# yigolden/JpegLibrary

Measured on AMD Instinct MI355X. Metric: Mpixels/s decoded, 4K 4:2:0 baseline Q75 RST=4, 1 & 8 GPU vs CPU ref, higher is better.
Workload: dtype f32; 1 GPU; 1024 x 3840x2160 420 baseline Q75 DRI=4 per GPU, output interleaved_u8 resident in HBM; images_per_gpu=1024

## Files before the change

jpeglibrary_amd/csrc/capi.cpp:

```cpp
#include <hip/hip_runtime.h>
#include <string.h>

#include <algorithm>
#include <chrono>
#include <exception>
#include <memory>
#include <new>
#include <thread>
#include <vector>

#include "../../include/jpgpu.h"
#include "device_batch.h"
#include "device_encode.h"
#include "device_optimize.h"
#include "host.h"

using namespace jpgpu;

struct jpgpu_batch {
    jpgpu_ctx *ctx;
    DeviceBatch impl;
    explicit jpgpu_batch(jpgpu_ctx *c) : ctx(c), impl(c) {}
};

// ... 311 lines not shown
    case JPGPU_DETAIL_MARKER_IN_DATA: return "Failed to decode JPEG data. Expect raw data from bit stream. Yet a marker is encountered.";
    case JPGPU_DETAIL_STREAM_ENDED: return "Failed to decode JPEG data. The bit stream ended prematurely.";
    case JPGPU_DETAIL_EXPECT_RESTART: return "Expect restart marker.";
    case JPGPU_DETAIL_MISSING_TABLE: return "Failed to decode JPEG data. A Huffman or quantization table is not defined.";
    case JPGPU_DETAIL_UNSUPPORTED_FRAME: return "This type of JPEG stream is not supported on the GPU path.";
    case JPGPU_DETAIL_BAD_HEADER: return "Failed to decode JPEG data. Malformed marker segment.";
    case JPGPU_DETAIL_EARLY_EOI: return "EndOfImage met at a restart boundary; image partially decoded.";
    case JPGPU_DETAIL_UNEXPECTED_END: return "Failed to decode JPEG data. Unexpected end of JPEG data stream.";
    case JPGPU_DETAIL_NULL_TABLE: return "Object reference not set to an instance of an object.";
    default: return "unknown detail";
    }
}


int jpgpu_batch_create(jpgpu_ctx *ctx, jpgpu_batch **out) {
    if (!ctx || !out) return JPGPU_ERR_ARGUMENT;
    *out = new (std::nothrow) jpgpu_batch(ctx);
    return *out ? JPGPU_OK : JPGPU_ERR_OUT_OF_MEMORY;
}
void jpgpu_batch_destroy(jpgpu_batch *b) { delete b; }

#define JPGPU_GUARD(b, expr)                                                   \
    if (!(b)) return JPGPU_ERR_ARGUMENT;                                       \
    try {                                                                      \
        return (expr);                                                         \
    } catch (const DecodeError &e) {                                           \
        (b)->ctx->last_error = e.what();                                       \
        return e.status;                                                       \
    } catch (const std::bad_alloc &) {                                         \
        (b)->ctx->last_error = "host allocation failed";                       \
        return JPGPU_ERR_OUT_OF_MEMORY;                                        \
    } catch (const std::exception &e) {                                        \
        (b)->ctx->last_error = e.what();                                       \
        return JPGPU_ERR_DEVICE;                                               \
    }

int jpgpu_batch_upload(jpgpu_batch *b, const uint8_t *const *jpeg, const size_t *len, int n, int format) {
    JPGPU_GUARD(b, b->impl.upload_files(jpeg, len, n, format));
}
int jpgpu_batch_upload_segments(jpgpu_batch *b, const jpgpu_segment *segments, const int *segments_per_file, int n, int format, unsigned flags) {
    JPGPU_GUARD(b, b->impl.upload_segments(segments, segments_per_file, n, format, flags));
}
int jpgpu_batch_upload_frames(jpgpu_batch *b, const jpgpu_frame *frames, const uint16_t *qt, int n, int format) {
    JPGPU_GUARD(b, b->impl.upload_frames(frames, qt, n, format));
}
int jpgpu_batch_decode(jpgpu_batch *b) { JPGPU_GUARD(b, b->impl.decode()); }
static int run_entropy_stages(DeviceBatch &impl) {
    impl.note_entropy_only_request();
    const int rc = impl.run_marker_index();
    return rc != JPGPU_OK ? rc : impl.run_huffman();
}
int jpgpu_batch_run_entropy(jpgpu_batch *b) { JPGPU_GUARD(b, run_entropy_stages(b->impl)); }
int jpgpu_batch_run_idct(jpgpu_batch *b) { JPGPU_GUARD(b, b->impl.run_idct()); }
int jpgpu_batch_sync(jpgpu_batch *b) { JPGPU_GUARD(b, b->impl.sync()); }
int jpgpu_batch_size(const jpgpu_batch *b) { return b ? b->impl.size() : 0; }

int jpgpu_batch_image_info(const jpgpu_batch *b, int i, jpgpu_image_info *info) {
    if (!b || !info) return JPGPU_ERR_ARGUMENT;
    const ImagePlan *img = b->impl.image(i);
    if (!img) return JPGPU_ERR_ARGUMENT;
    memset(info, 0, sizeof *info);
    info->status = img->status;
    info->detail = img->detail;
    info->width = img->width;
    info->height = img->height;
    info->precision = img->precision;
    info->num_components = img->num_components;
    info->sof = img->sof;
    info->restart_interval = img->restart_interval;
    info->mcus_per_line = img->mcus_per_line;
    info->mcus_per_column = img->mcus_per_column;
    info->blocks_per_mcu = img->blocks_per_mcu;
    info->total_blocks = img->total_blocks;
    info->out_offset = img->out_offset;
    info->out_bytes = img->out_bytes;
    info->coef_offset = img->coef_offset;
    memcpy(info->plane, img->plane, sizeof info->plane);
    if (img->status != JPGPU_OK) b->ctx->last_error = img->error;
    return JPGPU_OK;
}

int jpgpu_batch_result(jpgpu_batch *b, int i, jpgpu_image_result *res) { JPGPU_GUARD(b, b->impl.result(i, res)); }
void *jpgpu_batch_output_device(const jpgpu_batch *b, uint64_t *total_bytes) { return b ? b->impl.output_device(total_bytes) : nullptr; }
void *jpgpu_batch_coefficients_device(const jpgpu_batch *b, uint64_t *total_blocks) { return b ? b->impl.coefs_device(total_blocks) : nullptr; }
int jpgpu_batch_download_output(jpgpu_batch *b, int i, void *dst, size_t cap) { JPGPU_GUARD(b, b->impl.download_output(i, dst, cap)); }
int jpgpu_batch_download_coefficients(jpgpu_batch *b, int i, int16_t *dst, size_t cap_blocks) {
    JPGPU_GUARD(b, b->impl.download_coefficients(i, dst, cap_blocks));
}
int jpgpu_batch_upload_coefficients(jpgpu_batch *b, int i, const int16_t *src, size_t nblocks) {
    JPGPU_GUARD(b, b->impl.upload_coefficients(i, src, nblocks));
}
int jpgpu_batch_stage_ms(jpgpu_batch *b, float ms[4]) { JPGPU_GUARD(b, b->impl.stage_ms(ms)); }
int jpgpu_batch_subseq_rounds(const jpgpu_batch *b) { return b ? b->impl.last_subseq_rounds() : 0; }
int jpgpu_batch_set_partial_flush(jpgpu_batch *b, int on) {
    if (!b) return JPGPU_ERR_ARGUMENT;
    b->impl.set_partial_flush(on != 0);
    return JPGPU_OK;
}
int jpgpu_batch_marker_fallbacks(const jpgpu_batch *b) { return b ? b->impl.marker_fallbacks() : 0; }
int jpgpu_batch_progressive_replays(const jpgpu_batch *b) { return b ? b->impl.progressive_replays() : 0; }
int jpgpu_batch_subseq_fallbacks(const jpgpu_batch *b) { return b ? b->impl.subseq_fallbacks() : 0; }
int jpgpu_batch_progressive_fallbacks(const jpgpu_batch *b) { return b ? b->impl.progressive_fallbacks() : 0; }
int jpgpu_batch_ingest_stats(const jpgpu_batch *b, jpgpu_ingest_stats *stats) {
    if (!b || !stats) return JPGPU_ERR_ARGUMENT;
    const IngestStats &s = b->impl.ingest_stats();
    stats->threads = s.threads;
    stats->n_header_only = s.n_header_only;
    stats->n_full_walk = s.n_full_walk;
    stats->parse_ms = s.parse_ms;
    stats->copy_ms = s.copy_ms;
    stats->full_walk_ms = s.full_walk_ms;
    stats->layout_ms = s.layout_ms;
    stats->total_ms = s.total_ms;
    stats->n_pinned_dma = s.n_pinned_dma;
    stats->n_linearised = s.n_linearised;
    return JPGPU_OK;
}
size_t jpgpu_sizeof_plan_stats(void) { return sizeof(jpgpu_plan_stats); }
int jpgpu_batch_plan_stats(const jpgpu_batch *b, jpgpu_plan_stats *stats) {
    if (!b || !stats) return JPGPU_ERR_ARGUMENT;
    b->impl.plan_stats(stats);
    return JPGPU_OK;
}
static_assert(JPGPU_PROGRESSIVE_CHAINS == jpgpu_ctx::kProgChains, "jpgpu_progressive_plan: one count per chain stream");
size_t jpgpu_sizeof_progressive_plan(void) { return sizeof(jpgpu_progressive_plan); }
int jpgpu_batch_progressive_plan(const jpgpu_batch *b, jpgpu_progressive_plan *plan) {
    if (!b || !plan) return JPGPU_ERR_ARGUMENT;
    b->impl.progressive_plan(plan);
    return JPGPU_OK;
}
static_assert(JPGPU_IDCT_LAYOUT_CLASSES == kNumIdctLayoutClasses, "jpgpu_batch_idct_work: one count per K3 layout class");
int jpgpu_batch_idct_work(const jpgpu_batch *b, int32_t *counts, int n) {
    if (!b || !counts || n != JPGPU_IDCT_LAYOUT_CLASSES) return JPGPU_ERR_ARGUMENT;
    b->impl.idct_work(counts);
    return JPGPU_OK;
}
int jpgpu_batch_totals(const jpgpu_batch *b, uint64_t *compressed_bytes, uint64_t *blocks, uint64_t *pixels, uint64_t *output_bytes) {
    if (!b) return JPGPU_ERR_ARGUMENT;
    b->impl.totals(compressed_bytes, blocks, pixels, output_bytes);
    return JPGPU_OK;
}

}


namespace {

[[noreturn]] void throw_for_result(const jpgpu_image_result &res) {
    throw DecodeError(res.status, jpgpu_detail_string(res.detail), res.detail);
}

void write_block_expanded(jpgpu_write_block_fn fn, void *user, const int16_t *block, int component_index, int x, int y, int hs, int vs) {
    if (hs == 1 && vs == 1) {
        fn(user, block, component_index, x, y);
        return;
    }
    int16_t temp[64];
    int hshift = 0, vshift = 0;
    while ((1 << (hshift + 1)) <= hs) hshift++;
    while ((1 << (vshift + 1)) <= vs) vshift++;
    for (int v = 0; v < vs; v++)
        for (int h = 0; h < hs; h++) {
            for (int i = 0; i < 8; i++) {
                const int16_t *row = block + ((8 * v + i) >> vshift) * 8;
                for (int j = 0; j < 8; j++) temp[8 * i + j] = row[(8 * h + j) >> hshift];
            }
            fn(user, temp, component_index, x + 8 * h, y + 8 * v);
// ... 887 lines not shown
```

jpeglibrary_amd/csrc/common.h:

```cpp
#pragma once
#include <stdint.h>

namespace jpgpu {

constexpr int kMaxScanComponents = 4;
constexpr int kMaxBlocksPerMcu = 16;
constexpr int kHuffLutBits = 9;
constexpr int kHuffLutSize = 1 << kHuffLutBits;
constexpr int kMaxHuffSlots = 8;

struct alignas(16) DevHuffTable {
    uint16_t lut[kHuffLutSize];
    uint16_t maxcode[18];
    uint8_t valoffset[20];
    uint8_t values[256];
    uint8_t pad[8];
};
static_assert(sizeof(DevHuffTable) % 16 == 0, "DevHuffTable must be a multiple of 16 bytes");

struct alignas(16) DevQuantTable {
    uint16_t q[64];
};

struct DevScanComponent {
    uint8_t component_index;
    uint8_t h, v;
    uint8_t hs, vs;
    uint8_t quant_slot;
    uint8_t dc_slot, ac_slot;
};

enum OutputFormat : int32_t { kFmtInterleavedU8 = 0, kFmtPlanarU8 = 1, kFmtPlanarI16 = 2, kFmtRgbU8 = 3, kFmtRgbaU8 = 4, kFmtExtendedU16 = 5, kFmtInterleavedU8Scaled = 6 };
constexpr int kNumOutputFormats = 7;
constexpr bool fmt_is_sample_bytes(int f) { return f == kFmtInterleavedU8 || f == kFmtInterleavedU8Scaled; }
constexpr bool fmt_is_interleaved(int f) { return fmt_is_sample_bytes(f) || f == kFmtRgbU8 || f == kFmtRgbaU8; }
constexpr int fmt_bytes_per_pixel_rgb(int f) { return f == kFmtRgbaU8 ? 4 : 3; }

struct YccRgbFactors {
    int32_t cr_r, cr_g, cb_b, cb_g;
};

struct alignas(16) DevScan {
    uint64_t data_off;
    uint64_t coef_off;
    uint64_t out_off;
    uint64_t plane_off[kMaxScanComponents];
    uint32_t plane_pitch[kMaxScanComponents];
    uint32_t data_len;
    uint32_t dri;
    uint32_t total_mcus, mcus_per_line, mcus_per_column;
    uint32_t n_intervals;
    uint32_t ends_off;
    uint32_t image_index;
    uint32_t level_shift;
    uint16_t width, height;
    uint8_t precision, frame_components, scan_components, max_h, max_v, blocks_per_mcu;
    uint8_t restart_check_at_end;
    uint8_t shadow_mask;
    DevScanComponent comp[kMaxScanComponents];
    uint8_t blk_comp[kMaxBlocksPerMcu];
    uint8_t blk_x[kMaxBlocksPerMcu];
    uint8_t blk_y[kMaxBlocksPerMcu];
    uint16_t huff_pool[kMaxHuffSlots];
    uint16_t quant_pool[kMaxScanComponents];
    uint64_t reserved0;
    uint32_t chunk_off;
    uint32_t n_chunks;
    uint32_t sub_off;
    uint32_t n_subs;
    uint8_t kind;
    uint8_t ss, se, ah, al;
    uint8_t frame_bpm;
    uint8_t fblk_base[kMaxScanComponents];
    uint8_t publishes;
    uint8_t sub_shift;
    uint8_t wave_next;
    uint8_t debug_delay_ms;
    uint8_t pad1[2];
    uint16_t hblocks[kMaxScanComponents];
    uint16_t vblocks[kMaxScanComponents];
    uint32_t units_per_line;
    uint32_t dep[3];
    uint32_t last_interval;
    uint32_t first_scan;
    uint32_t sr_set;
    uint32_t pad2;
};
constexpr uint32_t kNoDep = 0xFFFFFFFFu;
constexpr uint32_t kFailBlockBase = 0xFFFFFFFFu;
constexpr uint32_t kIdctPartialMcu = 0xFFFFFFFFu;
constexpr uint64_t kScanStoreHoldsSamples = 1;
struct alignas(16) DisposeJob {
    uint64_t coef_off;
    uint32_t n_blocks;
    uint32_t bpm, level_shift;
    uint8_t blk_comp[kMaxBlocksPerMcu];
    uint8_t n[kMaxScanComponents];
    uint16_t quant[kMaxScanComponents][kMaxScanComponents];
    uint32_t pad[3];
};
constexpr uint8_t kKeepUnreachedMcus = 0x80;
enum ScanKind : uint8_t { kScanSequential = 0, kScanFrameOnly = 1, kScanProgressive = 2 };
static_assert(sizeof(DevScan) % 16 == 0, "DevScan must be a multiple of 16 bytes");

struct alignas(16) DevScanStatus {
    uint32_t n_ends;
    uint32_t terminator;
    uint32_t first_error;
    uint32_t decoded_mcus;
    uint32_t end_pos;
    uint32_t pad[3];
};

struct HuffWork {
    uint32_t scan;
    uint32_t first_interval;
};
struct ChunkWork {
    uint32_t scan;
    uint32_t chunk;
};
struct GatherPiece {
    uint64_t src;
    uint64_t dst_off;
    uint32_t len;
    uint32_t pad;
};
struct ChunkSum {
    uint32_t rst_cnt;
    uint32_t keep_cnt;
    uint32_t first_term;
    uint32_t pad;
};
struct IdctWork {
    uint32_t scan;
    uint32_t first_mcu;
    uint32_t n_mcus;
    uint32_t mcus_per_tile;
};

struct ExtendPlanes {
    uint64_t plane_off[4];
    uint64_t out_off;
    uint32_t pitch[4];
    uint32_t hshift[4], vshift[4];
    uint32_t width, height, ncomp, precision;
    uint32_t hcnt[4], vcnt[4];
    uint32_t max_h, max_v;
};

constexpr uint32_t kNoError = 0xFFFFFFFFu;

enum Detail : uint32_t {
    kDetailNone = 0,
    kDetailInvalidHuffmanCode = 1,
    kDetailMarkerInData = 2,
    kDetailStreamEnded = 3,
    kDetailExpectRestart = 4,
    kDetailMissingTable = 5,
    kDetailUnsupportedFrame = 6,
    kDetailBadHeader = 7,
    kDetailEarlyEoi = 8,
    kDetailUnexpectedEnd = 9,
    kDetailNullTable = 10,
    kDetailSpinTimeout = 11
};

}
```

jpeglibrary_amd/csrc/device_batch.cpp:

```cpp
#include "device_batch.h"

#include <hip/hip_runtime.h>
#include <sched.h>
#include <stdio.h>
#include <stdlib.h>
#include <string.h>

#include <algorithm>
#include <atomic>
#include <chrono>
#include <thread>

#include "host_pool.h"
#include "kernels.h"

namespace jpgpu {

static inline uint64_t align_up(uint64_t v, uint64_t a) { return (v + a - 1) / a * a; }

hipError_t DevBuffer::reserve(size_t bytes) {
    if (bytes <= cap && ptr) return hipSuccess;
    if (ptr) {
        hipError_t e = hipFree(ptr);
        ptr = nullptr;
        cap = 0;
        if (e != hipSuccess) return e;
    }
    if (bytes == 0) bytes = 256;
    hipError_t e = hipMalloc(&ptr, bytes);
    if (e == hipSuccess) cap = bytes;
    return e;
}
void DevBuffer::release() {
    if (ptr) (void)hipFree(ptr);
    ptr = nullptr;
    cap = 0;
}

DeviceBatch::~DeviceBatch() {
    if (ctx_) (void)hipSetDevice(ctx_->device);
    for (DevBuffer *b : {&d_sub_work_, &d_sub_final_work_, &d_sub_scan_ids_, &d_sub_exit_a_, &d_sub_exit_b_, &d_sub_nblk_, &d_sub_first_, &d_sub_entry_, &d_sub_dcsum_, &d_sub_dcentry_, &d_sub_changed_, &d_sub_same_, &d_sub_perm_, &d_k1_desc_, &d_k1_tickets_, &d_k2_tickets_, &d_sr_luts_, &d_sr_set_scan_, &d_k1_order_, &d_prog_snapshot_, &d_dispose_, &d_verify_, &d_lut_pool_, &d_prog_work_, &d_prog_sync_, &d_planes_, &d_extend_desc_, &d_gather_, &d_rgb_scratch_, &d_chunk_work_, &d_chunk_sums_, &d_unstuffed_, &d_ends_u_, &d_input_, &d_scans_, &d_status_, &d_ends_, &d_huff_pool_, &d_quant_pool_, &d_huff_work_, &d_idct_work_, &d_idct_work_split_, &d_coefs_, &d_out_})
        b->release();
    for (hipEvent_t &e : ev_pool_)
        if (e) (void)hipEventDestroy(e);
    if (done_ev_) (void)hipEventDestroy(done_ev_);
    if (h_k1_giveup_) (void)hipHostFree(h_k1_giveup_);
}

int DeviceBatch::fail(int status, const std::string &msg) {
    ctx_->last_error = msg;
    return status;
}
int DeviceBatch::hip_fail(hipError_t e, const char *what) {
    return fail(e == hipErrorOutOfMemory ? JPGPU_ERR_OUT_OF_MEMORY : JPGPU_ERR_DEVICE, std::string(what) + ": " + hipGetErrorString(e));
}

namespace {

class PlanHandler final : public ScanHandler {
  public:
    explicit PlanHandler(std::vector<ScanJob> *jobs, bool first_scan_only = false, const std::vector<int> *forced = nullptr)
        : jobs_(jobs), first_scan_only_(first_scan_only), forced_(forced) {}
    PlanHandler(const std::vector<size_t> *ends, int swallow) : jobs_(nullptr), replay_ends_(ends), swallow_(swallow) {}
    const std::vector<size_t> &sequential_ends() const { return ends_; }
    void on_frame(HostDecoder &dec, int sof) override {
        sof_ = sof;
        baseline_ = false;
        flush_progressive();
        if (sof == kSOF0 || sof == kSOF1) {
            geo_ = BaselineGeometry::latch(dec, dec.frame_header());
            baseline_ = true;
        } else if (sof == kSOF2) {
            prog_.begin(dec, dec.frame_header());
        }
    }
    void on_scan(HostDecoder &dec, MarkerReader &reader, const ScanHeader &scan) override {
        const uint8_t *entropy = reader.remaining_bytes();
        const size_t len = (size_t)reader.remaining_byte_count();
        if (prog_.active()) {
            prog_.add_scan(dec, scan, entropy, len);
            return;
        }
        if (!baseline_)
            throw DecodeError(JPGPU_ERR_NOT_SUPPORTED, "Only Huffman DCT frames (SOF0, SOF1, SOF2) run on this path.", kDetailUnsupportedFrame);
        if (scan.num_components == 0) {
            const uint64_t mcus = (uint64_t)geo_.mcus_per_line * (uint64_t)geo_.mcus_per_column;
            if (geo_.restart_interval != 0 && mcus >= geo_.restart_interval && len != 0 &&
                !(len >= 2 && entropy[0] == 0xFF && entropy[1] != 0x00 && entropy[1] != 0xFF))
                throw DecodeError(JPGPU_ERR_INVALID_OPERATION, "Expect restart marker.", kDetailExpectRestart);
            if (first_scan_only_)
                throw DecodeError(JPGPU_ERR_NOT_SUPPORTED, "A scan without components is not supported by the optimizer path.", kDetailUnsupportedFrame);
            if (geo_.restart_interval != 0 && mcus >= geo_.restart_interval)
                throw DecodeError(JPGPU_ERR_NOT_SUPPORTED, "A scan without components in front of restart markers is not supported.", kDetailUnsupportedFrame);
            reader.try_advance((int)find_scan_end(entropy, len));
            return;
        }
        if (replay_ends_) {
            const int k = replayed_++;
            if (k > swallow_ || k >= (int)replay_ends_->size())
                throw DecodeError(JPGPU_ERR_NOT_SUPPORTED, "A scan behind a scan that left one byte unread is not supported.", kDetailUnsupportedFrame);
            reader.try_advance((int)(*replay_ends_)[k] + (k == swallow_ ? 1 : 0));
            return;
        }
        jobs_->push_back(make_scan_job(dec, geo_, scan, entropy, len, first_scan_only_));
        if (!first_scan_only_) {
            const bool forced = forced_ != nullptr && std::find(forced_->begin(), forced_->end(), (int)ends_.size()) != forced_->end();
            ends_.push_back(find_scan_end(entropy, len));
            jobs_->back().forced_swallow = forced && ends_.back() < len;
            reader.try_advance((int)ends_.back() + (jobs_->back().forced_swallow ? 1 : 0));
            return;
        }
        reader.try_advance(first_scan_only_ ? (int)len : (int)find_scan_end(entropy, len));
    }
    void on_dispose(HostDecoder &) override { flush_progressive(); }
    const BaselineGeometry &geo() const { return prog_geo_valid_ ? prog_geo_ : geo_; }
    int sof() const { return sof_; }

  private:
    void flush_progressive() {
        if (!prog_.active()) return;
        if (jobs_) {
            jobs_->push_back(prog_.make_frame_job());
            for (ScanJob &j : prog_.scans()) jobs_->push_back(std::move(j));
            prog_geo_ = prog_.geo();
// ... 941 lines not shown
```

jpeglibrary_amd/csrc/device_batch.h:

```cpp
#pragma once
#include <hip/hip_runtime_api.h>

#include <map>
#include <string>
#include <vector>

#include "../../include/jpgpu.h"
#include "common.h"
#include "host.h"
#include "kernels.h"

namespace jpgpu {
int default_host_threads();
int granted_host_cpus();
}

struct StagingRing {
    static constexpr int kMaxSlots = 16;
    int n_slots = 8;
    size_t slot_bytes = 32u << 20;
    uint8_t *slot[kMaxSlots] = {};
    hipEvent_t drained[kMaxSlots] = {};
    uint32_t *verdict = nullptr;
    size_t verdict_cap = 0;
// ... 12 lines not shown
    std::string last_error;
    int num_cus = 0;
    uint64_t device_bytes = 0;
};

namespace jpgpu {

struct DevBuffer {
    void *ptr = nullptr;
    size_t cap = 0;
    hipError_t reserve(size_t bytes);
    void release();
};

struct IngestStats {
    int threads = 0;
    int n_header_only = 0;
    int n_full_walk = 0;
    float parse_ms = 0, copy_ms = 0, full_walk_ms = 0, layout_ms = 0, total_ms = 0;
    int n_pinned_dma = 0;
    int n_linearised = 0;
};

struct ImagePlan {
    int status = JPGPU_OK;
    int detail = 0;
    std::string error;
    int late_status = JPGPU_OK, late_detail = 0;
    bool replay_skip = false;
    std::string late_error;
    int swallow_job = -1, swallow_status = JPGPU_OK, swallow_detail = 0;
    std::string swallow_error;
    uint16_t width = 0, height = 0;
    uint8_t precision = 0, num_components = 0, sof = 0;
    uint32_t restart_interval = 0;
    uint32_t mcus_per_line = 0, mcus_per_column = 0, blocks_per_mcu = 0;
    uint64_t total_blocks = 0;
    uint64_t out_offset = 0, out_bytes = 0;
    uint64_t planes_offset = 0, planes_bytes = 0;
    uint64_t coef_offset = 0;
    jpgpu_plane_info plane[4] = {};
    std::vector<int> jobs;
    uint64_t file_offset = 0;
    size_t file_len = 0;
};

class WorkCrew;

class DeviceBatch {
  public:
    const IngestStats &ingest_stats() const { return ingest_; }
    void plan_stats(jpgpu_plan_stats *st) const;
    void progressive_plan(jpgpu_progressive_plan *p) const;
    void idct_work(int32_t counts[kNumIdctLayoutClasses]) const;
    explicit DeviceBatch(jpgpu_ctx *ctx) : ctx_(ctx) {}
    ~DeviceBatch();

    int upload_files(const uint8_t *const *jpeg, const size_t *len, int n, int format);
    void set_forced_swallow(const std::vector<int> &ordinals) { forced_swallow_ = ordinals; }
    int upload_segments(const jpgpu_segment *segments, const int *segments_per_file, int n, int format, unsigned flags);
    int upload_progressive_frame(const ProgressiveFrame &frame, const uint8_t *file, size_t file_len, int sof, int format);
    int upload_progressive_scan(const ProgressiveFrame &frame, int scan_index, bool first_scan);
    int snapshot_progressive_store();
    int rerun_failed_progressive_scan(bool first_scan);
    int upload_progressive_dispose(const ProgressiveFrame &frame, int format);
    int upload_single_job(const ScanJob &job, int format, const void *initial_output, size_t initial_output_bytes);
    int upload_frames(const jpgpu_frame *frames, const uint16_t *qt , int n, int format);

    int run_marker_index();
    int run_huffman();
    int run_subseq_sync(const uint32_t **final_state, const uint32_t **first_block);
    int run_idct();
    int run_progressive();
    int decode();
    int sync();

    int size() const { return (int)images_.size(); }
    const ImagePlan *image(int i) const { return (i >= 0 && i < (int)images_.size()) ? &images_[i] : nullptr; }
    int result(int i, jpgpu_image_result *res);
    void *output_device(uint64_t *total) const {
        if (total) *total = out_bytes_;
        return d_out_.ptr;
    }
    void *coefs_device(uint64_t *total_blocks) const {
        if (total_blocks) *total_blocks = total_blocks_;
        return d_coefs_.ptr;
    }
    int download_output(int i, void *dst, size_t cap);
    int download_coefficients(int i, int16_t *dst, size_t cap_blocks);
    int upload_coefficients(int i, const int16_t *src, size_t nblocks);
    int stage_ms(float ms[4]);
    void totals(uint64_t *compressed, uint64_t *blocks, uint64_t *pixels, uint64_t *out_bytes) const;
    int format() const { return format_; }
    void note_entropy_only_request() { in_decode_request_ = false; }
    int last_subseq_rounds() const { return last_subseq_rounds_; }
    int progressive_fallbacks() const { return prog_fallbacks_; }
    int subseq_fallbacks() const { return k2s_fallbacks_; }
    int marker_fallbacks() const { return k1_fallbacks_; }
    int progressive_replays() const { return prog_replays_; }
    void set_partial_flush(bool on) { partial_flush_ = on; }
    void set_entropy_only(bool on) { entropy_only_ = on; }
    void set_preset_restart_intervals(std::vector<int> v) { preset_dri_ = std::move(v); }
    void set_preset_no_subseq(std::vector<uint8_t> v) { preset_no_subseq_ = std::move(v); }

  private:
    friend class OptimizeBatch;
    bool entropy_only_ = false;
    std::vector<int> preset_dri_;
    std::vector<uint8_t> preset_no_subseq_;
    int fail(int status, const std::string &msg);
    int hip_fail(hipError_t e, const char *what);
    int layout_and_upload(const std::vector<const uint8_t *> &file_ptr, const std::vector<size_t> &file_len);
    void plan_image_geometry(ImagePlan &img, const BaselineGeometry &geo) const;
    struct FilePlan;
    void plan_file_headers(const uint8_t *file, size_t len, FilePlan &fp) const;
    void plan_file_full(const uint8_t *file, size_t len, int index, FilePlan &fp) const;
    void plan_swallowed_terminator(FilePlan &fp, const uint8_t *file, size_t len, bool identify_is_clean) const;
    struct FileSegs;
    int stage_files(WorkCrew &crew, const std::vector<FileSegs> &files, const std::vector<FilePlan> &plans, bool pinned);
    int mark_work();
    int order_upload_behind_work();
    std::pair<const uint8_t *, size_t> arena_span_ = {nullptr, 0};
    hipEvent_t done_ev_ = nullptr;
    bool work_in_flight_ = false;
    int verify_plans(const std::vector<FilePlan> &plans, const std::vector<int> &spec, std::vector<uint32_t> &first);
    bool whole_files_ = false;
    bool files_resident_ = false;
    IngestStats ingest_;
    DevBuffer d_verify_;
    int fetch_status();
    int clear_partial_outputs();
    bool keep_progressive_store_ = false;
    bool defer_refusal_ = false;
    bool keep_canvas_ = false;
    struct OutClear {
        uint64_t first, second;
        uint64_t planes_first, planes_bytes;
    };
    std::vector<OutClear> out_clear_;

    jpgpu_ctx *ctx_;
    int format_ = JPGPU_FMT_INTERLEAVED_U8;
    std::vector<ImagePlan> images_;
    std::vector<ScanJob> jobs_;
    std::vector<int> job_image_;
    std::vector<uint64_t> job_entropy_off_;
    std::vector<DevScan> h_scans_;
    std::vector<DevScanStatus> h_status_;
    bool status_valid_ = false;
    std::vector<DevHuffTable> huff_pool_;
    std::vector<DevQuantTable> quant_pool_;
    int n_huff_slots_ = 1;
    int redo_swallowed(int i, int job, jpgpu_image_result *res);
    std::vector<int> forced_swallow_;
    struct Redo {
        jpgpu_image_result res;
        std::string error;
    };
    std::map<int, Redo> redo_;
    std::vector<SubseqPool> k2_pools_;
    uint32_t k2_ticket_base_[kK2MaxPools] = {};
    uint32_t k2_tab_bytes_ = 0;
    int n_huff_work_ = 0, n_idct_work_ = 0;
    int idct_class_begin_[kNumIdctLayoutClasses + 1] = {};
    std::vector<int> idct_later_begin_;
    uint64_t total_blocks_ = 0, out_bytes_ = 0, planes_bytes_ = 0, input_bytes_ = 0, compressed_bytes_ = 0, total_pixels_ = 0;
    DevBuffer d_planes_;
    DevBuffer d_extend_desc_;
    DevBuffer d_gather_;
    bool in_decode_request_ = false;
    uint32_t total_ends_ = 0;

    DevBuffer d_lut_pool_;
    DevBuffer d_sub_work_, d_sub_scan_ids_, d_sub_exit_a_, d_sub_exit_b_, d_sub_nblk_, d_sub_first_, d_sub_entry_, d_sub_dcsum_, d_sub_dcentry_, d_sub_changed_, d_sub_same_, d_sub_perm_;
    DevBuffer d_prog_snapshot_;
    uint64_t prog_snapshot_blocks_ = 0;
    DevBuffer d_dispose_;
    std::vector<DisposeJob> dispose_jobs_;
    uint32_t dispose_max_blocks_ = 0;
    int run_dispose_passes(hipStream_t stream);
    bool dispose_done_ = false;
    int replay_failed_progressive();
    bool replay_done_ = false, replay_possible_ = false, prog_by_scan_ = false;
    bool replay_layout_active_ = false, in_replay_ = false;
    bool partial_flush_ = true;
    std::vector<std::pair<size_t, ScanJob>> replay_saved_jobs_;
    int restore_after_replay();
    int prog_replays_ = 0;
  public:
    int clear_progressive_stores();
  private:
    DevBuffer d_k1_desc_, d_k1_tickets_, d_k1_order_;
    int n_k1_groups_ = 0;
    uint32_t *h_k1_giveup_ = nullptr;
    uint32_t k1_epoch_ = 0, k1_tag_ = 0;
    bool k1_onepass_ = true;
    int k1_fallbacks_ = 0;
    bool sub_same_valid_ = false;
    int n_sub_work_ = 0, n_sub_gather_ = 0, n_sub_scans_ = 0, n_sub_final_work_ = 0, sub_final_spl_ = 2;
    int n_sr_sets_ = 0;
    DevBuffer d_sub_final_work_;
    std::vector<SubseqPool> sub_pools_;
    uint32_t total_subs_ = 0, max_subs_per_scan_ = 0;
    std::vector<uint32_t> sub_scan_ids_;
    int last_subseq_rounds_ = 0;
    int k2s_budget_ = 0, k2s_issued_ = 0, k2s_fallbacks_ = 0;
    bool k2s_unchecked_ = false, k2s_idct_behind_ = false, k2s_host_checked_ = false;
    int check_subseq_rounds();
    DevBuffer d_prog_work_, d_prog_sync_;
    std::vector<int> prog_begin_;
    std::vector<int> prog_stream_begin_;
    int prog_pipe_begin_ = 0, prog_pipe_count_ = 0;
    std::vector<int> prog_chain_begin_[jpgpu_ctx::kProgChains];
    bool prog_chains_ok_ = false;
    bool prog_pipelined_ = false;
    uint32_t prog_spin_budget_ = 1u << 22;
    int prog_scans_ = 0, prog_max_deps_ = 0, prog_wave_tails_ = 0, prog_launch_form_ = 0;
    int prog_chain_scans_[jpgpu_ctx::kProgChains] = {};
    int prog_fallbacks_ = 0;
    std::vector<std::pair<uint64_t, uint64_t>> prog_clear_;
    struct RgbConvert {
        uint32_t image;
        uint64_t out_offset, pixels;
        int components;
    };
    std::vector<RgbConvert> rgb_convert_;
    DevBuffer d_rgb_scratch_;
    DevBuffer d_chunk_work_, d_chunk_sums_;
    int n_chunk_work_ = 0;
    DevBuffer d_unstuffed_, d_ends_u_;
    DevBuffer d_input_, d_scans_, d_status_, d_ends_, d_huff_pool_, d_quant_pool_, d_huff_work_, d_idct_work_, d_coefs_, d_out_, d_k2_tickets_;
    DevBuffer d_sr_luts_, d_sr_set_scan_;
    std::vector<hipEvent_t> ev_pool_;
    size_t ev_used_ = 0;
    std::vector<bool> ev_serial_;
    static constexpr int kSerialEvery = 8;
    bool overlap_ok_ = false;
    int decodes_since_query_ = 0;
    int huff_split_ = 0;
    int idct_split_begin_[2][kNumIdctLayoutClasses + 1] = {};
    DevBuffer d_idct_work_split_;
};

}
```

jpeglibrary_amd/csrc/device_batch_launch.cpp:

```cpp
#include "device_batch.h"

#include <hip/hip_runtime.h>
#include <stdio.h>
#include <stdlib.h>
#include <string.h>

#include <algorithm>
#include <atomic>
#include <chrono>
#include <thread>
#include <vector>

#include "kernels.h"

namespace jpgpu {

int DeviceBatch::run_marker_index() {
    status_valid_ = false;
    redo_.clear();
    if (k1_onepass_) {
        const char *bev = getenv("JPGPU_K1_SPIN_BUDGET");
        const uint32_t budget = bev ? (uint32_t)strtoul(bev, nullptr, 10) : (1u << 20);
        uint32_t *tickets = (uint32_t *)d_k1_tickets_.ptr;
        hipError_t e1 = launch_marker_onepass(ctx_->stream, (const uint8_t *)d_input_.ptr, (const DevScan *)d_scans_.ptr, (const ChunkWork *)d_k1_order_.ptr,
                                              n_k1_groups_, d_k1_desc_.ptr, tickets, k1_epoch_, ++k1_tag_ ? k1_tag_ : ++k1_tag_, budget,
                                              h_k1_giveup_, (uint32_t *)d_ends_.ptr, (DevScanStatus *)d_status_.ptr,
                                              (uint8_t *)d_unstuffed_.ptr, (uint32_t *)d_ends_u_.ptr);
        if (e1 != hipSuccess) return hip_fail(e1, "marker_onepass_kernel");
        k1_epoch_++;
        return mark_work();
    }
    hipError_t e = launch_marker_index(ctx_->stream, (const uint8_t *)d_input_.ptr, (const DevScan *)d_scans_.ptr, (int)h_scans_.size(),
                                       (const ChunkWork *)d_chunk_work_.ptr, n_chunk_work_, (ChunkSum *)d_chunk_sums_.ptr,
                                       (uint32_t *)d_ends_.ptr, (DevScanStatus *)d_status_.ptr, (uint8_t *)d_unstuffed_.ptr,
                                       (uint32_t *)d_ends_u_.ptr);
    return e == hipSuccess ? mark_work() : hip_fail(e, "marker_index_kernel");
}
int DeviceBatch::run_huffman() {
    status_valid_ = false;
    redo_.clear();
    dispose_done_ = false;
    hipError_t e = launch_huffman(ctx_->stream, (const uint8_t *)d_unstuffed_.ptr, (const DevScan *)d_scans_.ptr, (const HuffWork *)d_huff_work_.ptr,
                                  n_huff_work_, (const uint32_t *)d_ends_u_.ptr, (DevScanStatus *)d_status_.ptr,
                                  (const DevHuffTable *)d_huff_pool_.ptr, (int16_t *)d_coefs_.ptr, n_huff_slots_, (const uint8_t *)d_lut_pool_.ptr, k2_tab_bytes_);
    if (e != hipSuccess) return hip_fail(e, "huffman_decode_kernel");
    for (size_t p = 0; p < k2_pools_.size(); p++) {
        const int waves = huffman_waves(k2_tab_bytes_);
        const int groups = std::min(ctx_->num_cus > 0 ? ctx_->num_cus : 256, (k2_pools_[p].count + waves - 1) / waves);
        e = launch_huffman_pool(ctx_->stream, (const uint8_t *)d_unstuffed_.ptr, (const DevScan *)d_scans_.ptr,
                                (const HuffWork *)d_huff_work_.ptr + n_huff_work_ + k2_pools_[p].first, k2_pools_[p].count, (uint32_t *)d_k2_tickets_.ptr + p,
                                k2_ticket_base_[p], groups, (const uint32_t *)d_ends_u_.ptr, (DevScanStatus *)d_status_.ptr, (int16_t *)d_coefs_.ptr,
                                n_huff_slots_, (const uint8_t *)d_lut_pool_.ptr, k2_tab_bytes_);
        if (e != hipSuccess) return hip_fail(e, "huffman_pool_kernel");
        k2_ticket_base_[p] += (uint32_t)k2_pools_[p].count + (uint32_t)(groups * waves);
    }
    if (n_sub_work_ > 0) {
        const int max_rounds = (int)max_subs_per_scan_ + 2;
        const int first_budget = getenv("JPGPU_SUBSEQ_BUDGET") ? std::max(2, atoi(getenv("JPGPU_SUBSEQ_BUDGET"))) : kSubseqFirstBudget;
        const int device_rounds = k2s_host_checked_ ? 0 : std::min(max_rounds, k2s_budget_ > 0 ? k2s_budget_ : first_budget);
        k2s_issued_ = std::min(device_rounds, kSubseqMaxDeviceRounds);
        k2s_unchecked_ = device_rounds > 0;
        k2s_idct_behind_ = false;
        e = launch_subseq_decode(ctx_->stream, (const uint8_t *)d_unstuffed_.ptr, (const DevScan *)d_scans_.ptr, (const HuffWork *)d_sub_work_.ptr,
                                 n_sub_work_, (const uint32_t *)d_sub_scan_ids_.ptr, n_sub_scans_, (const uint32_t *)d_ends_u_.ptr,
                                 (DevScanStatus *)d_status_.ptr, (const DevHuffTable *)d_huff_pool_.ptr, (uint32_t *)d_sub_exit_a_.ptr,
                                 (uint32_t *)d_sub_exit_b_.ptr, (uint32_t *)d_sub_nblk_.ptr, (uint32_t *)d_sub_first_.ptr,
                                 (uint32_t *)d_sub_entry_.ptr, d_sub_dcsum_.ptr, d_sub_dcentry_.ptr, (uint32_t *)d_sub_changed_.ptr, (int16_t *)d_coefs_.ptr, n_huff_slots_, max_rounds,
                                 &last_subseq_rounds_, (const uint8_t *)d_lut_pool_.ptr, (const HuffWork *)d_sub_final_work_.ptr, n_sub_final_work_,
                                 (uint32_t *)d_sub_same_.ptr, &sub_same_valid_, device_rounds, (const HuffWork *)d_sub_work_.ptr + n_sub_work_, n_sub_gather_,
                                 (const HuffWork *)d_sub_final_work_.ptr + n_sub_final_work_, sub_pools_.data(), (int)sub_pools_.size(), ctx_->num_cus,
                                 (uint32_t *)d_sub_perm_.ptr, sub_final_spl_, k2_tab_bytes_, (const uint8_t *)d_sr_luts_.ptr);
        if (e != hipSuccess) return hip_fail(e, "subsequence decode");
    }
    const int rc = run_progressive();
    return rc != JPGPU_OK ? rc : mark_work();
}
int DeviceBatch::run_subseq_sync(const uint32_t **final_state, const uint32_t **first_block) {
    *final_state = (const uint32_t *)d_sub_exit_a_.ptr;
    *first_block = (const uint32_t *)d_sub_first_.ptr;
    if (n_sub_work_ <= 0) return JPGPU_OK;
    status_valid_ = false;
    hipError_t e = launch_subseq_sync(ctx_->stream, (const uint8_t *)d_unstuffed_.ptr, (const DevScan *)d_scans_.ptr, (const HuffWork *)d_sub_work_.ptr,
                                      n_sub_work_, (const uint32_t *)d_sub_scan_ids_.ptr, n_sub_scans_, (const uint32_t *)d_ends_u_.ptr,
                                      (DevScanStatus *)d_status_.ptr, (const DevHuffTable *)d_huff_pool_.ptr, (uint32_t *)d_sub_exit_a_.ptr,
                                      (uint32_t *)d_sub_exit_b_.ptr, (uint32_t *)d_sub_nblk_.ptr, (uint32_t *)d_sub_first_.ptr,
                                      (uint32_t *)d_sub_entry_.ptr, d_sub_dcsum_.ptr, d_sub_dcentry_.ptr, (uint32_t *)d_sub_changed_.ptr,
                                      n_huff_slots_, (int)max_subs_per_scan_ + 2, &last_subseq_rounds_, (const uint8_t *)d_lut_pool_.ptr,
                                      final_state, (uint32_t *)d_sub_same_.ptr, &sub_same_valid_, 0 ,
                                      (const HuffWork *)d_sub_work_.ptr + n_sub_work_, n_sub_gather_, (const uint8_t *)d_sr_luts_.ptr);
    if (e != hipSuccess) return hip_fail(e, "subsequence synchronisation");
    return mark_work();
}
int DeviceBatch::run_progressive() {
    if (prog_begin_.size() <= 1 && prog_clear_.empty()) return JPGPU_OK;
    status_valid_ = false;
    for (size_t k = 0; k < prog_clear_.size() && !keep_progressive_store_;) {
        uint64_t first = prog_clear_[k].first, blocks = prog_clear_[k].second;
        for (k++; k < prog_clear_.size() && prog_clear_[k].first == first + blocks; k++) blocks += prog_clear_[k].second;
        hipError_t e = hipMemsetAsync((int16_t *)d_coefs_.ptr + first * 64, 0, (size_t)blocks * 128, ctx_->stream);
        if (e != hipSuccess) return hip_fail(e, "hipMemsetAsync(progressive store)");
    }
    if (prog_begin_.size() <= 1) return JPGPU_OK;
    const char *dbg_max = getenv("JPGPU_DEBUG_MAX_PROGRESSIVE_SCANS");
    const int n_streams = prog_stream_begin_.back() - prog_stream_begin_.front();
    const int n_waves = prog_pipe_count_;
    const size_t lds_per_wg = (progressive_stream_lds_bytes(n_huff_slots_) + 1023) / 1024 * 1024;
    const int cus = ctx_->num_cus > 0 ? ctx_->num_cus : 256;
    int per_cu = (int)std::min<size_t>(32, (160u << 10) / lds_per_wg);
    {
        static std::atomic<int> cached[kMaxHuffSlots + 1];
        const int slot_key = std::min(std::max(n_huff_slots_, 0), kMaxHuffSlots);
        int occ = cached[slot_key].load(std::memory_order_relaxed);
        if (occ == 0) {
            occ = progressive_stream_blocks_per_cu(n_huff_slots_);
            cached[slot_key].store(occ > 0 ? occ : -1, std::memory_order_relaxed);
        }
        if (occ > 0) per_cu = std::min(per_cu, occ);
    }
    const bool force = getenv("JPGPU_PROG_FORCE_PIPELINE") != nullptr;
    const bool resident = n_waves <= per_cu * 3 / 4 * cus;
    const bool fits = resident || force;
    const int launch_mode = resident && !force ? 1 : 2;
    const bool no_chains = getenv("JPGPU_PROG_NO_CHAINS") != nullptr;
    if (!(prog_pipelined_ && fits) && prog_chains_ok_ && !no_chains && !dbg_max && getenv("JPGPU_PROG_BY_SCAN") == nullptr && !prog_by_scan_ && n_streams > 0) {
// ... 19 lines not shown
            if ((e = hipStreamWaitEvent(st, cx->prog_ev[jpgpu_ctx::kProgChains], 0)) != hipSuccess) return hip_fail(e, "hipStreamWaitEvent");
            for (size_t jx = 0; jx + 1 < prog_chain_begin_[x].size(); jx++) {
                e = launch_progressive_streams(st, (const uint8_t *)d_unstuffed_.ptr, (const DevScan *)d_scans_.ptr,
                                               (const HuffWork *)d_prog_work_.ptr + prog_chain_begin_[x][jx],
                                               prog_chain_begin_[x][jx + 1] - prog_chain_begin_[x][jx], (const uint32_t *)d_ends_u_.ptr,
                                               (DevScanStatus *)d_status_.ptr, (const DevHuffTable *)d_huff_pool_.ptr, (int16_t *)d_coefs_.ptr,
                                               n_huff_slots_, 0, 0, nullptr);
                if (e != hipSuccess) return hip_fail(e, "progressive_stream_kernel");
            }
            if ((e = hipEventRecord(cx->prog_ev[x], st)) != hipSuccess) return hip_fail(e, "hipEventRecord");
            if ((e = hipStreamWaitEvent(cx->stream, cx->prog_ev[x], 0)) != hipSuccess) return hip_fail(e, "hipStreamWaitEvent");
        }
        return JPGPU_OK;
    }
    if (prog_pipelined_ && fits && !dbg_max) {
        hipError_t e0 = hipMemsetAsync(d_prog_sync_.ptr, 0, 256, ctx_->stream);
        if (e0 != hipSuccess) return hip_fail(e0, "hipMemsetAsync(progressive sync)");
        const int n = n_waves;
        prog_launch_form_ = launch_mode == 1 ? JPGPU_PROG_LAUNCH_PIPELINED_GATED : JPGPU_PROG_LAUNCH_PIPELINED_FORCED;
        hipError_t e = launch_progressive_streams(ctx_->stream, (const uint8_t *)d_unstuffed_.ptr, (const DevScan *)d_scans_.ptr,
                                                  (const HuffWork *)d_prog_work_.ptr + prog_pipe_begin_, n,
                                                  (const uint32_t *)d_ends_u_.ptr, (DevScanStatus *)d_status_.ptr,
                                                  (const DevHuffTable *)d_huff_pool_.ptr, (int16_t *)d_coefs_.ptr, n_huff_slots_, launch_mode, prog_spin_budget_, (uint32_t *)d_prog_sync_.ptr);
        if (e != hipSuccess) return hip_fail(e, "progressive_stream_kernel");
        return JPGPU_OK;
    }
    prog_launch_form_ = JPGPU_PROG_LAUNCH_BY_LEVEL;
    for (size_t k = 0; k + 1 < prog_begin_.size(); k++) {
        if (dbg_max && (int)k >= atoi(dbg_max)) break;
        hipError_t e = launch_progressive(ctx_->stream, (const uint8_t *)d_unstuffed_.ptr, (const DevScan *)d_scans_.ptr,
                                          (const HuffWork *)d_prog_work_.ptr + prog_begin_[k], prog_begin_[k + 1] - prog_begin_[k],
                                          (const uint32_t *)d_ends_u_.ptr, (DevScanStatus *)d_status_.ptr,
                                          (const DevHuffTable *)d_huff_pool_.ptr, (int16_t *)d_coefs_.ptr, n_huff_slots_);
        if (e != hipSuccess) return hip_fail(e, "progressive_scan_kernel");
        e = launch_progressive_streams(ctx_->stream, (const uint8_t *)d_unstuffed_.ptr, (const DevScan *)d_scans_.ptr,
                                       (const HuffWork *)d_prog_work_.ptr + prog_stream_begin_[k],
                                       prog_stream_begin_[k + 1] - prog_stream_begin_[k], (const uint32_t *)d_ends_u_.ptr,
                                       (DevScanStatus *)d_status_.ptr, (const DevHuffTable *)d_huff_pool_.ptr, (int16_t *)d_coefs_.ptr,
                                       n_huff_slots_, 0, 0, nullptr);
        if (e != hipSuccess) return hip_fail(e, "progressive_stream_kernel");
    }
    return JPGPU_OK;
}
int DeviceBatch::clear_partial_outputs() {
    for (const auto &c : out_clear_) {
        hipError_t e = hipMemsetAsync((uint8_t *)d_out_.ptr + c.first, 0, c.second, ctx_->stream);
        if (e == hipSuccess && format_ == JPGPU_FMT_EXTENDED_U16 && c.planes_bytes)
            e = hipMemsetAsync((uint8_t *)d_planes_.ptr + c.planes_first, 0, c.planes_bytes, ctx_->stream);
        if (e == hipSuccess && d_rgb_scratch_.ptr && c.first + c.second <= d_rgb_scratch_.cap)
            e = hipMemsetAsync((uint8_t *)d_rgb_scratch_.ptr + c.first, 0, c.second, ctx_->stream);
        if (e != hipSuccess) return hip_fail(e, "hipMemsetAsync(output)");
    }
    return JPGPU_OK;
}

int DeviceBatch::clear_progressive_stores() {
    dispose_done_ = false;
    for (const auto &c : prog_clear_) {
        hipError_t e = hipMemsetAsync((int16_t *)d_coefs_.ptr + c.first * 64, 0, (size_t)c.second * 128, ctx_->stream);
        if (e != hipSuccess) return hip_fail(e, "hipMemsetAsync(progressive store)");
    }
    return JPGPU_OK;
}

int DeviceBatch::run_dispose_passes(hipStream_t stream) {
    if (dispose_jobs_.empty() || dispose_done_) return JPGPU_OK;
    dispose_done_ = true;
    const hipError_t e = launch_dispose_pass(stream, (int16_t *)d_coefs_.ptr, (const DisposeJob *)d_dispose_.ptr, (int)dispose_jobs_.size(), dispose_max_blocks_,
                                             (const DevQuantTable *)d_quant_pool_.ptr);
    return e == hipSuccess ? JPGPU_OK : hip_fail(e, "dispose_pass_kernel");
}

int DeviceBatch::run_idct() {
    redo_.clear();
    if (k2s_unchecked_) k2s_idct_behind_ = true;
    const YccRgbFactors kf = ycc_rgb_factors();
    int rc0 = clear_partial_outputs();
    if (rc0 != JPGPU_OK) return rc0;
    if ((rc0 = run_dispose_passes(ctx_->stream)) != JPGPU_OK) return rc0;
    const bool extended = format_ == JPGPU_FMT_EXTENDED_U16;
    hipError_t e = launch_idct(ctx_->stream, (const int16_t *)d_coefs_.ptr, (const DevScan *)d_scans_.ptr, (const IdctWork *)d_idct_work_.ptr,
                               idct_class_begin_, (const DevScanStatus *)d_status_.ptr, (const DevQuantTable *)d_quant_pool_.ptr,
                               extended ? (uint8_t *)d_planes_.ptr : (uint8_t *)d_out_.ptr, extended ? (int)JPGPU_FMT_PLANAR_I16 : format_, kf,
                               (uint8_t *)d_rgb_scratch_.ptr);
    if (e != hipSuccess) return hip_fail(e, "idct_output_kernel");
    for (size_t lv = 0; lv + 1 < idct_later_begin_.size(); lv++) {
        int cb[kNumIdctLayoutClasses + 1];
        cb[0] = idct_later_begin_[lv];
        for (int c = 1; c <= kNumIdctLayoutClasses; c++) cb[c] = idct_later_begin_[lv + 1];
        e = launch_idct(ctx_->stream, (const int16_t *)d_coefs_.ptr, (const DevScan *)d_scans_.ptr, (const IdctWork *)d_idct_work_.ptr, cb,
                        (const DevScanStatus *)d_status_.ptr, (const DevQuantTable *)d_quant_pool_.ptr,
                        extended ? (uint8_t *)d_planes_.ptr : (uint8_t *)d_out_.ptr, extended ? (int)JPGPU_FMT_PLANAR_I16 : format_, kf,
                        (uint8_t *)d_rgb_scratch_.ptr);
        if (e != hipSuccess) return hip_fail(e, "idct_output_kernel (ordered scans)");
    }
    if (extended) {
        std::vector<ExtendPlanes> desc;
        uint32_t max_pixels = 0;
        for (const ImagePlan &img : images_) {
            if (img.status != JPGPU_OK || img.jobs.empty() || img.out_bytes == 0) continue;
            ExtendPlanes g;
            memset(&g, 0, sizeof g);
            const BaselineGeometry &geo = jobs_[img.jobs[0]].geo;
            for (int c = 0; c < 4; c++) g.pitch[c] = 1;
            for (int c = 0; c < img.num_components && c < 4; c++) {
                g.plane_off[c] = img.planes_offset + img.plane[c].offset;
                g.pitch[c] = img.plane[c].pitch;
                const int hs = geo.max_h / std::max<int>(1, geo.frame.components[c].h), vs = geo.max_v / std::max<int>(1, geo.frame.components[c].v);
                while ((1 << (g.hshift[c] + 1)) <= hs) g.hshift[c]++;
                while ((1 << (g.vshift[c] + 1)) <= vs) g.vshift[c]++;
                g.hcnt[c] = std::max<int>(1, geo.frame.components[c].h);
                g.vcnt[c] = std::max<int>(1, geo.frame.components[c].v);
            }
            bool flush = false;
            for (int j : img.jobs) flush |= jobs_[j].kind != kScanSequential;
            g.max_h = flush ? 0u : (uint32_t)geo.max_h;
            g.max_v = flush ? 0u : (uint32_t)geo.max_v;
            g.out_off = img.out_offset;
            g.width = img.width;
            g.height = img.height;
            g.ncomp = img.num_components;
            g.precision = img.precision;
            max_pixels = std::max<uint64_t>(max_pixels, std::min<uint64_t>((uint64_t)img.width * img.height, 0xFFFFFFFFu));
            desc.push_back(g);
        }
        if (!desc.empty()) {
            e = d_extend_desc_.reserve(desc.size() * sizeof(ExtendPlanes));
            if (e != hipSuccess) return hip_fail(e, "hipMalloc(extend descriptors)");
            e = hipMemcpyAsync(d_extend_desc_.ptr, desc.data(), desc.size() * sizeof(ExtendPlanes), hipMemcpyHostToDevice, ctx_->stream);
            if (e == hipSuccess) e = hipStreamSynchronize(ctx_->stream);
            if (e != hipSuccess) return hip_fail(e, "hipMemcpyAsync(extend descriptors)");
            e = launch_extend_u16(ctx_->stream, (const uint8_t *)d_planes_.ptr, (uint8_t *)d_out_.ptr, (const ExtendPlanes *)d_extend_desc_.ptr,
                                  (int)desc.size(), max_pixels);
            if (e != hipSuccess) return hip_fail(e, "extend_u16_kernel");
        }
    }
    for (const RgbConvert &rc : rgb_convert_) {
        e = launch_ycc_to_rgb(ctx_->stream, (const uint8_t *)d_rgb_scratch_.ptr + rc.out_offset, (uint8_t *)d_out_.ptr + rc.out_offset, rc.pixels,
                              rc.components, format_ == JPGPU_FMT_RGBA_U8 ? 4 : 3, kf);
        if (e != hipSuccess) return hip_fail(e, "ycc_to_rgb_kernel");
    }
    return mark_work();
}

int DeviceBatch::decode() {
    hipError_t e = hipSetDevice(ctx_->device);
    if (e != hipSuccess) return hip_fail(e, "hipSetDevice");
    if (replay_layout_active_ && !in_replay_) {
        const int rr = restore_after_replay();
        if (rr != JPGPU_OK) return rr;
    }
    if (ev_used_ + 4 > 4 * 256) {
        ev_used_ = 0;
        ev_serial_.clear();
    }
    if (ev_pool_.size() < ev_used_ + 4) {
        for (int k = 0; k < 64; k++) {
            hipEvent_t ev = nullptr;
            e = hipEventCreate(&ev);
            if (e != hipSuccess) return hip_fail(e, "hipEventCreate");
            ev_pool_.push_back(ev);
        }
    }
    hipEvent_t *ev = &ev_pool_[ev_used_];
    redo_.clear();
    in_decode_request_ = true;
    const bool serial = !overlap_ok_ || (decodes_since_query_ % kSerialEvery) == 0;
// ... 118 lines not shown
```

jpeglibrary_amd/csrc/device_batch_layout.cpp:

```cpp
#include "device_batch.h"

#include <hip/hip_runtime.h>
#include <stdio.h>
#include <stdlib.h>
#include <string.h>

#include <algorithm>
#include <atomic>
#include <chrono>
#include <thread>
#include <vector>

#include "kernels.h"

namespace jpgpu {

static inline uint64_t align_up(uint64_t v, uint64_t a) { return (v + a - 1) / a * a; }

namespace {
template <typename T>
void xcd_interleave(std::vector<T> &w, int xcds) {
    if (xcds <= 1 || w.size() < (size_t)xcds * 8) return;
    const size_t n = w.size(), per = (n + xcds - 1) / xcds;
    std::vector<T> m;
// ... 8 lines not shown

int DeviceBatch::layout_and_upload(const std::vector<const uint8_t *> &file_ptr, const std::vector<size_t> &file_len) {
    dispose_done_ = false;
    if (!in_replay_) {
        replay_done_ = false;
        replay_possible_ = false;
        prog_by_scan_ = false;
        replay_layout_active_ = false;
        replay_saved_jobs_.clear();
        for (ImagePlan &img : images_) img.replay_skip = false;
    }
    hipError_t e = hipSetDevice(ctx_->device);
    if (e != hipSuccess) return hip_fail(e, "hipSetDevice");
    {
        const int rc0 = order_upload_behind_work();
        if (rc0 != JPGPU_OK) return rc0;
    }
    status_valid_ = false;
    ev_used_ = 0;
    keep_progressive_store_ = false;
    defer_refusal_ = false;

    if (!files_resident_) {
        uint64_t in_off = 256;
        for (size_t i = 0; i < images_.size(); i++) {
            images_[i].file_offset = in_off;
            if (images_[i].status == JPGPU_OK && !images_[i].jobs.empty()) in_off = align_up(in_off + file_len[i], 256);
        }
        input_bytes_ = in_off + 256;
    }
    hipStream_t up = ctx_->upload_stream;

    int dbg_delay_scan = -1, dbg_delay_ms = 0;
    if (const char *dd = getenv("JPGPU_DEBUG_DELAY_SCAN")) {
        if (sscanf(dd, "%d:%d", &dbg_delay_scan, &dbg_delay_ms) != 2) dbg_delay_scan = -1;
    }
    const bool dbg_status = getenv("JPGPU_DEBUG_STATUS") != nullptr;
    huff_pool_.clear();
    quant_pool_.clear();
    h_scans_.assign(jobs_.size(), DevScan());
    std::vector<HuffWork> huff_work;
    std::vector<ChunkWork> chunk_work;
    std::vector<ChunkWork> k1_order;
    std::vector<HuffWork> sub_work;
    uint32_t subseq_shift = 10;
    {
        uint64_t dri0_bits = 0;
        for (size_t j = 0; j < jobs_.size(); j++)
            if (jobs_[j].kind == kScanSequential && jobs_[j].geo.restart_interval == 0) dri0_bits += (uint64_t)jobs_[j].entropy_len * 8;
        while (subseq_shift < 12 && (dri0_bits >> subseq_shift) >= 500000u) subseq_shift++;
        while (subseq_shift > 9 && (dri0_bits >> subseq_shift) < 4096u) subseq_shift--;
        if (const char *ev = getenv("JPGPU_SUBSEQ_SHIFT")) subseq_shift = (uint32_t)std::min(14, std::max(8, atoi(ev)));
    }
    uint32_t idct_tiles_per_wg = (uint32_t)kIdctTilesPerWg;
    {
        uint64_t blocks = 0;
        for (const ScanJob &job : jobs_)
            if (job.kind != kScanProgressive) blocks += (uint64_t)job.geo.mcus_per_line * job.geo.mcus_per_column * (uint64_t)std::max(1, job.blocks_per_mcu);
        const uint64_t tiles = blocks / (uint64_t)kIdctBlocksPerWg + 1, want_wgs = 3ull * (uint64_t)(ctx_->num_cus > 0 ? ctx_->num_cus : 256);
        while (idct_tiles_per_wg > 1 && tiles / idct_tiles_per_wg < want_wgs) idct_tiles_per_wg /= 2;
    }
    std::vector<std::vector<HuffWork>> prog_work_by_ordinal, prog_streams_by_ordinal;
    std::vector<std::vector<HuffWork>> prog_chain_work[jpgpu_ctx::kProgChains];
    prog_chains_ok_ = true;
    prog_scans_ = prog_max_deps_ = prog_wave_tails_ = prog_launch_form_ = 0;
    for (int &n : prog_chain_scans_) n = 0;
    const uint32_t stream_max_intervals = getenv("JPGPU_PROG_STREAM_MAX_INTERVALS") ? (uint32_t)atoi(getenv("JPGPU_PROG_STREAM_MAX_INTERVALS")) : 16u;
    prog_clear_.clear();
    prog_pipelined_ = getenv("JPGPU_PROG_NO_PIPELINE") == nullptr;
    prog_spin_budget_ = getenv("JPGPU_PROG_SPIN_BUDGET") ? (uint32_t)strtoul(getenv("JPGPU_PROG_SPIN_BUDGET"), nullptr, 10) : (1u << 17);
    prog_fallbacks_ = 0;
    rgb_convert_.clear();
    sub_scan_ids_.clear();
    total_subs_ = 0;
    max_subs_per_scan_ = 0;
    sub_same_valid_ = false;
    k2s_budget_ = 0;
    k2s_unchecked_ = k2s_idct_behind_ = false;
    k2s_host_checked_ = getenv("JPGPU_SUBSEQ_HOST_CHECK") != nullptr || keep_canvas_;
    dispose_jobs_.clear();
    dispose_max_blocks_ = 0;
    std::vector<IdctWork> idct_work;
    std::vector<IdctWork> idct_work_by_class[kNumIdctLayoutClasses];
    std::vector<std::vector<IdctWork>> idct_later_levels;
    std::vector<IdctWork> idct_partial;
    std::vector<int> scan_level(jobs_.size(), 0);
    const bool tile_align = !(getenv("JPGPU_TILE_ALIGN") && atoi(getenv("JPGPU_TILE_ALIGN")) == 0);
    uint64_t out_off = 0, coef_off = 0, planes_off = 0;
    uint32_t ends_off = 0, total_chunks = 0;
    compressed_bytes_ = 0;
    total_pixels_ = 0;
    n_huff_slots_ = 1;
    for (const ScanJob &job : jobs_) n_huff_slots_ = std::max(n_huff_slots_, job.n_huff);
    k2_tab_bytes_ = kK2AcTabBytes + kK2DcTabBytes;
    for (const ScanJob &job : jobs_) {
        if (job.kind != kScanSequential) continue;
        uint32_t bytes = 0;
        for (int k = 0; k < job.n_huff; k++) {
            bool is_dc = false;
            for (int c = 0; c < job.scan_components; c++) is_dc |= job.dc_slot[c] == k;
            bytes += is_dc ? kK2DcTabBytes : kK2AcTabBytes;
        }
        k2_tab_bytes_ = std::max(k2_tab_bytes_, bytes);
    }
    const uint32_t huff_intervals_per_wg = 64u * (uint32_t)huffman_waves(k2_tab_bytes_);
    struct HuffKey {
        uint8_t bits[16];
        uint16_t num_values;
        uint8_t values[256];
    };
    std::vector<HuffKey> huff_keys;
    auto huff_index = [&](const HuffTable &t) -> uint16_t {
        for (size_t i = 0; i < huff_keys.size(); i++)
            if (huff_keys[i].num_values == t.num_values && memcmp(huff_keys[i].bits, t.bits, 16) == 0 &&
                memcmp(huff_keys[i].values, t.values, t.num_values) == 0)
                return (uint16_t)i;
        DevHuffTable d;
        t.to_device(&d);
        HuffKey k;
        memcpy(k.bits, t.bits, 16);
        k.num_values = t.num_values;
        memcpy(k.values, t.values, sizeof k.values);
        huff_keys.push_back(k);
        huff_pool_.push_back(d);
        return (uint16_t)(huff_pool_.size() - 1);
    };
    auto quant_index = [&](const QuantTable &t) -> uint16_t {
        DevQuantTable d;
        memcpy(d.q, t.elements, sizeof d.q);
        for (size_t i = 0; i < quant_pool_.size(); i++)
            if (memcmp(&quant_pool_[i], &d, sizeof d) == 0) return (uint16_t)i;
        quant_pool_.push_back(d);
        return (uint16_t)(quant_pool_.size() - 1);
    };

    for (size_t ii = 0; ii < images_.size(); ii++) {
        ImagePlan &img = images_[ii];
        img.out_offset = out_off;
        img.planes_offset = planes_off;
        img.coef_offset = coef_off;
        img.total_blocks = 0;
        if (img.status != JPGPU_OK) continue;
        out_off = align_up(out_off + img.out_bytes, 256);
        planes_off = align_up(planes_off + img.planes_bytes, 256);
        if (!img.jobs.empty()) total_pixels_ += (uint64_t)img.width * img.height;
        bool overlapping_scans = false;
        {
            uint32_t seen = 0;
            for (int j : img.jobs) {
                const ScanJob &job = jobs_[j];
                if (job.kind != kScanSequential || job.disabled) continue;
                uint32_t mine = 0;
                for (int c = 0; c < job.scan_components; c++) mine |= 1u << (job.comp[c].component_index & 31);
                overlapping_scans |= (mine & seen) != 0;
                seen |= mine;
            }
        }
        for (int j : img.jobs) {
            const ScanJob &job = jobs_[j];
            DevScan &s = h_scans_[j];
            memset(&s, 0, sizeof s);
            const BaselineGeometry &g = job.geo;
            s.kind = (uint8_t)job.kind;
            s.last_interval = job.last_interval;
            s.data_off = img.file_offset + job_entropy_off_[j];
            s.data_len = (uint32_t)(file_len[ii] - job_entropy_off_[j]);
// ... 43 lines not shown
            s.blocks_per_mcu = (uint8_t)job.blocks_per_mcu;
            s.restart_check_at_end = (s.dri != 0 && s.total_mcus % s.dri == 0) ? 1 : 0;
            for (int k = 0; k < kMaxHuffSlots; k++) s.huff_pool[k] = 0xFFFF;
            for (int k = 0; k < job.n_huff; k++) s.huff_pool[k] = huff_index(job.huff_copy[k]);
            n_huff_slots_ = std::max(n_huff_slots_, job.n_huff);
            for (int c = 0; c < job.scan_components; c++) {
                DevScanComponent &dc = s.comp[c];
                dc.component_index = (uint8_t)job.comp[c].component_index;
                dc.h = job.comp[c].h;
                dc.v = job.comp[c].v;
                dc.hs = (uint8_t)job.comp[c].hs;
                dc.vs = (uint8_t)job.comp[c].vs;
                dc.quant_slot = (uint8_t)c;
                dc.dc_slot = job.dc_slot[c];
                dc.ac_slot = job.ac_slot[c];
                s.quant_pool[c] = quant_index(job.quant_copy[c]);
                const int fc = job.comp[c].component_index;
                if (fc < 4) {
                    s.plane_off[c] = img.plane[fc].offset;
                    s.plane_pitch[c] = img.plane[fc].pitch;
                }
            }
            s.shadow_mask = keep_canvas_ ? kKeepUnreachedMcus : 0;
            for (int c = 0; c < job.scan_components; c++)
                for (int d = c + 1; d < job.scan_components; d++)
                    if (job.comp[c].component_index == job.comp[d].component_index) s.shadow_mask |= (uint8_t)(1u << c);
            memcpy(s.blk_comp, job.blk_comp, sizeof s.blk_comp);
            memcpy(s.blk_x, job.blk_x, sizeof s.blk_x);
            memcpy(s.blk_y, job.blk_y, sizeof s.blk_y);
            if (job.kind == kScanFrameOnly && job.dispose_generic) {
                s.reserved0 |= kScanStoreHoldsSamples;
                DisposeJob dj;
                memset(&dj, 0, sizeof dj);
                dj.bpm = (uint32_t)job.blocks_per_mcu;
                dj.level_shift = 1u << (g.frame.precision - 1);
                memcpy(dj.blk_comp, job.blk_comp, sizeof dj.blk_comp);
                for (int c = 0; c < kMaxScanComponents; c++) {
                    dj.n[c] = job.dispose_n[c];
                    for (int t = 0; t < job.dispose_n[c]; t++) dj.quant[c][t] = quant_index(job.dispose_q[c][t]);
                }
                dj.n_blocks = 0xFFFFFFFFu;
                dj.coef_off = (uint64_t)j;
                if (!img.replay_skip) dispose_jobs_.push_back(dj);
            }

            if (job.kind == kScanProgressive) {
                static const bool by_scan_env = getenv("JPGPU_PROG_BY_SCAN") != nullptr;
                const bool by_scan = by_scan_env || prog_by_scan_;
                if (job.disabled || img.replay_skip) continue;
                const int ordinal = by_scan ? j - img.jobs[0] - 1 : job.ordinal;
                prog_scans_++;
                prog_max_deps_ = std::max(prog_max_deps_, (int)job.n_deps);
                if (by_scan) prog_pipelined_ = false;
                if ((size_t)ordinal >= prog_work_by_ordinal.size()) {
                    prog_work_by_ordinal.resize((size_t)ordinal + 1);
                    prog_streams_by_ordinal.resize((size_t)ordinal + 1);
                }
                for (int d = 0; d < 3; d++) s.dep[d] = d < job.n_deps && job.deps[d] >= 0 ? (uint32_t)(img.jobs[0] + 1 + job.deps[d]) : kNoDep;
                s.publishes = job.has_consumers ? 1 : 0;
                if (dbg_delay_scan >= 0 && dbg_delay_scan == j - img.jobs[0] - 1) s.debug_delay_ms = (uint8_t)std::min(255, std::max(0, dbg_delay_ms));
                const bool empty_band = job.ss != 0 && job.ss > job.se;
                if (job.n_deps > 3 || s.n_intervals != 1 || s.n_intervals > stream_max_intervals || empty_band || job.force_lane) prog_pipelined_ = false;
                if (s.n_intervals <= stream_max_intervals && !job.force_lane && !empty_band) {
                    for (uint32_t i = 0; i < s.n_intervals; i++) prog_streams_by_ordinal[ordinal].push_back({(uint32_t)j, i});
                    const int chain = (job.scan_components != 1 || job.ss == 0) ? 0 : 1 + std::min(3, job.comp[0].component_index);
                    int in_chain = 0;
                    for (int jj = img.jobs[0] + 1; jj < j; jj++) {
                        const ScanJob &o = jobs_[jj];
                        in_chain += ((o.scan_components != 1 || o.ss == 0) ? 0 : 1 + std::min(3, o.comp[0].component_index)) == chain;
                    }
                    if (prog_chain_work[chain].size() <= (size_t)in_chain) prog_chain_work[chain].resize((size_t)in_chain + 1);
                    prog_chain_scans_[chain]++;
                    for (uint32_t i = 0; i < s.n_intervals; i++) prog_chain_work[chain][(size_t)in_chain].push_back({(uint32_t)j, i});
                } else {
                    prog_chains_ok_ = false;
                    for (uint32_t first = 0; first < s.n_intervals; first += 256) prog_work_by_ordinal[ordinal].push_back({(uint32_t)j, first});
                }
                compressed_bytes_ += s.data_len;
                continue;
            }
            const uint64_t nblocks = (uint64_t)s.mcus_per_line * s.mcus_per_column * s.blocks_per_mcu;
            if (job.kind == kScanFrameOnly && !img.replay_skip) prog_clear_.push_back({coef_off, nblocks});
            coef_off += nblocks;
            img.total_blocks += nblocks;
            compressed_bytes_ += s.data_len;
            bool null_table = false;
            for (int c = 0; c < job.scan_components; c++) null_table |= job.dc_slot[c] == kNullHuffSlot || job.ac_slot[c] == kNullHuffSlot;
            const bool use_subseq = s.dri == 0 && s.total_mcus > 0 && s.data_len >= 512 && !null_table && getenv("JPGPU_NO_SUBSEQ") == nullptr &&
                                    !(entropy_only_ && (size_t)ii < preset_no_subseq_.size() && preset_no_subseq_[ii]);
            if (job.kind == kScanFrameOnly) {
            } else if (use_subseq) {
                s.sub_shift = (uint8_t)subseq_shift;
                s.n_subs = (uint32_t)((((uint64_t)s.data_len * 8) + ((1u << subseq_shift) - 1)) >> subseq_shift);
                s.sub_off = total_subs_;
                total_subs_ += s.n_subs;
                max_subs_per_scan_ = std::max(max_subs_per_scan_, s.n_subs);
                if (!img.replay_skip) {
                    sub_scan_ids_.push_back((uint32_t)j);
                    for (uint32_t first = 0; first < s.n_subs; first += 256) sub_work.push_back({(uint32_t)j, first});
                }
            } else {
                for (uint32_t first = 0; first < s.n_intervals && !img.replay_skip; first += huff_intervals_per_wg) huff_work.push_back({(uint32_t)j, first});
            }
            if (img.replay_skip) continue;
            if (s.blocks_per_mcu == 0) continue;
            uint32_t mcus_per_wg = (uint32_t)kIdctBlocksPerWg / s.blocks_per_mcu;
            if (tile_align) {
                uint32_t row_bytes = 8u * s.max_h;
                if (fmt_is_sample_bytes(format_)) row_bytes *= s.frame_components;
                else if (format_ == JPGPU_FMT_RGB_U8) row_bytes *= 3;
                else if (format_ == JPGPU_FMT_RGBA_U8) row_bytes *= 4;
                else if (format_ == JPGPU_FMT_PLANAR_I16 || format_ == JPGPU_FMT_EXTENDED_U16) row_bytes *= 2;
                for (uint32_t t = mcus_per_wg; t * 4 >= mcus_per_wg * 3 && t > 0; t--)
                    if ((t * row_bytes) % 128 == 0) {
                        mcus_per_wg = t;
                        break;
                    }
            }
            const bool holds_samples = (s.reserved0 & kScanStoreHoldsSamples) != 0;
            int cls = holds_samples ? kIdctClassStoreHoldsSamples : (fmt_is_interleaved(format_) ? idct_layout_class(s) : 0);
            if (!holds_samples && overlapping_scans && (format_ == JPGPU_FMT_RGB_U8 || format_ == JPGPU_FMT_RGBA_U8)) cls = 0;
            if ((cls == 0 || holds_samples) && (format_ == JPGPU_FMT_RGB_U8 || format_ == JPGPU_FMT_RGBA_U8)) {
                bool listed = false;
                for (const RgbConvert &rc : rgb_convert_) listed |= rc.image == (uint32_t)ii;
                if (!listed) rgb_convert_.push_back({(uint32_t)ii, img.out_offset, (uint64_t)img.width * img.height, img.num_components});
            }
            int level = 0;
            if (job.kind == kScanSequential && img.jobs.size() > 1) {
                uint32_t mine = 0;
                for (int c = 0; c < job.scan_components; c++) mine |= 1u << (job.comp[c].component_index & 31);
                for (int j2 : img.jobs) {
                    if (j2 == j) break;
                    const ScanJob &o = jobs_[(size_t)j2];
                    if (o.kind != kScanSequential || o.disabled) continue;
                    uint32_t theirs = 0;
                    for (int c = 0; c < o.scan_components; c++) theirs |= 1u << (o.comp[c].component_index & 31);
                    if (mine & theirs) level = std::max(level, scan_level[(size_t)j2] + 1);
                }
            }
            scan_level[(size_t)j] = level;
            const uint32_t run = mcus_per_wg * idct_tiles_per_wg;
            if (level > 0) {
                h_scans_[j].shadow_mask |= kKeepUnreachedMcus;
                if ((size_t)level > idct_later_levels.size()) idct_later_levels.resize((size_t)level);
                const uint32_t generic_per_wg = ((uint32_t)kIdctBlocksPerWg / s.blocks_per_mcu);
                const uint32_t grun = generic_per_wg * idct_tiles_per_wg;
                for (uint32_t first = 0; first < s.total_mcus; first += grun)
                    idct_later_levels[(size_t)level - 1].push_back({(uint32_t)j, first, std::min(grun, s.total_mcus - first), generic_per_wg});
                if (format_ == JPGPU_FMT_RGB_U8 || format_ == JPGPU_FMT_RGBA_U8) {
                    bool listed = false;
                    for (const RgbConvert &rc : rgb_convert_) listed |= rc.image == (uint32_t)ii;
                    if (!listed) rgb_convert_.push_back({(uint32_t)ii, img.out_offset, (uint64_t)img.width * img.height, img.num_components});
                }
            } else {
                for (uint32_t first = 0; first < s.total_mcus; first += run)
                    idct_work_by_class[cls].push_back({(uint32_t)j, first, std::min(run, s.total_mcus - first), mcus_per_wg});
                if (keep_canvas_ && job.kind == kScanSequential && fmt_is_sample_bytes(format_) &&
                    cls >= 1 && cls <= 3)
                    idct_partial.push_back({(uint32_t)j, kIdctPartialMcu, 1, ((uint32_t)kIdctBlocksPerWg / s.blocks_per_mcu)});
            }
        }
    }
    for (DisposeJob &dj : dispose_jobs_) {
        const DevScan &fs = h_scans_[(size_t)dj.coef_off];
        dj.coef_off = fs.coef_off;
        dj.n_blocks = fs.total_mcus * (uint32_t)fs.blocks_per_mcu;
        dispose_max_blocks_ = std::max(dispose_max_blocks_, dj.n_blocks);
    }
    total_blocks_ = coef_off;
    out_bytes_ = out_off;
    planes_bytes_ = planes_off;
    total_ends_ = ends_off;
    auto same_tables = [&](const DevScan &a, const DevScan &b) {
        return memcmp(a.huff_pool, b.huff_pool, sizeof a.huff_pool) == 0 && a.scan_components == b.scan_components &&
               a.blocks_per_mcu == b.blocks_per_mcu && memcmp(a.blk_comp, b.blk_comp, sizeof a.blk_comp) == 0 &&
               memcmp(a.comp, b.comp, sizeof a.comp) == 0;
    };
    k2_pools_.clear();
    {
        std::vector<HuffWork> plain, pooled;
#ifdef JPGPU_K2_NO_POOL
        const bool no_pool = true;
#else
        const bool no_pool = getenv("JPGPU_OVERLAP") != nullptr && atoi(getenv("JPGPU_OVERLAP")) != 0;
#endif
        size_t i = 0;
        while (i < huff_work.size() && !no_pool) {
            size_t k = i;
            uint64_t chunks = 0;
            const DevScan &a = h_scans_[huff_work[i].scan];
            while (k < huff_work.size() && same_tables(a, h_scans_[huff_work[k].scan])) {
                if (huff_work[k].first_interval == 0) chunks += (h_scans_[huff_work[k].scan].n_intervals + 63u) / 64u;
                k++;
            }
            const bool pool = (int)k2_pools_.size() < kK2MaxPools && chunks >= 2 && chunks < 0x7FFFFFFFu;
            if (pool) k2_pools_.push_back({(int)pooled.size(), (int)chunks});
            for (size_t q = i; q < k; q++) {
                if (!pool) plain.push_back(huff_work[q]);
                else if (huff_work[q].first_interval == 0)
                    for (uint32_t first = 0; first < h_scans_[huff_work[q].scan].n_intervals; first += 64u) pooled.push_back({huff_work[q].scan, first});
            }
            i = k;
        }
        if (!no_pool) huff_work.swap(plain);
        n_huff_work_ = (int)huff_work.size();
        huff_work.insert(huff_work.end(), pooled.begin(), pooled.end());
    }
    for (uint32_t &b : k2_ticket_base_) b = 0;
    std::vector<uint32_t> sr_set_scan;
    for (uint32_t j : sub_scan_ids_) {
        uint32_t k = 0;
        while (k < sr_set_scan.size() && !same_tables(h_scans_[sr_set_scan[k]], h_scans_[j])) k++;
        if (k == sr_set_scan.size()) sr_set_scan.push_back(j);
        h_scans_[j].sr_set = k;
    }
    n_sr_sets_ = (int)sr_set_scan.size();
    n_chunk_work_ = (int)chunk_work.size();
    std::stable_sort(k1_order.begin(), k1_order.end(), [](const ChunkWork &a, const ChunkWork &b) { return a.chunk < b.chunk; });
    n_k1_groups_ = (int)k1_order.size();
    n_sub_work_ = (int)sub_work.size();
    for (uint32_t j : sub_scan_ids_)
        for (uint32_t first = 0; first < h_scans_[j].n_subs; first += kSubseqGatherSpan) sub_work.push_back({j, first});
    n_sub_gather_ = (int)sub_work.size() - n_sub_work_;
    std::vector<HuffWork> sub_final_work;
    sub_pools_.clear();
    {
#ifdef JPGPU_SF_NO_POOL
        const bool no_pool = true;
#else
        const bool no_pool = !subseq_pool_fits(k2_tab_bytes_);
#endif
#ifdef JPGPU_SF_ONE_SUB
        sub_final_spl_ = 1;
#else
        sub_final_spl_ = (kSubFinalSubsPerLane >= 2 && total_subs_ >= kSubFinalFewSubs) ? 2 : 1;
#endif
        const uint32_t lanes_subs = 64u * (uint32_t)sub_final_spl_;
        std::vector<HuffWork> pooled;
        size_t i = 0;
        while (i < sub_scan_ids_.size()) {
            size_t k = i + 1;
            uint64_t waves = (h_scans_[sub_scan_ids_[i]].n_subs + lanes_subs - 1) / lanes_subs;
            while (k < sub_scan_ids_.size() && same_tables(h_scans_[sub_scan_ids_[i]], h_scans_[sub_scan_ids_[k]])) {
                waves += (h_scans_[sub_scan_ids_[k]].n_subs + lanes_subs - 1) / lanes_subs;
                k++;
            }
            const bool pool = !no_pool && waves >= (uint64_t)kSubFinalPoolMinChunks && (int)sub_pools_.size() < kSubFinalMaxPools && waves < 0x7FFFFFFFu;
            if (pool) sub_pools_.push_back({(int)pooled.size(), (int)waves});
            for (size_t q = i; q < k; q++) {
                const uint32_t j = sub_scan_ids_[q];
                const uint32_t step = pool ? lanes_subs : lanes_subs * (uint32_t)subseq_final_waves();
                for (uint32_t first = 0; first < h_scans_[j].n_subs; first += step) (pool ? pooled : sub_final_work).push_back({j, first});
// ... 6 lines not shown
    n_sub_scans_ = (int)sub_scan_ids_.size();
    std::vector<HuffWork> prog_work;
    prog_begin_.assign(1, 0);
    for (const std::vector<HuffWork> &w : prog_work_by_ordinal) {
        prog_work.insert(prog_work.end(), w.begin(), w.end());
        prog_begin_.push_back((int)prog_work.size());
    }
    prog_stream_begin_.assign(1, (int)prog_work.size());
    for (const std::vector<HuffWork> &w : prog_streams_by_ordinal) {
        prog_work.insert(prog_work.end(), w.begin(), w.end());
        prog_stream_begin_.push_back((int)prog_work.size());
    }
    prog_pipe_begin_ = (int)prog_work.size();
    {
        static const bool no_wave_chains = getenv("JPGPU_PROG_NO_WAVE_CHAINS") != nullptr;
        std::vector<uint8_t> is_tail(h_scans_.size(), 0);
        for (const ImagePlan &img : images_) {
            if (img.jobs.size() < 2 || no_wave_chains) continue;
            const int j0 = img.jobs[0] + 1, n = (int)img.jobs.size() - 1;
            uint64_t largest = 0;
            for (int k = 0; k < n; k++)
                if (jobs_[(size_t)(j0 + k)].kind == kScanProgressive) largest = std::max<uint64_t>(largest, h_scans_[(size_t)(j0 + k)].data_len);
            std::vector<uint64_t> wave_bytes((size_t)n, 0);
            std::vector<uint8_t> has_next((size_t)n, 0);
            for (int k = 0; k < n; k++) {
                const ScanJob &job = jobs_[(size_t)(j0 + k)];
                if (job.kind != kScanProgressive) continue;
                const uint64_t own = h_scans_[(size_t)(j0 + k)].data_len;
                wave_bytes[(size_t)k] = own;
                if (job.n_deps != 1 || job.deps[0] < 0 || job.deps[0] >= k || job.has_consumers) continue;
                if (job.scan_components != 1 || job.ss == 0) continue;
                const int a = job.deps[0];
                if (jobs_[(size_t)(j0 + a)].kind != kScanProgressive || has_next[(size_t)a] || k - a > 255) continue;
                const uint64_t together = wave_bytes[(size_t)a] + own;
                if (together > largest / 2 || together > (1u << 20)) continue;
                if (dbg_status && &img == &images_[0])
                    fprintf(stderr, "jpgpu: wave chain: scan %d behind scan %d (%llu + %llu bytes, largest scan %llu)\n", k, a,
                            (unsigned long long)wave_bytes[(size_t)a], (unsigned long long)own, (unsigned long long)largest);
                h_scans_[(size_t)(j0 + a)].wave_next = (uint8_t)(k - a);
                has_next[(size_t)a] = 1;
                is_tail[(size_t)(j0 + k)] = 1;
                prog_wave_tails_++;
                wave_bytes[(size_t)k] = together;
            }
        }
        for (const std::vector<HuffWork> &w : prog_streams_by_ordinal)
            for (const HuffWork &hw : w)
                if (!is_tail[hw.scan]) prog_work.push_back(hw);
    }
    prog_pipe_count_ = (int)prog_work.size() - prog_pipe_begin_;
    for (int x = 0; x < jpgpu_ctx::kProgChains; x++) {
        prog_chain_begin_[x].assign(1, (int)prog_work.size());
        for (const std::vector<HuffWork> &w : prog_chain_work[x]) {
            prog_work.insert(prog_work.end(), w.begin(), w.end());
            prog_chain_begin_[x].push_back((int)prog_work.size());
        }
    }
    out_clear_.clear();
    for (const ImagePlan &img : images_) {
        if (img.status != JPGPU_OK || img.out_bytes == 0) continue;
        uint64_t covered[4] = {0, 0, 0, 0};
        for (int j : img.jobs) {
            const DevScan &s = h_scans_[j];
            if (jobs_[j].kind == kScanProgressive) continue;
            for (int c = 0; c < s.scan_components; c++) covered[s.comp[c].component_index >> 6] |= 1ull << (s.comp[c].component_index & 63);
        }
        bool all = true;
        for (int j : img.jobs) {
            const DevScan &s = h_scans_[j];
            if (jobs_[j].kind != kScanSequential) continue;
            for (int c = 0; c < s.scan_components; c++) all &= !((s.comp[c].h > 1 && s.comp[c].hs > 1) || (s.comp[c].v > 1 && s.comp[c].vs > 1));
        }
        for (int c = 0; c < img.num_components; c++) all &= ((covered[c >> 6] >> (c & 63)) & 1ull) != 0;
        if (!all && !img.replay_skip) out_clear_.push_back({img.out_offset, img.out_bytes, img.planes_offset, img.planes_bytes});
        if (img.jobs.empty() && !img.replay_skip && (format_ == JPGPU_FMT_RGB_U8 || format_ == JPGPU_FMT_RGBA_U8))
            rgb_convert_.push_back({(uint32_t)(&img - images_.data()), img.out_offset, (uint64_t)img.width * img.height, img.num_components});
    }
    idct_class_begin_[0] = 0;
    const int xcds = getenv("JPGPU_XCD_MAP") ? atoi(getenv("JPGPU_XCD_MAP")) : 8;
    for (int c = 0; c < kNumIdctLayoutClasses; c++) {
        std::vector<IdctWork> &w = idct_work_by_class[c];
        xcd_interleave(w, xcds);
        idct_work.insert(idct_work.end(), w.begin(), w.end());
        idct_class_begin_[c + 1] = (int)idct_work.size();
    }
    n_idct_work_ = (int)idct_work.size();
    idct_later_begin_.assign(1, n_idct_work_);
    for (const std::vector<IdctWork> &w : idct_later_levels) {
        idct_work.insert(idct_work.end(), w.begin(), w.end());
        idct_later_begin_.push_back((int)idct_work.size());
    }
    if (!idct_partial.empty()) {
        idct_work.insert(idct_work.end(), idct_partial.begin(), idct_partial.end());
        idct_later_begin_.push_back((int)idct_work.size());
    }

    overlap_ok_ = false;
    std::vector<IdctWork> idct_work_split;
    {
        const char *ev = getenv("JPGPU_OVERLAP");
        const bool wanted = ev && atoi(ev) != 0 && dispose_jobs_.empty();
        uint32_t split_image = 0;
        uint64_t acc = 0;
        for (size_t ii = 0; ii < images_.size() && acc * 2 < total_blocks_; ii++) {
            acc += images_[ii].total_blocks;
            split_image = (uint32_t)ii + 1;
        }
        huff_split_ = 0;
        while (huff_split_ < n_huff_work_ && h_scans_[huff_work[huff_split_].scan].image_index < split_image) huff_split_++;
        if (wanted && !entropy_only_ && sub_work.empty() && prog_work.empty() && total_blocks_ >= (4u << 20) && huff_split_ > 0 &&
            huff_split_ < n_huff_work_ && rgb_convert_.empty() && format_ != JPGPU_FMT_EXTENDED_U16 && idct_later_begin_.size() == 1) {
            for (int half = 0; half < 2; half++) {
                idct_split_begin_[half][0] = (int)idct_work_split.size();
                for (int c = 0; c < kNumIdctLayoutClasses; c++) {
                    std::vector<IdctWork> w;
                    for (const IdctWork &x : idct_work_by_class[c])
                        if ((h_scans_[x.scan].image_index < split_image) == (half == 0)) w.push_back(x);
                    std::sort(w.begin(), w.end(), [](const IdctWork &a, const IdctWork &b) { return a.scan != b.scan ? a.scan < b.scan : a.first_mcu < b.first_mcu; });
                    xcd_interleave(w, xcds);
                    idct_work_split.insert(idct_work_split.end(), w.begin(), w.end());
                    idct_split_begin_[half][c + 1] = (int)idct_work_split.size();
                }
            }
            overlap_ok_ = true;
        }
    }
    decodes_since_query_ = 0;

    h_status_.assign(jobs_.size(), DevScanStatus());
    for (size_t j = 0; j < jobs_.size(); j++) {
        DevScanStatus &st = h_status_[j];
        memset(&st, 0, sizeof st);
        st.first_error = kNoError;
        st.decoded_mcus = h_scans_[j].total_mcus;
    }

    struct Up {
        DevBuffer *buf;
        const void *src;
        size_t bytes;
        size_t reserve;
    };
    const Up ups[] = {
        {&d_scans_, h_scans_.data(), h_scans_.size() * sizeof(DevScan), 0},
        {&d_status_, h_status_.data(), h_status_.size() * sizeof(DevScanStatus), 0},
        {&d_huff_pool_, huff_pool_.data(), huff_pool_.size() * sizeof(DevHuffTable), 0},
        {&d_quant_pool_, quant_pool_.data(), quant_pool_.size() * sizeof(DevQuantTable), 0},
        {&d_huff_work_, huff_work.data(), huff_work.size() * sizeof(HuffWork), 0},
        {&d_chunk_work_, chunk_work.data(), chunk_work.size() * sizeof(ChunkWork), 0},
        {&d_k1_order_, k1_order.data(), k1_order.size() * sizeof(ChunkWork), 16},
        {&d_sub_work_, sub_work.data(), sub_work.size() * sizeof(HuffWork), 0},
        {&d_sub_final_work_, sub_final_work.data(), sub_final_work.size() * sizeof(HuffWork), 0},
        {&d_prog_work_, prog_work.data(), prog_work.size() * sizeof(HuffWork), 0},
        {&d_prog_sync_, nullptr, 0, (size_t)(prog_work.empty() ? 0 : 256)},
        {&d_sub_scan_ids_, sub_scan_ids_.data(), sub_scan_ids_.size() * sizeof(uint32_t), 0},
        {&d_sub_exit_a_, nullptr, 0, (size_t)total_subs_ * sizeof(uint32_t) + 256},
        {&d_sub_exit_b_, nullptr, 0, (size_t)total_subs_ * sizeof(uint32_t) + 256},
        {&d_sub_nblk_, nullptr, 0, (size_t)total_subs_ * sizeof(uint32_t) + 256},
        {&d_sub_first_, nullptr, 0, (size_t)total_subs_ * sizeof(uint32_t) + 256},
        {&d_sub_entry_, nullptr, 0, (size_t)total_subs_ * sizeof(uint32_t) + 256},
        {&d_sub_dcsum_, nullptr, 0, (size_t)total_subs_ * 16 + 256},
        {&d_sub_dcentry_, nullptr, 0, (size_t)total_subs_ * 16 + 256},
        {&d_sub_changed_, nullptr, 0, kSubseqCtlWords * sizeof(uint32_t)},
        {&d_dispose_, dispose_jobs_.data(), dispose_jobs_.size() * sizeof(DisposeJob), 0},
        {&d_sub_same_, nullptr, 0, (size_t)total_subs_ * sizeof(uint32_t) + 256},
        {&d_sub_perm_, nullptr, 0, (size_t)total_subs_ * sizeof(uint32_t) + 256},
        {&d_lut_pool_, nullptr, 0, huff_pool_.size() * kLutPoolBytesPerTable},
        {&d_chunk_sums_, nullptr, 0, (size_t)total_chunks * sizeof(ChunkSum) + 256},
        {&d_k1_tickets_, nullptr, 0, 256},
        {&d_k2_tickets_, nullptr, 0, 256},
        {&d_sr_set_scan_, sr_set_scan.data(), sr_set_scan.size() * sizeof(uint32_t), 16},
        {&d_sr_luts_, nullptr, 0, sr_set_scan.size() * kSrLutSetBytes + 16},
        {&d_idct_work_, idct_work.data(), idct_work.size() * sizeof(IdctWork), 0},
        {&d_idct_work_split_, idct_work_split.data(), idct_work_split.size() * sizeof(IdctWork), 0},
        {&d_ends_, nullptr, 0, (size_t)total_ends_ * sizeof(uint32_t) + 256},
        {&d_ends_u_, nullptr, 0, (size_t)total_ends_ * sizeof(uint32_t) + 256},
        {&d_unstuffed_, nullptr, 0, (size_t)input_bytes_},
        {&d_coefs_, nullptr, 0, entropy_only_ ? 256 : (size_t)total_blocks_ * 128 + (size_t)kIdctBlocksPerWg * 128 + 256},
        {&d_out_, nullptr, 0, entropy_only_ ? 256 : (size_t)out_bytes_ + 256},
        {&d_rgb_scratch_, nullptr, 0, rgb_convert_.empty() ? 0 : (size_t)out_bytes_ + 256},
        {&d_planes_, nullptr, 0, format_ == JPGPU_FMT_EXTENDED_U16 && !entropy_only_ ? (size_t)planes_bytes_ + 256 : 0},
        {&d_input_, nullptr, 0, (size_t)input_bytes_},
    };
    for (const Up &u : ups) {
        e = u.buf->reserve(std::max(u.bytes, u.reserve));
        if (e != hipSuccess) return hip_fail(e, "hipMalloc");
        if (u.bytes) {
            e = hipMemcpyAsync(u.buf->ptr, u.src, u.bytes, hipMemcpyHostToDevice, up);
            if (e != hipSuccess) return hip_fail(e, "hipMemcpyAsync(descriptors)");
        }
    }
    e = hipMemsetAsync(d_k2_tickets_.ptr, 0, kK2MaxPools * sizeof(uint32_t), up);
    if (e != hipSuccess) return hip_fail(e, "hipMemsetAsync(K2 tickets)");
    {
        const size_t want = (size_t)total_chunks * kMarkerDescBytes + 256;
        if (want > d_k1_desc_.cap) {
            e = d_k1_desc_.reserve(want);
            if (e != hipSuccess) return hip_fail(e, "hipMalloc(K1 descriptors)");
            e = hipMemsetAsync(d_k1_desc_.ptr, 0, d_k1_desc_.cap, up);
            if (e != hipSuccess) return hip_fail(e, "hipMemsetAsync(K1 descriptors)");
        }
        e = hipMemsetAsync(d_k1_tickets_.ptr, 0, 2 * sizeof(uint32_t), up);
        if (e != hipSuccess) return hip_fail(e, "hipMemsetAsync(K1 tickets)");
        if (!h_k1_giveup_) {
            e = hipHostMalloc((void **)&h_k1_giveup_, 64, hipHostMallocMapped);
            if (e != hipSuccess) return hip_fail(e, "hipHostMalloc(K1 give-up word)");
        }
        *h_k1_giveup_ = 0;
        k1_epoch_ = 0;
        static const bool three_pass = getenv("JPGPU_K1_THREE_PASS") != nullptr;
        k1_onepass_ = !three_pass;
    }
    e = hipMemsetAsync(d_sub_changed_.ptr, 0, kSubseqCtlWords * sizeof(uint32_t), up);
    if (e != hipSuccess) return hip_fail(e, "hipMemsetAsync(K2S control)");
    e = launch_lut_pool(up, (const DevHuffTable *)d_huff_pool_.ptr, (int)huff_pool_.size(), (uint8_t *)d_lut_pool_.ptr);
    if (e != hipSuccess) return hip_fail(e, "lut_pool_kernel");
    e = launch_sr_luts(up, (const DevScan *)d_scans_.ptr, (const uint32_t *)d_sr_set_scan_.ptr, (int)sr_set_scan.size(), (const uint8_t *)d_lut_pool_.ptr,
                       (uint8_t *)d_sr_luts_.ptr);
    if (e != hipSuccess) return hip_fail(e, "sr_lut_build_kernel");
    if (!files_resident_) {
        e = hipMemsetAsync(d_input_.ptr, 0, 256, up);
        if (e != hipSuccess) return hip_fail(e, "hipMemsetAsync");
        for (size_t i = 0; i < images_.size(); i++) {
            const ImagePlan &img = images_[i];
            if (img.status != JPGPU_OK || img.jobs.empty() || !file_ptr[i] || file_len[i] == 0) continue;
            e = hipMemcpyAsync((uint8_t *)d_input_.ptr + img.file_offset, file_ptr[i], file_len[i], hipMemcpyHostToDevice, up);
            if (e != hipSuccess) return hip_fail(e, "hipMemcpyAsync(input)");
            const uint64_t tail = img.file_offset + file_len[i];
            if (align_up(tail, 256) > tail) {
                e = hipMemsetAsync((uint8_t *)d_input_.ptr + tail, 0, (size_t)(align_up(tail, 256) - tail), up);
                if (e != hipSuccess) return hip_fail(e, "hipMemsetAsync(tail)");
            }
        }
        e = hipMemsetAsync((uint8_t *)d_input_.ptr + input_bytes_ - 256, 0, 256, up);
        if (e != hipSuccess) return hip_fail(e, "hipMemsetAsync(slack)");
    }
    e = hipStreamSynchronize(up);
    if (e != hipSuccess) return hip_fail(e, "hipStreamSynchronize(upload)");
    work_in_flight_ = false;
    return JPGPU_OK;
}

}
```

jpeglibrary_amd/csrc/device_batch_result.cpp:

```cpp
#include "device_batch.h"

#include <hip/hip_runtime.h>
#include <stdio.h>
#include <stdlib.h>
#include <string.h>

#include <algorithm>
#include <atomic>
#include <chrono>
#include <thread>
#include <vector>

#include "kernels.h"

namespace jpgpu {

int DeviceBatch::fetch_status() {
    if (status_valid_) return JPGPU_OK;
    int rc = sync();
    if (rc != JPGPU_OK) return rc;
    if (!h_status_.empty()) {
        hipError_t e = hipMemcpy(h_status_.data(), d_status_.ptr, h_status_.size() * sizeof(DevScanStatus), hipMemcpyDeviceToHost);
        if (e != hipSuccess) return hip_fail(e, "hipMemcpy(status)");
    }
// ... 173 lines not shown

int DeviceBatch::redo_swallowed(int i, int job, jpgpu_image_result *res) {
    auto hit = redo_.find(i);
    if (hit == redo_.end()) {
        const ImagePlan &img = images_[(size_t)i];
        if (forced_swallow_.size() >= 64) {
            res->status = JPGPU_ERR_NOT_SUPPORTED;
            res->detail = kDetailUnsupportedFrame;
            ctx_->last_error = "More than 64 scans of one file leave a byte unread in front of their terminating markers.";
            return JPGPU_OK;
        }
        int ordinal = 0;
        for (int j : img.jobs) {
            if (j == job) break;
            ordinal += jobs_[j].kind == kScanSequential ? 1 : 0;
        }
        std::vector<uint8_t> file(img.file_len);
        hipError_t e = hipMemcpy(file.data(), (const uint8_t *)d_input_.ptr + img.file_offset, img.file_len, hipMemcpyDeviceToHost);
        if (e != hipSuccess) return hip_fail(e, "hipMemcpy(file of a re-planned image)");
        Redo r;
        memset(&r.res, 0, sizeof r.res);
        {
            DeviceBatch sub(ctx_);
            std::vector<int> forced = forced_swallow_;
            forced.push_back(ordinal);
            sub.set_forced_swallow(forced);
            const uint8_t *fptr = file.data();
            const size_t flen = file.size();
            int rc = sub.upload_files(&fptr, &flen, 1, format_);
            if (rc == JPGPU_OK) rc = sub.decode();
            if (rc == JPGPU_OK) rc = sub.result(0, &r.res);
            if (rc != JPGPU_OK) return rc;
            r.error = ctx_->last_error;
            const ImagePlan *si = sub.image(0);
            if (si && si->status == JPGPU_OK && si->out_bytes == img.out_bytes && img.out_bytes != 0) {
                e = hipMemcpy((uint8_t *)d_out_.ptr + img.out_offset, (const uint8_t *)sub.d_out_.ptr + si->out_offset, img.out_bytes, hipMemcpyDeviceToDevice);
                if (e != hipSuccess) return hip_fail(e, "hipMemcpy(output of a re-planned image)");
            } else if (si && si->status != JPGPU_OK) {
                r.res.status = si->status;
                r.res.detail = si->detail;
                r.error = si->error;
            }
        }
        hit = redo_.emplace(i, std::move(r)).first;
    }
    *res = hit->second.res;
    ctx_->last_error = hit->second.error;
    return JPGPU_OK;
}

int DeviceBatch::download_output(int i, void *dst, size_t cap) {
    const ImagePlan *img = image(i);
    if (!img || !dst) return fail(JPGPU_ERR_ARGUMENT, "jpgpu_batch_download_output: bad argument");
    if (img->status != JPGPU_OK) return fail(img->status, img->error);
    if (cap < img->out_bytes) return fail(JPGPU_ERR_ARGUMENT, "Destination buffer is too small.");
    if (img->jobs.size() > 1 && !entropy_only_ && redo_.find(i) == redo_.end()) {
        jpgpu_image_result tmp;
        const int rr = result(i, &tmp);
        if (rr != JPGPU_OK) return rr;
    }
    int rc = (replay_possible_ && !replay_done_) ? fetch_status() : sync();
    if (rc != JPGPU_OK) return rc;
    hipError_t e = hipMemcpy(dst, (const uint8_t *)d_out_.ptr + img->out_offset, img->out_bytes, hipMemcpyDeviceToHost);
    return e == hipSuccess ? JPGPU_OK : hip_fail(e, "hipMemcpy(output)");
}

int DeviceBatch::download_coefficients(int i, int16_t *dst, size_t cap_blocks) {
    const ImagePlan *img = image(i);
    if (!img || !dst) return fail(JPGPU_ERR_ARGUMENT, "jpgpu_batch_download_coefficients: bad argument");
    if (img->status != JPGPU_OK) return fail(img->status, img->error);
    if (cap_blocks < img->total_blocks) return fail(JPGPU_ERR_ARGUMENT, "Destination buffer is too small.");
    if (img->jobs.size() > 1 && !entropy_only_) {
        if (redo_.find(i) == redo_.end()) {
            jpgpu_image_result tmp;
            const int rr = result(i, &tmp);
            if (rr != JPGPU_OK) return rr;
        }
        if (redo_.find(i) != redo_.end())
            return fail(JPGPU_ERR_NOT_SUPPORTED, "The image's scans were planned again (a middle scan leaves one byte unread in front of its "
                                                 "terminating marker): its coefficients are not in the batch's store.");
    }
    int rc = (replay_possible_ && !replay_done_) ? fetch_status() : sync();
    if (rc != JPGPU_OK) return rc;
    hipError_t e = hipMemcpy(dst, (const int16_t *)d_coefs_.ptr + img->coef_offset * 64, img->total_blocks * 128, hipMemcpyDeviceToHost);
    return e == hipSuccess ? JPGPU_OK : hip_fail(e, "hipMemcpy(coefficients)");
}

int DeviceBatch::upload_coefficients(int i, const int16_t *src, size_t nblocks) {
    const ImagePlan *img = image(i);
    if (!img || !src) return fail(JPGPU_ERR_ARGUMENT, "jpgpu_batch_upload_coefficients: bad argument");
    if (img->status != JPGPU_OK) return fail(img->status, img->error);
    if (nblocks != img->total_blocks) return fail(JPGPU_ERR_ARGUMENT, "Block count does not match the image.");
    dispose_done_ = false;
    int rc = sync();
    if (rc != JPGPU_OK) return rc;
    hipError_t e = hipMemcpy((int16_t *)d_coefs_.ptr + img->coef_offset * 64, src, nblocks * 128, hipMemcpyHostToDevice);
    return e == hipSuccess ? JPGPU_OK : hip_fail(e, "hipMemcpy(coefficients)");
}

void DeviceBatch::plan_stats(jpgpu_plan_stats *st) const {
    memset(st, 0, sizeof *st);
    st->k2_plain_work = n_huff_work_;
    st->k2_pools = (int32_t)k2_pools_.size();
    for (const SubseqPool &p : k2_pools_) st->k2_pooled_chunks += p.count;
    st->huffman_waves = huffman_waves(k2_tab_bytes_);
    st->k2s_scans = n_sub_scans_;
    st->k2s_plain_work = n_sub_final_work_;
    st->k2s_pools = (int32_t)sub_pools_.size();
    st->k2s_table_sets = n_sr_sets_;
    st->k2s_subs_per_lane = sub_final_spl_;
}

void DeviceBatch::progressive_plan(jpgpu_progressive_plan *p) const {
    memset(p, 0, sizeof *p);
    p->scans = prog_scans_;
    p->levels = prog_begin_.empty() ? 0 : (int32_t)prog_begin_.size() - 1;
    p->max_deps = prog_max_deps_;
    p->pipelined = prog_scans_ > 0 && prog_pipelined_;
    p->chains_ok = prog_scans_ > 0 && prog_chains_ok_;
    p->pipe_waves = prog_pipe_count_;
    p->wave_tails = prog_wave_tails_;
    p->lane_work = prog_begin_.empty() ? 0 : prog_begin_.back();
    for (int x = 0; x < jpgpu_ctx::kProgChains; x++) p->chain_scans[x] = prog_chain_scans_[x];
    p->launch_form = prog_launch_form_;
}

void DeviceBatch::idct_work(int32_t counts[kNumIdctLayoutClasses]) const {
    for (int c = 0; c < kNumIdctLayoutClasses; c++) counts[c] = idct_class_begin_[c + 1] - idct_class_begin_[c];
}

void DeviceBatch::totals(uint64_t *compressed, uint64_t *blocks, uint64_t *pixels, uint64_t *out_bytes) const {
    if (compressed) *compressed = compressed_bytes_;
    if (blocks) *blocks = total_blocks_;
    if (pixels) *pixels = total_pixels_;
    if (out_bytes) {
        uint64_t s = 0;
        for (const ImagePlan &img : images_)
            if (img.status == JPGPU_OK && !img.jobs.empty()) s += img.out_bytes;
        *out_bytes = s;
    }
}

}
```

jpeglibrary_amd/csrc/k2_huffman.hip:

```cpp
#include <hip/hip_runtime.h>
#include <stdint.h>

#include <algorithm>
#include <atomic>
#include <cstdio>
#include <cstdlib>

#include "common.h"
#include "kernels.h"
#include "encode_kernels.h"
#include "kernels_device.h"

namespace jpgpu {


__global__ __launch_bounds__(256) void lut_pool_kernel(const DevHuffTable *__restrict__ pool, uint8_t *__restrict__ lut_pool) {
    const DevHuffTable &h = pool[blockIdx.x >> 1];
    const bool is_dc = (blockIdx.x & 1) != 0;
    uint8_t *tab = lut_pool + (size_t)(blockIdx.x >> 1) * kLutPoolBytesPerTable;
    uint8_t *img = tab + (is_dc ? kK2TabBytes : 0u);
    uint16_t *l1 = reinterpret_cast<uint16_t *>(img);
    uint16_t *l2 = reinterpret_cast<uint16_t *>(img + kK2L1Bytes);
    const uint32_t lb = is_dc ? kK2DcBits : kK2AcBits;
    uint8_t *img32 = tab + (is_dc ? kPoolNewDc : kPoolNewAc);
// ... 27 lines not shown
        const uint32_t t16 = lo > 65536u - kK2L2Entries ? lo : 65536u - kK2L2Entries;
        for (uint32_t j = threadIdx.x; j < kK2L2Entries; j += 256) f2[j] = t16 + j < 65536u ? (uint16_t)k2_entry_of(h, t16 + j, is_dc, 16) : (uint16_t)0;
        if (threadIdx.x < 4) reinterpret_cast<uint32_t *>(img32 + (4u << lb) + 2u * kK2L2Entries)[threadIdx.x] = threadIdx.x == 0 ? t16 : 0u;
        if (threadIdx.x < kK2SmallBytes / 16)
            reinterpret_cast<uint4 *>(img32 + (4u << lb) + 2u * kK2L2Entries + 16u)[threadIdx.x] =
                reinterpret_cast<const uint4 *>(reinterpret_cast<const uint8_t *>(&h) + offsetof(DevHuffTable, maxcode))[threadIdx.x];
    }
}

#ifdef JPGPU_K2_PROFILE
__device__ unsigned long long k2_prof[8];
#define K2_TICK() __builtin_readcyclecounter()
#define K2_PROF_ADD(i, v) do { if (lane == 0) atomicAdd(&k2_prof[i], (unsigned long long)(v)); } while (0)
extern "C" int jpgpu_debug_k2_profile(unsigned long long *out, int reset) {
    if (hipMemcpyFromSymbol(out, HIP_SYMBOL(k2_prof), sizeof(k2_prof)) != hipSuccess) return 1;
    if (reset) { unsigned long long z[8] = {}; if (hipMemcpyToSymbol(HIP_SYMBOL(k2_prof), z, sizeof z) != hipSuccess) return 1; }
    return 0;
}
#else
#define K2_TICK() 0ull
#define K2_PROF_ADD(i, v) do { (void)(v); } while (0)
#endif

__device__ __forceinline__ void k2_wave(const uint8_t *__restrict__ udata, const DevScan &s, uint32_t scan_index, uint32_t wave_first,
                                        const uint32_t *__restrict__ ends_u, DevScanStatus *__restrict__ status, int16_t *__restrict__ coefs,
                                        const uint8_t *tabs, const uint32_t *blk_info, uint8_t *stage, uint8_t *ring, uint32_t lane,
                                        unsigned long long k2_t0) {
    struct { uint32_t scan; } wk = {scan_index};
    const unsigned long long k2_t1 = K2_TICK();
    const DevScanStatus st = status[wk.scan];
    const uint32_t n_ends = st.n_ends;
    const uint32_t n_intervals = s.n_intervals;
    const uint32_t total_mcus = s.total_mcus;
    const uint32_t dri_eff = s.dri ? s.dri : total_mcus;
    const uint32_t bpm = s.blocks_per_mcu;
    const uint32_t interval = wave_first + lane;
    const bool active = interval < n_ends;
    const uint32_t *eu = ends_u + s.ends_off;
    const uint8_t *ubase = udata + s.data_off;

    uint32_t my_mcus = 0;
    bool closed_by_marker = false;
    uint32_t u0 = 0, u1 = 0;
    if (active) {
        u0 = interval == 0 ? 0u : eu[interval - 1] + 2u;
        u1 = eu[interval];
        my_mcus = (interval == n_intervals - 1) ? total_mcus - interval * dri_eff : dri_eff;
        closed_by_marker = !(interval == n_ends - 1 && st.terminator == 0);
    }
    const int32_t pm1_0 = (int32_t)((u0 & 3u) * 8u) - 1;
    const int32_t endpos = pm1_0 + 1 + (int32_t)((u1 - u0) * 8u);
    K2Feed feed;
    K2Pos pos;
    {
        const uint8_t *g = ubase + (u0 & ~3u);
        uint4 c0, c1, c2, c3;
        __builtin_memcpy(&c0, g, 16);
        __builtin_memcpy(&c1, g + 16, 16);
        __builtin_memcpy(&c2, g + 32, 16);
        __builtin_memcpy(&c3, g + 48, 16);
        __builtin_memcpy(&feed.nx, g + 64, 16);
        k2_ring_write(ring, 0, c0);
        k2_ring_write(ring, 1, c1);
        k2_ring_write(ring, 2, c2);
        k2_ring_write(ring, 3, c3);
        feed.wr = 4;
        feed.gp = g + 80;
        k2_pos_init(pos, ring, pm1_0);
    }
    uint32_t wave_mcus = 0;
    if (wave_first < n_ends) {
        wave_mcus = dri_eff;
        if (wave_first == n_intervals - 1) wave_mcus = total_mcus - wave_first * dri_eff;
    }

    int32_t pred0 = 0, pred1 = 0, pred2 = 0, pred3 = 0;
    uint32_t err = 0;
    const unsigned long long k2_t2 = K2_TICK();
    unsigned long long k2_dec = 0, k2_top = 0, k2_fl = 0;
    uint8_t *my_stage = stage + lane * 128;
    const uint32_t swz16 = ((lane >> 1) & 7u) << 4;

    const uint64_t coef_off = s.coef_off;

    for (uint32_t mcu = 0; mcu < wave_mcus; mcu++) {
        for (uint32_t b = 0; b < bpm; b++) {
            const uint32_t bi = __builtin_amdgcn_readfirstlane(blk_info[b]);
            const uint32_t ci = bi & 0xFFu;
            const K2Tab hdc = k2_tab_dc(tabs, bi);
            const K2Tab hac = k2_tab_ac(tabs, bi);
            const unsigned long long k2_a = K2_TICK();
            int32_t lim = k2_limit(endpos, feed.wr);
            if (active && err == 0 && mcu < my_mcus) {
                int32_t v, vb;
                uint32_t ia = 0, adv_b = 0;
                k2_symbol<true>(ring, feed, pos, endpos, lim, hdc, closed_by_marker, 0u, v, vb, ia, adv_b, err);
                const int32_t pred = ci == 0 ? pred0 : (ci == 1 ? pred1 : (ci == 2 ? pred2 : pred3));
                v += pred;
                if (ci == 0) pred0 = v;
                else if (ci == 1) pred1 = v;
                else if (ci == 2) pred2 = v;
                else pred3 = v;
                *reinterpret_cast<int16_t *>(my_stage + swz16) = (int16_t)v;
                uint32_t i2 = err == 0 ? 2u : 128u;
                while (i2 < 128u) {
                    k2_symbol<false>(ring, feed, pos, endpos, lim, hac, closed_by_marker, i2, v, vb, ia, adv_b, err);
                    const uint32_t at = ia - 2u < 126u ? ia - 2u : 126u;
                    *reinterpret_cast<int16_t *>(my_stage + (at ^ swz16)) = (int16_t)v;
                    i2 = ia + 2u * adv_b;
                    const uint32_t at_b = i2 - 2u < 126u ? i2 - 2u : 126u;
                    *reinterpret_cast<int16_t *>(my_stage + (at_b ^ swz16)) = (int16_t)vb;
                }
                if (err != 0)
                    atomicMax(&status[wk.scan].pad[1], fail_block_word(((uint64_t)interval * dri_eff + mcu) * bpm + b));
            }
            const unsigned long long k2_b = K2_TICK();
            k2_topup(ring, feed, pos.pm1);
            const unsigned long long k2_c = K2_TICK();
            __builtin_amdgcn_fence(__ATOMIC_RELEASE, "wavefront");
            __builtin_amdgcn_wave_barrier();
            __builtin_amdgcn_fence(__ATOMIC_ACQUIRE, "wavefront");
#pragma unroll
            for (int it = 0; it < 8; it++) {
                const uint32_t blk = it * 8 + (lane >> 3);
                const uint32_t chunk = lane & 7;
                uint4 *src = reinterpret_cast<uint4 *>(stage + blk * 128 + ((chunk ^ ((blk >> 1) & 7)) * 16));
                const uint4 v = *src;
                const uint4 z = {0, 0, 0, 0};
                *src = z;
                const uint32_t owner = wave_first + blk;
                if (owner < n_ends) {
                    const uint32_t owner_mcus = (owner == n_intervals - 1) ? total_mcus - owner * dri_eff : dri_eff;
                    if (mcu < owner_mcus) {
                        const uint64_t block_index = coef_off + ((uint64_t)owner * dri_eff + mcu) * bpm + b;
                        *reinterpret_cast<uint4 *>(coefs + block_index * 64 + chunk * 8) = v;
                    }
                }
            }
            __builtin_amdgcn_fence(__ATOMIC_RELEASE, "wavefront");
            __builtin_amdgcn_wave_barrier();
            __builtin_amdgcn_fence(__ATOMIC_ACQUIRE, "wavefront");
            const unsigned long long k2_d = K2_TICK();
            k2_dec += k2_b - k2_a;
            k2_top += k2_c - k2_b;
            k2_fl += k2_d - k2_c;
        }
    }
    K2_PROF_ADD(0, 1);
    K2_PROF_ADD(1, k2_t1 - k2_t0);
    K2_PROF_ADD(2, k2_t2 - k2_t1);
    K2_PROF_ADD(3, k2_dec);
    K2_PROF_ADD(4, k2_top);
    K2_PROF_ADD(5, k2_fl);
    K2_PROF_ADD(6, K2_TICK() - k2_t0);

    if (active) {
        int32_t rem = endpos - (pos.pm1 + 1);
        if (rem < 0) rem = 0;
        const uint32_t code = restart_check(s, st, &status[wk.scan], interval, n_ends, n_intervals, dri_eff, rem, err);
        if (code != kNoError) atomicMin(&status[wk.scan].first_error, code);
    }
}

template <int WAVES>
__global__ __launch_bounds__(64 * WAVES) void huffman_decode_kernel(const uint8_t *__restrict__ udata,
                                                                    const DevScan *__restrict__ scans,
                                                                    const HuffWork *__restrict__ work,
                                                                    const uint32_t *__restrict__ ends_u,
                                                                    DevScanStatus *__restrict__ status,
                                                                    const DevHuffTable *__restrict__ huff_pool,
                                                                    int16_t *__restrict__ coefs, int n_slots,
                                                                    const uint8_t *__restrict__ lut_pool, uint32_t tab_bytes) {
    extern __shared__ __attribute__((aligned(16))) uint8_t smem[];
    uint8_t *tabs = smem;
    uint8_t *wave_all = smem + tab_bytes;
    uint32_t *blk_info = reinterpret_cast<uint32_t *>(wave_all + WAVES * kK2WaveBytes);
    const HuffWork wk = work[blockIdx.x];
    const DevScan &s = scans[wk.scan];
    const uint32_t lane = threadIdx.x & 63, wave = threadIdx.x >> 6;
    const unsigned long long k2_t0 = K2_TICK();
    k2_stage_scan_tables(s, lut_pool, tabs, blk_info, n_slots, 64 * WAVES);
    uint8_t *stage = wave_all + wave * kK2WaveBytes;
    uint8_t *ring = stage + 8192 + lane * kK2RingStride;
    {
        const uint4 z = {0, 0, 0, 0};
#pragma unroll
        for (int i = 0; i < 8; i++) reinterpret_cast<uint4 *>(stage)[i * 64 + lane] = z;
    }
    __syncthreads();
    k2_wave(udata, s, wk.scan, wk.first_interval + wave * 64, ends_u, status, coefs, tabs, blk_info, stage, ring, lane, k2_t0);
}

template <int WAVES>
__global__ __launch_bounds__(64 * WAVES) void huffman_pool_kernel(const uint8_t *__restrict__ udata, const DevScan *__restrict__ scans,
                                                                  const HuffWork *__restrict__ work, uint32_t n_chunks,
                                                                  uint32_t *__restrict__ counter, uint32_t ticket_base,
                                                                  const uint32_t *__restrict__ ends_u, DevScanStatus *__restrict__ status,
                                                                  int16_t *__restrict__ coefs, int n_slots, const uint8_t *__restrict__ lut_pool,
                                                                  uint32_t tab_bytes) {
    extern __shared__ __attribute__((aligned(16))) uint8_t smem[];
    uint8_t *tabs = smem;
    uint8_t *wave_all = smem + tab_bytes;
    uint32_t *blk_info = reinterpret_cast<uint32_t *>(wave_all + WAVES * kK2WaveBytes);
    const uint32_t lane = threadIdx.x & 63, wave = threadIdx.x >> 6;
    const unsigned long long k2_t0 = K2_TICK();
    k2_stage_scan_tables(scans[work[0].scan], lut_pool, tabs, blk_info, n_slots, 64 * WAVES);
    uint8_t *stage = wave_all + wave * kK2WaveBytes;
    uint8_t *ring = stage + 8192 + lane * kK2RingStride;
    {
        const uint4 z = {0, 0, 0, 0};
#pragma unroll
        for (int i = 0; i < 8; i++) reinterpret_cast<uint4 *>(stage)[i * 64 + lane] = z;
    }
    __syncthreads();
#if !defined(JPGPU_K2_TICKET_AHEAD)
    for (;;) {
        uint32_t c = 0;
        if (lane == 0) c = atomicAdd(counter, 1u) - ticket_base;
        c = (uint32_t)__builtin_amdgcn_readfirstlane((int)c);
        if (c >= n_chunks) break;
// ... 84 lines not shown
```

jpeglibrary_amd/csrc/k3_idct.hip:

```cpp
#include <hip/hip_runtime.h>
#include <stdint.h>

#include <algorithm>
#include <atomic>
#include <cstdio>
#include <cstdlib>

#include "common.h"
#include "kernels.h"
#include "encode_kernels.h"
#include "kernels_device.h"

namespace jpgpu {


__device__ constexpr uint8_t kNat[64] = {0,  1,  8,  16, 9,  2,  3,  10, 17, 24, 32, 25, 18, 11, 4,  5,  12, 19, 26, 33, 40, 48,
                                         41, 34, 27, 20, 13, 6,  7,  14, 21, 28, 35, 42, 49, 56, 57, 50, 43, 36, 29, 22, 15, 23,
                                         30, 37, 44, 51, 58, 59, 52, 45, 38, 31, 39, 46, 53, 60, 61, 54, 47, 55, 62, 63};

#define JPGPU_IDCT8(y0, y1, y2, y3, y4, y5, y6, y7)                     \
    {                                                                   \
        float mz0 = y1 + y7;                                            \
        float mz2 = y3 + y7;                                            \
        float mz1 = y3 + y5;                                            \
        float mz3 = y1 + y5;                                            \
        float mz4 = (mz0 + mz1) * 1.175875602f;                         \
        mz2 = (mz2 * -1.961570560f) + mz4;                              \
        mz3 = (mz3 * -0.390180644f) + mz4;                              \
        mz0 = mz0 * -0.899976223f;                                      \
        mz1 = mz1 * -2.562915447f;                                      \
        const float mb3 = ((y7 * 0.298631336f) + mz0) + mz2;            \
        const float mb2 = ((y5 * 2.053119869f) + mz1) + mz3;            \
        const float mb1 = ((y3 * 3.072711026f) + mz1) + mz2;            \
        const float mb0 = ((y1 * 1.501321110f) + mz0) + mz3;            \
        mz4 = (y2 + y6) * 0.541196100f;                                 \
        mz0 = y0 + y4;                                                  \
        mz1 = y0 - y4;                                                  \
        mz2 = mz4 + (y6 * -1.847759065f);                               \
        mz3 = mz4 + (y2 * 0.765366865f);                                \
        const float a0 = mz0 + mz3;                                     \
        const float a3 = mz0 - mz3;                                     \
        const float a1 = mz1 + mz2;                                     \
        const float a2 = mz1 - mz2;                                     \
        y0 = a0 + mb0;                                                  \
        y7 = a0 - mb0;                                                  \
        y1 = a1 + mb1;                                                  \
        y6 = a1 - mb1;                                                  \
        y2 = a2 + mb2;                                                  \
        y5 = a2 - mb2;                                                  \
        y3 = a3 + mb3;                                                  \
        y4 = a3 - mb3;                                                  \
    }

__device__ __forceinline__ void block_dequant(const uint8_t *c_lds, uint32_t swz, const uint16_t *q_lds, float (&f)[64]) {
#pragma unroll
    for (int piece = 0; piece < 8; piece++) {
        const uint4 cv = *reinterpret_cast<const uint4 *>(c_lds + ((piece ^ swz) * 16));
        const uint4 qv = reinterpret_cast<const uint4 *>(q_lds)[piece];
        const uint32_t cw[4] = {cv.x, cv.y, cv.z, cv.w};
        const uint32_t qw[4] = {qv.x, qv.y, qv.z, qv.w};
#pragma unroll
        for (int j = 0; j < 8; j++) {
            const int k = piece * 8 + j;
            const uint32_t w = cw[j >> 1], q = qw[j >> 1];
            const int32_t c = (j & 1) ? ((int32_t)w >> 16) : (int32_t)(int16_t)(w & 0xFFFF);
            const int32_t qq = (j & 1) ? (int32_t)(q >> 16) : (int32_t)(q & 0xFFFF);
            f[kNat[k]] = (float)(qq * c);
        }
    }
}

typedef float float2v __attribute__((ext_vector_type(2)));
typedef short short2v __attribute__((ext_vector_type(2)));
typedef unsigned short ushort2v __attribute__((ext_vector_type(2)));

template <typename T>
__device__ __forceinline__ void idct8(T &y0, T &y1, T &y2, T &y3, T &y4, T &y5, T &y6, T &y7) {
    T mz0 = y1 + y7;
    T mz2 = y3 + y7;
    T mz1 = y3 + y5;
    T mz3 = y1 + y5;
    T mz4 = (mz0 + mz1) * 1.175875602f;
    mz2 = (mz2 * -1.961570560f) + mz4;
    mz3 = (mz3 * -0.390180644f) + mz4;
    mz0 = mz0 * -0.899976223f;
    mz1 = mz1 * -2.562915447f;
    const T mb3 = ((y7 * 0.298631336f) + mz0) + mz2;
    const T mb2 = ((y5 * 2.053119869f) + mz1) + mz3;
    const T mb1 = ((y3 * 3.072711026f) + mz1) + mz2;
    const T mb0 = ((y1 * 1.501321110f) + mz0) + mz3;
    mz4 = (y2 + y6) * 0.541196100f;
    mz0 = y0 + y4;
    mz1 = y0 - y4;
    mz2 = mz4 + (y6 * -1.847759065f);
    mz3 = mz4 + (y2 * 0.765366865f);
    const T a0 = mz0 + mz3;
    const T a3 = mz0 - mz3;
    const T a1 = mz1 + mz2;
    const T a2 = mz1 - mz2;
    y0 = a0 + mb0;
    y7 = a0 - mb0;
// ... 243 lines not shown
    constexpr uint32_t vshift = max_v >> 1;
    constexpr uint32_t kbpm = max_h * max_v + 2;
    const uint32_t n_tasks = rows_per_mcu * n_mcu;
    for (uint32_t t = tid; t < n_tasks; t += kIdctThreads) {
        const uint32_t row = t / n_mcu, m = t - row * n_mcu;
        const uint32_t gm = tile_first + m;
        const uint32_t gx = gm % s.mcus_per_line, gy = gm / s.mcus_per_line;
        const uint32_t y = gy * rows_per_mcu + row;
        if (y >= H) continue;
        const uint8_t *yrow = sh_px + (row & 7) * kPxRowStride + (m * kbpm + (row >> 3) * max_h) * 8;
        const uint8_t *crow = sh_px + (row >> vshift) * kPxRowStride + (m * kbpm + max_h * max_v) * 8;
        if (max_h == 2 && CONV != 0) {
            const uint4 yv = *reinterpret_cast<const uint4 *>(yrow);
            const uint4 cv = *reinterpret_cast<const uint4 *>(crow);
            uint32_t px[16];
#pragma unroll
            for (int j = 0; j < 8; j++) {
                const ChromaTerms t = chroma_terms(byte_of(cv.x, cv.y, j), byte_of(cv.z, cv.w, j), kf);
                px[2 * j] = rgb_pixel(byte_of(j < 4 ? yv.x : yv.z, j < 4 ? yv.y : yv.w, (2 * j) & 7), t);
                px[2 * j + 1] = rgb_pixel(byte_of(j < 4 ? yv.x : yv.z, j < 4 ? yv.y : yv.w, (2 * j + 1) & 7), t);
            }
            store_rgb_pixels<16, (CONV == 4 ? 4 : 3)>(img + ((size_t)y * W + gx * 16) * (CONV == 4 ? 4 : 3), px);
        } else if (CONV != 0) {
            const uint2 yv = *reinterpret_cast<const uint2 *>(yrow);
            const uint2 bv = *reinterpret_cast<const uint2 *>(crow);
            const uint2 rv = *reinterpret_cast<const uint2 *>(crow + 8);
            uint32_t px[8];
#pragma unroll
            for (int j = 0; j < 8; j++) px[j] = rgb_pixel(byte_of(yv.x, yv.y, j), chroma_terms(byte_of(bv.x, bv.y, j), byte_of(rv.x, rv.y, j), kf));
            store_rgb_pixels<8, (CONV == 4 ? 4 : 3)>(img + ((size_t)y * W + gx * 8) * (CONV == 4 ? 4 : 3), px);
        } else if (max_h == 2) {
            const uint4 yv = *reinterpret_cast<const uint4 *>(yrow);
            const uint4 cv = *reinterpret_cast<const uint4 *>(crow);
            const uint32_t cc0 = pick4(cv.x, cv.z, JPGPU_SEL(0, 4, 1, 5)), cc1 = pick4(cv.x, cv.z, JPGPU_SEL(2, 6, 3, 7));
            const uint32_t cc2 = pick4(cv.y, cv.w, JPGPU_SEL(0, 4, 1, 5)), cc3 = pick4(cv.y, cv.w, JPGPU_SEL(2, 6, 3, 7));
            uint4 o0, o1, o2;
            o0.x = pick4(yv.x, cc0, JPGPU_SEL(0, 4, 5, 1));
            o0.y = pick4(yv.x, cc0, JPGPU_SEL(4, 5, 2, 6));
            o0.z = pick4(yv.x, cc0, JPGPU_SEL(7, 3, 6, 7));
            o0.w = pick4(yv.y, cc1, JPGPU_SEL(0, 4, 5, 1));
            o1.x = pick4(yv.y, cc1, JPGPU_SEL(4, 5, 2, 6));
            o1.y = pick4(yv.y, cc1, JPGPU_SEL(7, 3, 6, 7));
            o1.z = pick4(yv.z, cc2, JPGPU_SEL(0, 4, 5, 1));
            o1.w = pick4(yv.z, cc2, JPGPU_SEL(4, 5, 2, 6));
            o2.x = pick4(yv.z, cc2, JPGPU_SEL(7, 3, 6, 7));
            o2.y = pick4(yv.w, cc3, JPGPU_SEL(0, 4, 5, 1));
            o2.z = pick4(yv.w, cc3, JPGPU_SEL(4, 5, 2, 6));
            o2.w = pick4(yv.w, cc3, JPGPU_SEL(7, 3, 6, 7));
            uint4 *dst = reinterpret_cast<uint4 *>(img + ((size_t)y * W + gx * 16) * 3);
            dst[0] = o0;
            dst[1] = o1;
            dst[2] = o2;
        } else {
            const uint2 yv = *reinterpret_cast<const uint2 *>(yrow);
            const uint2 bv = *reinterpret_cast<const uint2 *>(crow);
            const uint2 rv = *reinterpret_cast<const uint2 *>(crow + 8);
            uint2 o0, o1, o2;
            {
                const uint32_t lo = pick4(bv.x, rv.x, JPGPU_SEL(0, 4, 1, 5)), hi = pick4(bv.x, rv.x, JPGPU_SEL(2, 6, 3, 7));
                const uint32_t mid = pick4(lo, hi, JPGPU_SEL(2, 3, 4, 5));
                o0.x = pick4(yv.x, lo, JPGPU_SEL(0, 4, 5, 1));
                o0.y = pick4(yv.x, mid, JPGPU_SEL(4, 5, 2, 6));
                o1.x = pick4(yv.x, hi, JPGPU_SEL(5, 3, 6, 7));
            }
            {
                const uint32_t lo = pick4(bv.y, rv.y, JPGPU_SEL(0, 4, 1, 5)), hi = pick4(bv.y, rv.y, JPGPU_SEL(2, 6, 3, 7));
                const uint32_t mid = pick4(lo, hi, JPGPU_SEL(2, 3, 4, 5));
                o1.y = pick4(yv.y, lo, JPGPU_SEL(0, 4, 5, 1));
                o2.x = pick4(yv.y, mid, JPGPU_SEL(4, 5, 2, 6));
                o2.y = pick4(yv.y, hi, JPGPU_SEL(5, 3, 6, 7));
            }
            uint2 *dst = reinterpret_cast<uint2 *>(img + ((size_t)y * W + gx * 8) * 3);
            dst[0] = o0;
            dst[1] = o1;
            dst[2] = o2;
        }
    }
    }
}

typedef __attribute__((address_space(3))) void jpgpu_lds_void;
typedef const __attribute__((address_space(1))) void jpgpu_gbl_void;

template <int FMT, int LAY, bool PRE>
__device__ __forceinline__ void idct_output_body(
    const int16_t *__restrict__ coefs, const DevScan *__restrict__ scans, const IdctWork *__restrict__ work,
    const DevScanStatus *__restrict__ status, const DevQuantTable *__restrict__ quant_pool, uint8_t *__restrict__ out, YccRgbFactors kf) {
    constexpr int CONV = FMT == kFmtRgbU8 ? 3 : (FMT == kFmtRgbaU8 ? 4 : 0);
    constexpr bool kSampleBytes = fmt_is_sample_bytes(FMT);
    __shared__ __attribute__((aligned(16))) uint8_t sh_all[kIdctThreads * 128 + kIdctThreads * 64 + kMaxScanComponents * 128];
    uint8_t *sh = sh_all;
    uint8_t *sh_px = sh_all + kIdctThreads * 128;
    uint16_t(*sh_q)[64] = reinterpret_cast<uint16_t(*)[64]>(sh_all + kIdctThreads * 128 + kIdctThreads * 64);

    const IdctWork wk = work[blockIdx.x];
    const DevScan &s = scans[wk.scan];
    const uint32_t tid = threadIdx.x;
    const uint32_t wave = tid >> 6;
    const uint32_t bpm = s.blocks_per_mcu;
    const uint32_t mcus_per_tile = wk.mcus_per_tile;
    uint32_t decoded = status ? status[wk.scan].decoded_mcus : s.total_mcus;
    if (decoded > s.total_mcus) decoded = s.total_mcus;
    uint32_t fail_block = 0xFFFFFFFFu;
    if (status != nullptr && s.kind == kScanSequential) {
        const uint32_t fb = status[wk.scan].pad[1];
        if (fb != 0) fail_block = kFailBlockBase - fb;
        for (uint32_t j = s.first_scan; j < wk.scan; j++)
            if (scans[j].image_index == s.image_index && status[j].first_error != kNoError) fail_block = 0;
    }
    const bool keep = (s.shadow_mask & kKeepUnreachedMcus) != 0;
    constexpr bool kPerMcuLayout = fmt_is_interleaved(FMT) && (LAY == kLayYccH1V1 || LAY == kLayYccH2V1 || LAY == kLayYccH2V2);
    uint32_t first_mcu = wk.first_mcu;
    uint32_t range_end = wk.first_mcu + wk.n_mcus;
    if (first_mcu == kIdctPartialMcu) {
        if (fail_block == 0xFFFFFFFFu || fail_block % bpm == 0 || fail_block / bpm >= decoded) return;
        first_mcu = fail_block / bpm;
        range_end = first_mcu + 1;
    } else if (keep) {
        const uint32_t reach = kPerMcuLayout ? fail_block / bpm : (fail_block == 0xFFFFFFFFu ? fail_block : (fail_block + bpm - 1) / bpm);
        if (range_end > decoded) range_end = decoded;
        if (range_end > reach) range_end = reach;
        if (first_mcu >= range_end) return;
    }

    if (tid < (uint32_t)s.scan_components * 32) {
        const uint32_t c = tid >> 5, i = tid & 31;
        reinterpret_cast<uint32_t *>(sh_q[c])[i] =
            reinterpret_cast<const uint32_t *>(quant_pool[s.quant_pool[s.comp[c].quant_slot]].q)[i];
    }

    const uint32_t mcu_local = tid / bpm;
    const uint32_t b = tid - mcu_local * bpm;
    const uint32_t ci_early = s.blk_comp[b < kMaxBlocksPerMcu ? b : 0];
    const uint8_t *coef_bytes = reinterpret_cast<const uint8_t *>(coefs + s.coef_off * 64);

    auto tile_mcus = [&](uint32_t first) { return (range_end - first) < mcus_per_tile ? (range_end - first) : mcus_per_tile; };
    const uint32_t tile_blocks = mcus_per_tile * bpm;
    auto dma_tile = [&](uint32_t tile_first) {
        uint32_t t_ = tid;
        asm volatile("" : "+v"(t_));
        const uint32_t dma_lane_off = (t_ >> 3) * 128 + (((t_ & 7) ^ ((t_ >> 4) & 7)) * 16);
        const uint8_t *src = coef_bytes + (uint64_t)tile_first * bpm * 128;
#pragma unroll
        for (int k = 0; k < 8; k++)
            if (k < 6 || (uint32_t)k * 32 + (tid >> 3) < tile_blocks)
                __builtin_amdgcn_global_load_lds((jpgpu_gbl_void *)(src + (uint32_t)(k * 4096) + dma_lane_off),
                                                 (jpgpu_lds_void *)(sh + ((uint32_t)k * kIdctThreads + wave * 64) * 16), 16, 0, 0);
    };

    dma_tile(first_mcu);
    asm volatile("s_waitcnt vmcnt(0)" ::: "memory");
    __syncthreads();

  for (uint32_t tile_first = first_mcu; tile_first < range_end; tile_first += mcus_per_tile) {
    const uint32_t n_mcu = tile_mcus(tile_first);
    const uint32_t n_blk = n_mcu * bpm;
    const uint32_t next_first = tile_first + mcus_per_tile;
    const bool have_next = next_first < range_end;

    const uint32_t mcu = tile_first + mcu_local;
    const bool have_block = tid < n_blk;
    bool writes = have_block && ((s.shadow_mask >> ci_early) & 1u) == 0;

    float f[64];
    uint32_t px[32];
    if (PRE) {
        if (have_block) {
#pragma unroll
            for (int piece = 0; piece < 8; piece++) {
                const uint4 cv = *reinterpret_cast<const uint4 *>(sh + tid * 128 + ((piece ^ ((tid >> 1) & 7)) * 16));
                px[piece * 4] = cv.x;
                px[piece * 4 + 1] = cv.y;
                px[piece * 4 + 2] = cv.z;
                px[piece * 4 + 3] = cv.w;
            }
        }
    } else {
        constexpr bool kPerTile = (FMT == kFmtRgbU8 && (LAY == kLayYccH2V1 || LAY == kLayYccH2V2)) || (kSampleBytes && LAY == kLayGeneric);
        uint32_t t_ = tid;
        if (kPerTile) asm volatile("" : "+v"(t_));
        if (have_block) block_dequant(sh + t_ * 128, (t_ >> 1) & 7, sh_q[ci_early], f);
    }
    asm volatile("s_waitcnt lgkmcnt(0)" ::: "memory");
    __builtin_amdgcn_s_barrier();
    if (have_next) dma_tile(next_first);

    if (!PRE && have_block) block_idct(f, (int32_t)s.level_shift, px);
    const bool reached = mcu < decoded && mcu * bpm + b < fail_block;
    if ((s.shadow_mask & 0xFu) == 0) {
        writes = writes && (reached || !keep);
    } else {
        const uint32_t bb = b < kMaxBlocksPerMcu ? b : 0u, me = s.blk_comp[bb], fc = s.comp[me & 3u].component_index;
        uint32_t later = 0xFFu, earlier = 0xFFu;
        for (uint32_t cc = 0; cc < s.scan_components && cc < (uint32_t)kMaxScanComponents; cc++) {
            if (cc == me || s.comp[cc].component_index != fc) continue;
            if (cc > me && later == 0xFFu) later = cc;
            if (cc < me) earlier = cc;
        }
        uint32_t first_me = 0xFFu, first_later = 0xFFu, first_earlier = 0xFFu;
        for (uint32_t k = 0; k < bpm && k < (uint32_t)kMaxBlocksPerMcu; k++) {
            const uint32_t ck = s.blk_comp[k];
            if (ck == me && first_me == 0xFFu) first_me = k;
            if (ck == later && first_later == 0xFFu) first_later = k;
            if (ck == earlier && first_earlier == 0xFFu) first_earlier = k;
        }
        const bool later_reached = later != 0xFFu && mcu < decoded && mcu * bpm + (b - first_me + first_later) < fail_block;
        const bool earlier_reached = earlier != 0xFFu && mcu < decoded && mcu * bpm + (b - first_me + first_earlier) < fail_block;
        writes = have_block && (reached ? !later_reached : (!keep && later == 0xFFu && !earlier_reached));
    }
    if (!reached) {
#pragma unroll
        for (int i = 0; i < 32; i++) px[i] = 0;
    }
    bool synced = false;
    uint32_t mcu_late = mcu, b_late = b;
    asm volatile("" : "+v"(mcu_late), "+v"(b_late));
    const uint32_t mcu_y = mcu_late / s.mcus_per_line, mcu_x = mcu_late - mcu_y * s.mcus_per_line;
    const uint32_t ci = s.blk_comp[b_late < kMaxBlocksPerMcu ? b_late : 0];
    const DevScanComponent comp = s.comp[ci];

    if (FMT == kFmtPlanarI16) {
        if (writes) {
            int16_t *plane = reinterpret_cast<int16_t *>(out + s.out_off + s.plane_off[ci]);
            const uint32_t pitch = s.plane_pitch[ci];
            const uint32_t x0 = (mcu_x * comp.h + s.blk_x[b]) * 8, y0 = (mcu_y * comp.v + s.blk_y[b]) * 8;
#pragma unroll
            for (int r = 0; r < 8; r++) {
                const uint4 v = {px[r * 4 + 0], px[r * 4 + 1], px[r * 4 + 2], px[r * 4 + 3]};
                *reinterpret_cast<uint4 *>(plane + (size_t)(y0 + r) * pitch + x0) = v;
            }
        }
    } else {
    uint2 rows[8];
    if constexpr (FMT == kFmtInterleavedU8Scaled) {
        const ScaleTo8 k8 = scale_to_8(s.precision);
        if (k8.expand) {
#pragma unroll
            for (int r = 0; r < 8; r++) {
                rows[r].x = __builtin_amdgcn_perm(expand2_u8(px[r * 4 + 1], k8), expand2_u8(px[r * 4 + 0], k8), 0x06040200u);
                rows[r].y = __builtin_amdgcn_perm(expand2_u8(px[r * 4 + 3], k8), expand2_u8(px[r * 4 + 2], k8), 0x06040200u);
            }
        } else {
#pragma unroll
            for (int r = 0; r < 8; r++) {
                rows[r].x = __builtin_amdgcn_perm(shift_sat2_u8(px[r * 4 + 1], k8), shift_sat2_u8(px[r * 4 + 0], k8), 0x05040100u);
                rows[r].y = __builtin_amdgcn_perm(shift_sat2_u8(px[r * 4 + 3], k8), shift_sat2_u8(px[r * 4 + 2], k8), 0x05040100u);
            }
        }
    } else {
#pragma unroll
    for (int r = 0; r < 8; r++) {
        rows[r].x = pack4_u8(px[r * 4 + 0], px[r * 4 + 1]);
        rows[r].y = pack4_u8(px[r * 4 + 2], px[r * 4 + 3]);
    }
    }

    if (CONV != 0 && LAY == kLayGray) {
        if (writes) {
            const uint32_t x0 = (mcu_x * comp.h + s.blk_x[b]) * 8, y0 = (mcu_y * comp.v + s.blk_y[b]) * 8;
#pragma unroll
            for (int r = 0; r < 8; r++) {
                if (y0 + r >= s.height) continue;
                uint32_t px[8];
#pragma unroll
                for (int j = 0; j < 8; j++) px[j] = byte_of(rows[r].x, rows[r].y, j) * 0x010101u;
                store_rgb_pixels<8, (CONV == 4 ? 4 : 3)>(out + s.out_off + ((size_t)(y0 + r) * s.width + x0) * (CONV == 4 ? 4 : 3), px);
            }
        }
    } else if (FMT == kFmtPlanarU8 || (kSampleBytes && LAY == kLayGray)) {
        if (writes) {
            const bool gray = kSampleBytes;
            uint8_t *plane = out + s.out_off + (gray ? 0 : s.plane_off[ci]);
            const uint32_t pitch = gray ? s.width : s.plane_pitch[ci];
            const uint32_t x0 = (mcu_x * comp.h + s.blk_x[b]) * 8, y0 = (mcu_y * comp.v + s.blk_y[b]) * 8;
#pragma unroll
            for (int r = 0; r < 8; r++)
                if (!gray || y0 + r < s.height) *reinterpret_cast<uint2 *>(plane + (size_t)(y0 + r) * pitch + x0) = rows[r];
        }
    } else {
    if (have_block) {
#pragma unroll
        for (int r = 0; r < 8; r++) *reinterpret_cast<uint2 *>(sh_px + r * kPxRowStride + tid * 8) = rows[r];
    }
    asm volatile("s_waitcnt vmcnt(0)\n\ts_waitcnt lgkmcnt(0)" ::: "memory");
    __builtin_amdgcn_s_barrier();
    synced = true;

    interleaved_output_from_tile<LAY, CONV>(sh_px, s, tile_first, n_mcu, tid, writes, comp, mcu_x, mcu_y, b, out, kf, reached, mcu, fail_block);
    }
    }

    if (!synced) {
        asm volatile("s_waitcnt vmcnt(0)\n\ts_waitcnt lgkmcnt(0)" ::: "memory");
        __builtin_amdgcn_s_barrier();
    }
  }
}


hipError_t launch_extend_u16(hipStream_t stream, const uint8_t *planes, uint8_t *out_base, const ExtendPlanes *images, int n_images,
                             uint32_t max_pixels) {
    if (n_images <= 0 || max_pixels == 0) return hipSuccess;
    const uint32_t bx = (uint32_t)std::min<uint64_t>(((uint64_t)max_pixels + 255) / 256, 4096);
    for (int base = 0; base < n_images; base += 65535) {
        const int n = n_images - base < 65535 ? n_images - base : 65535;
        hipLaunchKernelGGL(extend_u16_kernel, dim3(bx, (uint32_t)n), dim3(256), 0, stream, planes, out_base, images + base);
    }
    return hipGetLastError();
}


template <int FMT, int LAY>
__global__ __launch_bounds__(kIdctThreads, (FMT == kFmtPlanarI16 ? 2 : 3)) void idct_output_kernel(
    const int16_t *__restrict__ coefs, const DevScan *__restrict__ scans, const IdctWork *__restrict__ work,
    const DevScanStatus *__restrict__ status, const DevQuantTable *__restrict__ quant_pool, uint8_t *__restrict__ out, YccRgbFactors kf) {
    idct_output_body<FMT, LAY, false>(coefs, scans, work, status, quant_pool, out, kf);
}
template <int FMT>
__global__ __launch_bounds__(kIdctThreads, 2) void flush_output_kernel(
    const int16_t *__restrict__ coefs, const DevScan *__restrict__ scans, const IdctWork *__restrict__ work,
    const DevScanStatus *__restrict__ status, const DevQuantTable *__restrict__ quant_pool, uint8_t *__restrict__ out, YccRgbFactors kf) {
    idct_output_body<FMT, kLayGeneric, true>(coefs, scans, work, status, quant_pool, out, kf);
}

__global__ __launch_bounds__(64) void dispose_pass_kernel(int16_t *__restrict__ coefs, const DisposeJob *__restrict__ jobs,
                                                          const DevQuantTable *__restrict__ quant_pool) {
    const DisposeJob &j = jobs[blockIdx.y];
    const uint32_t g = blockIdx.x * 64u + threadIdx.x;
    if (g >= j.n_blocks) return;
    const uint32_t c = j.blk_comp[g % j.bpm];
    const uint32_t n = j.n[c];
    if (n == 0) return;
    int16_t *blk = coefs + (j.coef_off + g) * 64;
    uint32_t w[32];
#pragma unroll
    for (int i = 0; i < 8; i++) {
        const uint4 v = reinterpret_cast<const uint4 *>(blk)[i];
        w[i * 4] = v.x;
        w[i * 4 + 1] = v.y;
        w[i * 4 + 2] = v.z;
        w[i * 4 + 3] = v.w;
    }
    for (uint32_t t = 0; t < n; t++) {
        const uint16_t *q = quant_pool[j.quant[c][t]].q;
        float f[64];
#pragma unroll
        for (int k = 0; k < 64; k++) {
            const int32_t cv = (k & 1) ? ((int32_t)w[k >> 1] >> 16) : (int32_t)(int16_t)(w[k >> 1] & 0xFFFFu);
            f[kNat[k]] = (float)((int32_t)q[k] * cv);
        }
        block_idct(f, (int32_t)j.level_shift, w);
    }
#pragma unroll
    for (int i = 0; i < 8; i++) reinterpret_cast<uint4 *>(blk)[i] = make_uint4(w[i * 4], w[i * 4 + 1], w[i * 4 + 2], w[i * 4 + 3]);
}

template <int FMT, int LAY>
static void launch_idct_one(hipStream_t stream, const int16_t *coefs, const DevScan *scans, const IdctWork *work, int n_work,
                            const DevScanStatus *status, const DevQuantTable *quant_pool, uint8_t *out,
                            YccRgbFactors kf = YccRgbFactors{0, 0, 0, 0}) {
    hipLaunchKernelGGL((idct_output_kernel<FMT, LAY>), dim3(n_work), dim3(kIdctThreads), 0, stream, coefs, scans, work, status,
                       quant_pool, out, kf);
}

hipError_t launch_idct(hipStream_t stream, const int16_t *coefs, const DevScan *scans, const IdctWork *work,
                       const int class_begin[kNumIdctLayoutClasses + 1], const DevScanStatus *status,
                       const DevQuantTable *quant_pool, uint8_t *out, int format, const YccRgbFactors &kf, uint8_t *generic_out) {
    for (int c = 0; c < kNumIdctLayoutClasses; c++) {
        const int n = class_begin[c + 1] - class_begin[c];
        if (n <= 0) continue;
        const IdctWork *w = work + class_begin[c];
        if (c == kIdctClassStoreHoldsSamples) {
            if (format == kFmtPlanarI16) hipLaunchKernelGGL((flush_output_kernel<kFmtPlanarI16>), dim3(n), dim3(kIdctThreads), 0, stream, coefs, scans, w, status, quant_pool, out, kf);
            else if (format == kFmtPlanarU8) hipLaunchKernelGGL((flush_output_kernel<kFmtPlanarU8>), dim3(n), dim3(kIdctThreads), 0, stream, coefs, scans, w, status, quant_pool, out, kf);
            else if (format == kFmtInterleavedU8Scaled) hipLaunchKernelGGL((flush_output_kernel<kFmtInterleavedU8Scaled>), dim3(n), dim3(kIdctThreads), 0, stream, coefs, scans, w, status, quant_pool, out, kf);
            else hipLaunchKernelGGL((flush_output_kernel<kFmtInterleavedU8>), dim3(n), dim3(kIdctThreads), 0, stream, coefs, scans, w, status, quant_pool,
                                    (format == kFmtRgbU8 || format == kFmtRgbaU8) ? generic_out : out, kf);
        } else if (format == kFmtPlanarI16) {
            launch_idct_one<kFmtPlanarI16, kLayGeneric>(stream, coefs, scans, w, n, status, quant_pool, out);
        } else if (format == kFmtPlanarU8) {
            launch_idct_one<kFmtPlanarU8, kLayGeneric>(stream, coefs, scans, w, n, status, quant_pool, out);
        } else if (format == kFmtRgbU8) {
            switch (c) {
            case kLayYccH1V1: launch_idct_one<kFmtRgbU8, kLayYccH1V1>(stream, coefs, scans, w, n, status, quant_pool, out, kf); break;
            case kLayYccH2V1: launch_idct_one<kFmtRgbU8, kLayYccH2V1>(stream, coefs, scans, w, n, status, quant_pool, out, kf); break;
            case kLayYccH2V2: launch_idct_one<kFmtRgbU8, kLayYccH2V2>(stream, coefs, scans, w, n, status, quant_pool, out, kf); break;
            case kLayGray: launch_idct_one<kFmtRgbU8, kLayGray>(stream, coefs, scans, w, n, status, quant_pool, out, kf); break;
            default: launch_idct_one<kFmtInterleavedU8, kLayGeneric>(stream, coefs, scans, w, n, status, quant_pool, generic_out); break;
            }
        } else if (format == kFmtRgbaU8) {
            switch (c) {
            case kLayYccH1V1: launch_idct_one<kFmtRgbaU8, kLayYccH1V1>(stream, coefs, scans, w, n, status, quant_pool, out, kf); break;
            case kLayYccH2V1: launch_idct_one<kFmtRgbaU8, kLayYccH2V1>(stream, coefs, scans, w, n, status, quant_pool, out, kf); break;
            case kLayYccH2V2: launch_idct_one<kFmtRgbaU8, kLayYccH2V2>(stream, coefs, scans, w, n, status, quant_pool, out, kf); break;
            case kLayGray: launch_idct_one<kFmtRgbaU8, kLayGray>(stream, coefs, scans, w, n, status, quant_pool, out, kf); break;
            default: launch_idct_one<kFmtInterleavedU8, kLayGeneric>(stream, coefs, scans, w, n, status, quant_pool, generic_out); break;
            }
        } else if (format == kFmtInterleavedU8Scaled) {
            switch (c) {
            case kLayYccH1V1: launch_idct_one<kFmtInterleavedU8Scaled, kLayYccH1V1>(stream, coefs, scans, w, n, status, quant_pool, out); break;
            case kLayYccH2V1: launch_idct_one<kFmtInterleavedU8Scaled, kLayYccH2V1>(stream, coefs, scans, w, n, status, quant_pool, out); break;
            case kLayYccH2V2: launch_idct_one<kFmtInterleavedU8Scaled, kLayYccH2V2>(stream, coefs, scans, w, n, status, quant_pool, out); break;
            case kLayGray: launch_idct_one<kFmtInterleavedU8Scaled, kLayGray>(stream, coefs, scans, w, n, status, quant_pool, out); break;
            default: launch_idct_one<kFmtInterleavedU8Scaled, kLayGeneric>(stream, coefs, scans, w, n, status, quant_pool, out); break;
            }
        } else {
            switch (c) {
            case kLayYccH1V1: launch_idct_one<kFmtInterleavedU8, kLayYccH1V1>(stream, coefs, scans, w, n, status, quant_pool, out); break;
            case kLayYccH2V1: launch_idct_one<kFmtInterleavedU8, kLayYccH2V1>(stream, coefs, scans, w, n, status, quant_pool, out); break;
            case kLayYccH2V2: launch_idct_one<kFmtInterleavedU8, kLayYccH2V2>(stream, coefs, scans, w, n, status, quant_pool, out); break;
            case kLayGray: launch_idct_one<kFmtInterleavedU8, kLayGray>(stream, coefs, scans, w, n, status, quant_pool, out); break;
            default: launch_idct_one<kFmtInterleavedU8, kLayGeneric>(stream, coefs, scans, w, n, status, quant_pool, out); break;
            }
        }
        const hipError_t e = hipGetLastError();
        if (e != hipSuccess) return e;
    }
    return hipSuccess;
}

hipError_t launch_ycc_to_rgb(hipStream_t stream, const uint8_t *src, uint8_t *dst, uint64_t n_pixels, int comps, int bpp, const YccRgbFactors &kf) {
    if (n_pixels == 0) return hipSuccess;
    const uint64_t want = (n_pixels + 255) / 256;
    const int grid = (int)(want < 65536 ? want : 65536);
    hipLaunchKernelGGL(ycc_to_rgb_kernel, dim3(grid), dim3(256), 0, stream, src, dst, n_pixels, comps, bpp, kf);
    return hipGetLastError();
}


hipError_t launch_dispose_pass(hipStream_t stream, int16_t *coefs, const DisposeJob *jobs, int n_jobs, uint32_t max_blocks, const DevQuantTable *quant_pool) {
    if (n_jobs <= 0 || max_blocks == 0) return hipSuccess;
    hipLaunchKernelGGL(dispose_pass_kernel, dim3((max_blocks + 63u) / 64u, n_jobs), dim3(64), 0, stream, coefs, jobs, quant_pool);
    return hipGetLastError();
}

int idct_layout_class(const DevScan &s) {
    const uint32_t W = s.width;
    if (s.frame_components == 1 && s.scan_components == 1 && s.comp[0].h == 1 && s.comp[0].v == 1 && (W % 8) == 0 && (s.out_off % 8) == 0)
        return kLayGray;
    const bool ycc = s.frame_components == 3 && s.scan_components == 3 && s.comp[0].component_index == 0 &&
                     s.comp[1].component_index == 1 && s.comp[2].component_index == 2 && s.comp[0].hs == 1 && s.comp[0].vs == 1 &&
                     s.comp[1].h == 1 && s.comp[1].v == 1 && s.comp[2].h == 1 && s.comp[2].v == 1;
    if (!ycc) return kLayGeneric;
    if (s.max_h == 1 && s.max_v == 1 && (W % 8) == 0 && (s.out_off % 8) == 0) return kLayYccH1V1;
    if (s.max_h == 2 && (W % 16) == 0 && (s.out_off % 16) == 0) {
        if (s.max_v == 1) return kLayYccH2V1;
        if (s.max_v == 2) return kLayYccH2V2;
    }
    return kLayGeneric;
}

}
```

jpeglibrary_amd/csrc/kernels.h:

```cpp
#pragma once
#include <hip/hip_runtime_api.h>
#include <stddef.h>
#include <stdint.h>

#include "common.h"

namespace jpgpu {

constexpr int kHuffWaves = 11;
constexpr uint32_t kK2AcTabBytes = 8192 + 512 + 16 + 320, kK2DcTabBytes = 2048 + 512 + 16 + 320, kK2WaveLdsBytes = 8192 + 64 * 68;
constexpr uint32_t kK2LdsBudget = 160 * 1024 - 64;
inline uint32_t k2_scan_tab_bytes(const DevScan &s) {
    uint32_t bytes = 0;
    for (int sl = 0; sl < kMaxHuffSlots; sl++) {
        if (s.huff_pool[sl] == 0xFFFF) continue;
        bool is_dc = false;
        for (int c = 0; c < s.scan_components; c++) is_dc |= s.comp[c].dc_slot == sl;
        bytes += is_dc ? kK2DcTabBytes : kK2AcTabBytes;
    }
    return bytes;
}
constexpr int huffman_waves(uint32_t tab_bytes) {
    return (int)((kK2LdsBudget - tab_bytes) / kK2WaveLdsBytes) < kHuffWaves ? (int)((kK2LdsBudget - tab_bytes) / kK2WaveLdsBytes) : kHuffWaves;
}
constexpr int kIdctBlocksPerWg = 256;
constexpr int kIdctTilesPerWg = 16;


constexpr uint32_t kMarkerChunkBytes = 4096;
constexpr uint32_t kMarkerChunksPerWg = 1;
hipError_t launch_marker_index(hipStream_t stream, const uint8_t *data, const DevScan *scans, int n_scans, const ChunkWork *work,
                               int n_chunks, ChunkSum *sums, uint32_t *ends, DevScanStatus *status, uint8_t *udata, uint32_t *ends_u);
constexpr size_t kMarkerDescBytes = 64;
#ifndef JPGPU_K1_GROUP
#define JPGPU_K1_GROUP 4
#endif
constexpr uint32_t kMarkerGroupChunks = JPGPU_K1_GROUP;
hipError_t launch_marker_onepass(hipStream_t stream, const uint8_t *data, const DevScan *scans, const ChunkWork *order, int n_groups,
                                 void *desc, uint32_t *tickets, uint32_t epoch, uint32_t tag, uint32_t spin_budget,
                                 uint32_t *host_giveup, uint32_t *ends, DevScanStatus *status, uint8_t *udata, uint32_t *ends_u);
hipError_t launch_huffman(hipStream_t stream, const uint8_t *data, const DevScan *scans, const HuffWork *work, int n_work,
                          const uint32_t *ends, DevScanStatus *status, const DevHuffTable *huff_pool, int16_t *coefs,
                          int n_slots, const uint8_t *lut_pool, uint32_t tab_bytes);
constexpr int kK2MaxPools = 8;
hipError_t launch_huffman_pool(hipStream_t stream, const uint8_t *data, const DevScan *scans, const HuffWork *work, int n_chunks, uint32_t *counter,
                               uint32_t ticket_base, int groups, const uint32_t *ends, DevScanStatus *status, int16_t *coefs, int n_slots,
                               const uint8_t *lut_pool, uint32_t tab_bytes);
hipError_t launch_lut_pool(hipStream_t stream, const DevHuffTable *huff_pool, int n_tables, uint8_t *lut_pool);
constexpr int kNumIdctLayoutClasses = 6;
constexpr int kIdctClassStoreHoldsSamples = 5;
int idct_layout_class(const DevScan &s);
hipError_t launch_idct(hipStream_t stream, const int16_t *coefs, const DevScan *scans, const IdctWork *work,
                       const int class_begin[kNumIdctLayoutClasses + 1], const DevScanStatus *status,
                       const DevQuantTable *quant_pool, uint8_t *out, int format, const YccRgbFactors &kf, uint8_t *generic_out);
hipError_t launch_dispose_pass(hipStream_t stream, int16_t *coefs, const DisposeJob *jobs, int n_jobs, uint32_t max_blocks, const DevQuantTable *quant_pool);
hipError_t launch_ycc_to_rgb(hipStream_t stream, const uint8_t *src, uint8_t *dst, uint64_t n_pixels, int comps, int bpp, const YccRgbFactors &kf);

constexpr int kSubFinalPoolWaves = 11, kSubFinalPoolMinChunks = 40, kSubFinalMaxPools = 8;
constexpr int kSubseqCtlPoolCounter = 72;
struct SubseqPool {
    int first, count;
};
constexpr uint32_t kSubseqBits = 1024;
hipError_t launch_subseq_decode(hipStream_t stream, const uint8_t *udata, const DevScan *scans, const HuffWork *work, int n_work,
                                const uint32_t *scan_ids, int n_scans, const uint32_t *ends_u, DevScanStatus *status,
                                const DevHuffTable *huff_pool, uint32_t *exit_a, uint32_t *exit_b, uint32_t *nblk, uint32_t *first_block,
                                uint32_t *entry_used, void *dcsum, void *dc_entry, uint32_t *changed_dev, int16_t *coefs, int n_slots,
                                int max_rounds, int *rounds_used, const uint8_t *lut_pool, const HuffWork *final_work, int n_final_work,
                                uint32_t *same_dist, bool *same_valid, int device_rounds, const HuffWork *gather_work, int n_gather,
                                const HuffWork *pool_work, const SubseqPool *pools, int n_pools, int num_cus, uint32_t *lane_perm, int subs_per_lane,
                                uint32_t tab_bytes, const uint8_t *sr_luts);
#ifndef JPGPU_SR_LB
#define JPGPU_SR_LB 10
#endif
constexpr int kSrLutBits = JPGPU_SR_LB;
constexpr size_t kSrLutSetBytes = (size_t)kMaxHuffSlots << (kSrLutBits + 2);
hipError_t launch_sr_luts(hipStream_t stream, const DevScan *scans, const uint32_t *set_scan, int n_sets, const uint8_t *lut_pool, uint8_t *sr_luts);
constexpr uint64_t kSubFinalFewSubs = 1u << 20;
constexpr uint32_t kSubseqGatherSpan = 1024;
constexpr int kSubseqCtlWords = 128, kSubseqCtlSameDone = 96, kSubseqFirstBudget = 16;
constexpr int kSubseqMaxDeviceRounds = 61;
#ifndef JPGPU_SF_WAVES
#define JPGPU_SF_WAVES 4
#endif
constexpr int subseq_final_waves() { return JPGPU_SF_WAVES; }
constexpr uint32_t kSfWaveLdsBytes = kK2WaveLdsBytes;
constexpr bool subseq_pool_fits(uint32_t tab_bytes) { return tab_bytes + (uint32_t)kSubFinalPoolWaves * kSfWaveLdsBytes <= kK2LdsBudget; }
#ifndef JPGPU_SF_SUBS
#define JPGPU_SF_SUBS 2
#endif
constexpr int kSubFinalSubsPerLane = JPGPU_SF_SUBS;
constexpr size_t kLutPoolBytesPerTable = 2 * (4096 + 512 + 16 + 320) + (8192 + 512 + 16 + 320) + (2048 + 512 + 16 + 320);

hipError_t launch_progressive(hipStream_t stream, const uint8_t *udata, const DevScan *scans, const HuffWork *work, int n_work,
                              const uint32_t *ends_u, DevScanStatus *status, const DevHuffTable *huff_pool, int16_t *coefs, int n_slots);
hipError_t launch_progressive_streams(hipStream_t stream, const uint8_t *udata, const DevScan *scans, const HuffWork *work, int n_work,
                                      const uint32_t *ends_u, DevScanStatus *status, const DevHuffTable *huff_pool, int16_t *coefs,
                                      int n_slots, int pipelined, uint32_t spin_budget, uint32_t *started);
size_t progressive_stream_lds_bytes(int n_slots);
int progressive_stream_blocks_per_cu(int n_slots);

hipError_t launch_extend_u16(hipStream_t stream, const uint8_t *planes, uint8_t *out_base, const ExtendPlanes *images, int n_images,
                             uint32_t max_pixels);

hipError_t launch_gather_pinned(hipStream_t stream, const GatherPiece *pieces, int n_pieces, uint8_t *dst);
hipError_t launch_first_marker(hipStream_t stream, const uint8_t *data, const void *segs, const uint32_t *seg_hi, int n_segs,
                               uint32_t max_len, uint32_t *first);

struct EncHuffTable;
hipError_t launch_transcode(hipStream_t stream, int mode, const uint8_t *udata, const uint8_t *input, const DevScan *scans,
                            const HuffWork *work, int n_work, const uint32_t *ends_u, const uint32_t *ends_raw, DevScanStatus *status,
                            const DevHuffTable *huff_pool, uint32_t *hist, const EncHuffTable *enc, uint32_t *sizes,
                            const uint64_t *offsets, uint8_t *out, int n_slots);
hipError_t launch_transcode_offsets(hipStream_t stream, const DevScan *scans, const uint32_t *scan_ids, int n_scans, const uint32_t *sizes,
                                    const uint64_t *base, uint64_t *offsets, uint64_t *totals);
hipError_t launch_subseq_sync(hipStream_t stream, const uint8_t *udata, const DevScan *scans, const HuffWork *work, int n_work,
                              const uint32_t *scan_ids, int n_scans, const uint32_t *ends_u, DevScanStatus *status,
                              const DevHuffTable *huff_pool, uint32_t *exit_a, uint32_t *exit_b, uint32_t *nblk, uint32_t *first_block,
                              uint32_t *entry_used, void *dcsum, void *dc_entry, uint32_t *changed_dev, int n_slots, int max_rounds,
                              int *rounds_used, const uint8_t *lut_pool, const uint32_t **final_state_out, uint32_t *same_dist, bool *same_valid,
                              int device_rounds, const HuffWork *gather_work, int n_gather, const uint8_t *sr_luts);
hipError_t launch_subseq_transcode(hipStream_t stream, int mode, const uint8_t *udata, const DevScan *scans, const HuffWork *work, int n_work,
                                   const uint32_t *ends_u, DevScanStatus *status, const DevHuffTable *huff_pool, const uint32_t *exit_state,
                                   const uint32_t *first_block, uint32_t *hist, const EncHuffTable *enc, uint32_t *sub_bits,
                                   const uint64_t *sub_bitoff, const uint64_t *scan_raw_off, uint8_t *raw, int n_slots);
hipError_t launch_subseq_bit_offsets(hipStream_t stream, const DevScan *scans, const uint32_t *scan_ids, int n_scans, const uint32_t *sub_bits,
                                     uint64_t *bitoff, uint64_t *totals);
}
```

Measured before the change: 552,800 Mpixels/s.

## Add split hand-off coefficient layout between Huffman and IDCT for restart scans

Adds a split coefficient store layout for sequential restart-interval scans. Huffman output for paired intervals is interleaved into a compact region with per-block flag words, and the IDCT kernel reads it through a separate split work list. The goal is to cut coefficient memory traffic and store footprint between the entropy and IDCT stages. Coefficient export and upload now need an extra expand kernel to rebuild a dense copy, and the change adds complexity plus an env-var opt-out.

```diff
diff --git a/jpeglibrary_amd/csrc/capi.cpp b/jpeglibrary_amd/csrc/capi.cpp
--- a/jpeglibrary_amd/csrc/capi.cpp
+++ b/jpeglibrary_amd/csrc/capi.cpp
@@ -417,7 +417,9 @@
 
 int jpgpu_batch_result(jpgpu_batch *b, int i, jpgpu_image_result *res) { JPGPU_GUARD(b, b->impl.result(i, res)); }
 void *jpgpu_batch_output_device(const jpgpu_batch *b, uint64_t *total_bytes) { return b ? b->impl.output_device(total_bytes) : nullptr; }
-void *jpgpu_batch_coefficients_device(const jpgpu_batch *b, uint64_t *total_blocks) { return b ? b->impl.coefs_device(total_blocks) : nullptr; }
+void *jpgpu_batch_coefficients_device(const jpgpu_batch *b, uint64_t *total_blocks) {
+    return b ? const_cast<jpgpu_batch *>(b)->impl.coefs_device(total_blocks) : nullptr;
+}
 int jpgpu_batch_download_output(jpgpu_batch *b, int i, void *dst, size_t cap) { JPGPU_GUARD(b, b->impl.download_output(i, dst, cap)); }
 int jpgpu_batch_download_coefficients(jpgpu_batch *b, int i, int16_t *dst, size_t cap_blocks) {
     JPGPU_GUARD(b, b->impl.download_coefficients(i, dst, cap_blocks));
diff --git a/jpeglibrary_amd/csrc/common.h b/jpeglibrary_amd/csrc/common.h
--- a/jpeglibrary_amd/csrc/common.h
+++ b/jpeglibrary_amd/csrc/common.h
@@ -90,6 +90,24 @@
 constexpr uint32_t kFailBlockBase = 0xFFFFFFFFu;
 constexpr uint32_t kIdctPartialMcu = 0xFFFFFFFFu;
 constexpr uint64_t kScanStoreHoldsSamples = 1;
+constexpr uint64_t kScanSplitHandoff = 2;
+constexpr int kSplitFlagShift = 8;
+constexpr uint64_t kSplitMaxBytesPerBlock = 8;
+constexpr uint64_t kSplitZeroWords = 16;
+#if defined(__HIPCC__) || defined(__CUDACC__)
+#define JPGPU_HD __host__ __device__
+#else
+#define JPGPU_HD
+#endif
+JPGPU_HD inline uint64_t split_plane_lines(uint32_t n_intervals, uint32_t dri, uint32_t bpm) { return (uint64_t)((n_intervals + 1) / 2) * dri * bpm; }
+JPGPU_HD inline uint64_t split_region_blocks(uint32_t n_intervals, uint32_t dri, uint32_t bpm) { return 2 * split_plane_lines(n_intervals, dri, bpm); }
+JPGPU_HD inline uint64_t split_flag_words(uint32_t n_intervals, uint32_t dri, uint32_t bpm) { return (uint64_t)((n_intervals + 63) / 64) * dri * bpm; }
+JPGPU_HD inline uint64_t split_slot(uint32_t i, uint32_t m, uint32_t b, uint32_t dri, uint32_t bpm) {
+    return ((((uint64_t)(i >> 1) * dri + m) * bpm + b) << 1) | (i & 1u);
+}
+JPGPU_HD inline uint64_t split_flag_word(uint32_t i, uint32_t m, uint32_t b, uint32_t dri, uint32_t bpm) {
+    return ((uint64_t)(i >> 6) * dri + m) * bpm + b;
+}
 struct alignas(16) DisposeJob {
     uint64_t coef_off;
     uint32_t n_blocks;
diff --git a/jpeglibrary_amd/csrc/device_batch.cpp b/jpeglibrary_amd/csrc/device_batch.cpp
--- a/jpeglibrary_amd/csrc/device_batch.cpp
+++ b/jpeglibrary_amd/csrc/device_batch.cpp
@@ -39,7 +39,7 @@
 
 DeviceBatch::~DeviceBatch() {
     if (ctx_) (void)hipSetDevice(ctx_->device);
-    for (DevBuffer *b : {&d_sub_work_, &d_sub_final_work_, &d_sub_scan_ids_, &d_sub_exit_a_, &d_sub_exit_b_, &d_sub_nblk_, &d_sub_first_, &d_sub_entry_, &d_sub_dcsum_, &d_sub_dcentry_, &d_sub_changed_, &d_sub_same_, &d_sub_perm_, &d_k1_desc_, &d_k1_tickets_, &d_k2_tickets_, &d_sr_luts_, &d_sr_set_scan_, &d_k1_order_, &d_prog_snapshot_, &d_dispose_, &d_verify_, &d_lut_pool_, &d_prog_work_, &d_prog_sync_, &d_planes_, &d_extend_desc_, &d_gather_, &d_rgb_scratch_, &d_chunk_work_, &d_chunk_sums_, &d_unstuffed_, &d_ends_u_, &d_input_, &d_scans_, &d_status_, &d_ends_, &d_huff_pool_, &d_quant_pool_, &d_huff_work_, &d_idct_work_, &d_idct_work_split_, &d_coefs_, &d_out_})
+    for (DevBuffer *b : {&d_sub_work_, &d_sub_final_work_, &d_sub_scan_ids_, &d_sub_exit_a_, &d_sub_exit_b_, &d_sub_nblk_, &d_sub_first_, &d_sub_entry_, &d_sub_dcsum_, &d_sub_dcentry_, &d_sub_changed_, &d_sub_same_, &d_sub_perm_, &d_k1_desc_, &d_k1_tickets_, &d_k2_tickets_, &d_sr_luts_, &d_sr_set_scan_, &d_k1_order_, &d_prog_snapshot_, &d_dense_, &d_split_ids_, &d_dispose_, &d_verify_, &d_lut_pool_, &d_prog_work_, &d_prog_sync_, &d_planes_, &d_extend_desc_, &d_gather_, &d_rgb_scratch_, &d_chunk_work_, &d_chunk_sums_, &d_unstuffed_, &d_ends_u_, &d_input_, &d_scans_, &d_status_, &d_ends_, &d_huff_pool_, &d_quant_pool_, &d_huff_work_, &d_idct_work_, &d_idct_work_split_, &d_coefs_, &d_out_})
         b->release();
     for (hipEvent_t &e : ev_pool_)
         if (e) (void)hipEventDestroy(e);
diff --git a/jpeglibrary_amd/csrc/device_batch.h b/jpeglibrary_amd/csrc/device_batch.h
--- a/jpeglibrary_amd/csrc/device_batch.h
+++ b/jpeglibrary_amd/csrc/device_batch.h
@@ -118,10 +118,7 @@
         if (total) *total = out_bytes_;
         return d_out_.ptr;
     }
-    void *coefs_device(uint64_t *total_blocks) const {
-        if (total_blocks) *total_blocks = total_blocks_;
-        return d_coefs_.ptr;
-    }
+    void *coefs_device(uint64_t *total_blocks);
     int download_output(int i, void *dst, size_t cap);
     int download_coefficients(int i, int16_t *dst, size_t cap_blocks);
     int upload_coefficients(int i, const int16_t *src, size_t nblocks);
@@ -200,6 +197,14 @@
     int n_huff_work_ = 0, n_idct_work_ = 0;
     int idct_class_begin_[kNumIdctLayoutClasses + 1] = {};
     std::vector<int> idct_later_begin_;
+    std::vector<uint32_t> split_scans_;
+    uint32_t split_max_blocks_ = 0;
+    uint64_t coef_store_blocks_ = 0;
+    int idct_split_begin_class_[kNumIdctLayoutClasses] = {};
+    bool dense_valid_ = false, dense_override_ = false;
+    DevBuffer d_dense_, d_split_ids_;
+    int dense_coefs(const int16_t **ptr);
+    int make_store_dense();
     uint64_t total_blocks_ = 0, out_bytes_ = 0, planes_bytes_ = 0, input_bytes_ = 0, compressed_bytes_ = 0, total_pixels_ = 0;
     DevBuffer d_planes_;
     DevBuffer d_extend_desc_;
diff --git a/jpeglibrary_amd/csrc/device_batch_launch.cpp b/jpeglibrary_amd/csrc/device_batch_launch.cpp
--- a/jpeglibrary_amd/csrc/device_batch_launch.cpp
+++ b/jpeglibrary_amd/csrc/device_batch_launch.cpp
@@ -40,6 +40,7 @@
     status_valid_ = false;
     redo_.clear();
     dispose_done_ = false;
+    dense_valid_ = false;
     hipError_t e = launch_huffman(ctx_->stream, (const uint8_t *)d_unstuffed_.ptr, (const DevScan *)d_scans_.ptr, (const HuffWork *)d_huff_work_.ptr,
                                   n_huff_work_, (const uint32_t *)d_ends_u_.ptr, (DevScanStatus *)d_status_.ptr,
                                   (const DevHuffTable *)d_huff_pool_.ptr, (int16_t *)d_coefs_.ptr, n_huff_slots_, (const uint8_t *)d_lut_pool_.ptr, k2_tab_bytes_);
@@ -225,7 +226,7 @@
     hipError_t e = launch_idct(ctx_->stream, (const int16_t *)d_coefs_.ptr, (const DevScan *)d_scans_.ptr, (const IdctWork *)d_idct_work_.ptr,
                                idct_class_begin_, (const DevScanStatus *)d_status_.ptr, (const DevQuantTable *)d_quant_pool_.ptr,
                                extended ? (uint8_t *)d_planes_.ptr : (uint8_t *)d_out_.ptr, extended ? (int)JPGPU_FMT_PLANAR_I16 : format_, kf,
-                               (uint8_t *)d_rgb_scratch_.ptr);
+                               (uint8_t *)d_rgb_scratch_.ptr, split_scans_.empty() || dense_override_ ? nullptr : idct_split_begin_class_);
     if (e != hipSuccess) return hip_fail(e, "idct_output_kernel");
     for (size_t lv = 0; lv + 1 < idct_later_begin_.size(); lv++) {
         int cb[kNumIdctLayoutClasses + 1];
diff --git a/jpeglibrary_amd/csrc/device_batch_layout.cpp b/jpeglibrary_amd/csrc/device_batch_layout.cpp
--- a/jpeglibrary_amd/csrc/device_batch_layout.cpp
+++ b/jpeglibrary_amd/csrc/device_batch_layout.cpp
@@ -114,6 +114,14 @@
     dispose_max_blocks_ = 0;
     std::vector<IdctWork> idct_work;
     std::vector<IdctWork> idct_work_by_class[kNumIdctLayoutClasses];
+    std::vector<IdctWork> idct_split_by_class[kNumIdctLayoutClasses];
+    split_scans_.clear();
+    split_max_blocks_ = 0;
+    dense_valid_ = dense_override_ = false;
+    const char *split_env = getenv("JPGPU_DENSE_HANDOFF");
+    const bool split_wanted = !(split_env && atoi(split_env) != 0) && !entropy_only_ && !keep_canvas_;
+    const bool split_always = split_env != nullptr;
+    uint64_t real_blocks = 0, flag_words = 0;
     std::vector<std::vector<IdctWork>> idct_later_levels;
     std::vector<IdctWork> idct_partial;
     std::vector<int> scan_level(jobs_.size(), 0);
@@ -323,6 +331,7 @@
             const uint64_t nblocks = (uint64_t)s.mcus_per_line * s.mcus_per_column * s.blocks_per_mcu;
             if (job.kind == kScanFrameOnly && !img.replay_skip) prog_clear_.push_back({coef_off, nblocks});
             coef_off += nblocks;
+            real_blocks += nblocks;
             img.total_blocks += nblocks;
             compressed_bytes_ += s.data_len;
             bool null_table = false;
@@ -342,6 +351,17 @@
                 }
             } else {
                 for (uint32_t first = 0; first < s.n_intervals && !img.replay_skip; first += huff_intervals_per_wg) huff_work.push_back({(uint32_t)j, first});
+                const int k3_class = fmt_is_interleaved(format_) ? idct_layout_class(s) : 0;
+                if (split_wanted && job.kind == kScanSequential && s.dri != 0 && img.jobs.size() == 1 && !img.replay_skip && s.total_mcus > 0 &&
+                    s.blocks_per_mcu != 0 && idct_split_supported(format_, k3_class) &&
+                    (split_always || (uint64_t)s.data_len <= nblocks * kSplitMaxBytesPerBlock)) {
+                    flag_words = (flag_words + kSplitZeroWords - 1) / kSplitZeroWords * kSplitZeroWords + kSplitZeroWords;
+                    s.reserved0 |= kScanSplitHandoff | (flag_words << kSplitFlagShift);
+                    flag_words += split_flag_words(s.n_intervals, s.dri, s.blocks_per_mcu);
+                    coef_off += split_region_blocks(s.n_intervals, s.dri, s.blocks_per_mcu) - nblocks;
+                    split_scans_.push_back((uint32_t)j);
+                    split_max_blocks_ = std::max<uint32_t>(split_max_blocks_, (uint32_t)nblocks);
+                }
             }
             if (img.replay_skip) continue;
             if (s.blocks_per_mcu == 0) continue;
@@ -394,8 +414,9 @@
                     if (!listed) rgb_convert_.push_back({(uint32_t)ii, img.out_offset, (uint64_t)img.width * img.height, img.num_components});
                 }
             } else {
+                std::vector<IdctWork> &list = (s.reserved0 & kScanSplitHandoff) ? idct_split_by_class[cls] : idct_work_by_class[cls];
                 for (uint32_t first = 0; first < s.total_mcus; first += run)
-                    idct_work_by_class[cls].push_back({(uint32_t)j, first, std::min(run, s.total_mcus - first), mcus_per_wg});
+                    list.push_back({(uint32_t)j, first, std::min(run, s.total_mcus - first), mcus_per_wg});
                 if (keep_canvas_ && job.kind == kScanSequential && fmt_is_sample_bytes(format_) &&
                     cls >= 1 && cls <= 3)
                     idct_partial.push_back({(uint32_t)j, kIdctPartialMcu, 1, ((uint32_t)kIdctBlocksPerWg / s.blocks_per_mcu)});
@@ -408,7 +429,9 @@
         dj.n_blocks = fs.total_mcus * (uint32_t)fs.blocks_per_mcu;
         dispose_max_blocks_ = std::max(dispose_max_blocks_, dj.n_blocks);
     }
-    total_blocks_ = coef_off;
+    total_blocks_ = real_blocks;
+    coef_store_blocks_ = coef_off;
+    for (uint32_t j : split_scans_) h_scans_[j].reserved0 += ((coef_store_blocks_ + (uint64_t)kIdctBlocksPerWg) * 16) << kSplitFlagShift;
     out_bytes_ = out_off;
     planes_bytes_ = planes_off;
     total_ends_ = ends_off;
@@ -581,6 +604,10 @@
         std::vector<IdctWork> &w = idct_work_by_class[c];
         xcd_interleave(w, xcds);
         idct_work.insert(idct_work.end(), w.begin(), w.end());
+        idct_split_begin_class_[c] = (int)idct_work.size();
+        std::vector<IdctWork> &ws = idct_split_by_class[c];
+        xcd_interleave(ws, xcds);
+        idct_work.insert(idct_work.end(), ws.begin(), ws.end());
         idct_class_begin_[c + 1] = (int)idct_work.size();
     }
     n_idct_work_ = (int)idct_work.size();
@@ -598,7 +625,7 @@
     std::vector<IdctWork> idct_work_split;
     {
         const char *ev = getenv("JPGPU_OVERLAP");
-        const bool wanted = ev && atoi(ev) != 0 && dispose_jobs_.empty();
+        const bool wanted = ev && atoi(ev) != 0 && dispose_jobs_.empty() && split_scans_.empty();
         uint32_t split_image = 0;
         uint64_t acc = 0;
         for (size_t ii = 0; ii < images_.size() && acc * 2 < total_blocks_; ii++) {
@@ -675,7 +702,8 @@
         {&d_ends_, nullptr, 0, (size_t)total_ends_ * sizeof(uint32_t) + 256},
         {&d_ends_u_, nullptr, 0, (size_t)total_ends_ * sizeof(uint32_t) + 256},
         {&d_unstuffed_, nullptr, 0, (size_t)input_bytes_},
-        {&d_coefs_, nullptr, 0, entropy_only_ ? 256 : (size_t)total_blocks_ * 128 + (size_t)kIdctBlocksPerWg * 128 + 256},
+        {&d_split_ids_, split_scans_.data(), split_scans_.size() * sizeof(uint32_t), 16},
+        {&d_coefs_, nullptr, 0, entropy_only_ ? 256 : (size_t)coef_store_blocks_ * 128 + (size_t)kIdctBlocksPerWg * 128 + (size_t)flag_words * 8 + 256},
         {&d_out_, nullptr, 0, entropy_only_ ? 256 : (size_t)out_bytes_ + 256},
         {&d_rgb_scratch_, nullptr, 0, rgb_convert_.empty() ? 0 : (size_t)out_bytes_ + 256},
         {&d_planes_, nullptr, 0, format_ == JPGPU_FMT_EXTENDED_U16 && !entropy_only_ ? (size_t)planes_bytes_ + 256 : 0},
@@ -688,6 +716,10 @@
             e = hipMemcpyAsync(u.buf->ptr, u.src, u.bytes, hipMemcpyHostToDevice, up);
             if (e != hipSuccess) return hip_fail(e, "hipMemcpyAsync(descriptors)");
         }
+    }
+    if (!split_scans_.empty()) {
+        e = hipMemsetAsync((uint8_t *)d_coefs_.ptr + ((size_t)coef_store_blocks_ + (size_t)kIdctBlocksPerWg) * 128, 0, (size_t)flag_words * 8, up);
+        if (e != hipSuccess) return hip_fail(e, "hipMemsetAsync(hand-off flags)");
     }
     e = hipMemsetAsync(d_k2_tickets_.ptr, 0, kK2MaxPools * sizeof(uint32_t), up);
     if (e != hipSuccess) return hip_fail(e, "hipMemsetAsync(K2 tickets)");
diff --git a/jpeglibrary_amd/csrc/device_batch_result.cpp b/jpeglibrary_amd/csrc/device_batch_result.cpp
--- a/jpeglibrary_amd/csrc/device_batch_result.cpp
+++ b/jpeglibrary_amd/csrc/device_batch_result.cpp
@@ -279,8 +279,50 @@
     }
     int rc = (replay_possible_ && !replay_done_) ? fetch_status() : sync();
     if (rc != JPGPU_OK) return rc;
-    hipError_t e = hipMemcpy(dst, (const int16_t *)d_coefs_.ptr + img->coef_offset * 64, img->total_blocks * 128, hipMemcpyDeviceToHost);
+    const int16_t *coefs = nullptr;
+    if ((rc = dense_coefs(&coefs)) != JPGPU_OK) return rc;
+    hipError_t e = hipMemcpy(dst, coefs + img->coef_offset * 64, img->total_blocks * 128, hipMemcpyDeviceToHost);
     return e == hipSuccess ? JPGPU_OK : hip_fail(e, "hipMemcpy(coefficients)");
+}
+
+int DeviceBatch::dense_coefs(const int16_t **ptr) {
+    *ptr = (const int16_t *)d_coefs_.ptr;
+    if (split_scans_.empty() || dense_override_ || !d_coefs_.ptr) return JPGPU_OK;
+    if (!dense_valid_) {
+        const size_t bytes = (size_t)coef_store_blocks_ * 128;
+        hipError_t e = d_dense_.reserve(bytes + (size_t)kIdctBlocksPerWg * 128 + 256);
+        if (e != hipSuccess) return hip_fail(e, "hipMalloc(dense coefficients)");
+        e = hipMemcpyAsync(d_dense_.ptr, d_coefs_.ptr, bytes, hipMemcpyDeviceToDevice, ctx_->stream);
+        if (e != hipSuccess) return hip_fail(e, "hipMemcpyAsync(dense coefficients)");
+        e = launch_expand_handoff(ctx_->stream, (const int16_t *)d_coefs_.ptr, (int16_t *)d_dense_.ptr, (const DevScan *)d_scans_.ptr,
+                                  (const uint32_t *)d_split_ids_.ptr, (int)split_scans_.size(), split_max_blocks_);
+        if (e != hipSuccess) return hip_fail(e, "expand_handoff_kernel");
+        e = hipStreamSynchronize(ctx_->stream);
+        if (e != hipSuccess) return hip_fail(e, "hipStreamSynchronize(dense coefficients)");
+        dense_valid_ = true;
+    }
+    *ptr = (const int16_t *)d_dense_.ptr;
+    return JPGPU_OK;
+}
+
+int DeviceBatch::make_store_dense() {
+    if (split_scans_.empty() || dense_override_) return JPGPU_OK;
+    const int16_t *coefs = nullptr;
+    const int rc = dense_coefs(&coefs);
+    if (rc != JPGPU_OK) return rc;
+    std::swap(d_coefs_, d_dense_);
+    for (uint32_t j : split_scans_) h_scans_[j].reserved0 &= kScanStoreHoldsSamples;
+    hipError_t e = hipMemcpy(d_scans_.ptr, h_scans_.data(), h_scans_.size() * sizeof(DevScan), hipMemcpyHostToDevice);
+    if (e != hipSuccess) return hip_fail(e, "hipMemcpy(scan descriptors)");
+    dense_override_ = true;
+    return JPGPU_OK;
+}
+
+void *DeviceBatch::coefs_device(uint64_t *total_blocks) {
+    if (total_blocks) *total_blocks = coef_store_blocks_;
+    const int16_t *coefs = (const int16_t *)d_coefs_.ptr;
+    if (!split_scans_.empty() && !dense_override_ && (sync() != JPGPU_OK || dense_coefs(&coefs) != JPGPU_OK)) return nullptr;
+    return (void *)coefs;
 }
 
 int DeviceBatch::upload_coefficients(int i, const int16_t *src, size_t nblocks) {
@@ -291,6 +333,7 @@
     dispose_done_ = false;
     int rc = sync();
     if (rc != JPGPU_OK) return rc;
+    if ((rc = make_store_dense()) != JPGPU_OK) return rc;
     hipError_t e = hipMemcpy((int16_t *)d_coefs_.ptr + img->coef_offset * 64, src, nblocks * 128, hipMemcpyHostToDevice);
     return e == hipSuccess ? JPGPU_OK : hip_fail(e, "hipMemcpy(coefficients)");
 }
diff --git a/jpeglibrary_amd/csrc/k2_huffman.hip b/jpeglibrary_amd/csrc/k2_huffman.hip
--- a/jpeglibrary_amd/csrc/k2_huffman.hip
+++ b/jpeglibrary_amd/csrc/k2_huffman.hip
@@ -133,6 +133,12 @@
     const uint32_t swz16 = ((lane >> 1) & 7u) << 4;
 
     const uint64_t coef_off = s.coef_off;
+    const bool split = (s.reserved0 & kScanSplitHandoff) != 0;
+    uint8_t *split_lo = reinterpret_cast<uint8_t *>(coefs + coef_off * 64);
+    const uint64_t split_hi_off = split_plane_lines(n_intervals, dri_eff, bpm) * 128;
+    uint64_t *split_flags = reinterpret_cast<uint64_t *>(coefs) + (s.reserved0 >> kSplitFlagShift) + (uint64_t)(wave_first >> 6) * dri_eff * bpm;
+    uint32_t split_step = 0;
+    uint64_t my_flags = 0;
 
     for (uint32_t mcu = 0; mcu < wave_mcus; mcu++) {
         for (uint32_t b = 0; b < bpm; b++) {
@@ -171,22 +177,56 @@
             __builtin_amdgcn_fence(__ATOMIC_RELEASE, "wavefront");
             __builtin_amdgcn_wave_barrier();
             __builtin_amdgcn_fence(__ATOMIC_ACQUIRE, "wavefront");
+            if (!split) {
 #pragma unroll
-            for (int it = 0; it < 8; it++) {
-                const uint32_t blk = it * 8 + (lane >> 3);
-                const uint32_t chunk = lane & 7;
-                uint4 *src = reinterpret_cast<uint4 *>(stage + blk * 128 + ((chunk ^ ((blk >> 1) & 7)) * 16));
-                const uint4 v = *src;
-                const uint4 z = {0, 0, 0, 0};
-                *src = z;
-                const uint32_t owner = wave_first + blk;
-                if (owner < n_ends) {
-                    const uint32_t owner_mcus = (owner == n_intervals - 1) ? total_mcus - owner * dri_eff : dri_eff;
-                    if (mcu < owner_mcus) {
-                        const uint64_t block_index = coef_off + ((uint64_t)owner * dri_eff + mcu) * bpm + b;
-                        *reinterpret_cast<uint4 *>(coefs + block_index * 64 + chunk * 8) = v;
+                for (int it = 0; it < 8; it++) {
+                    const uint32_t blk = it * 8 + (lane >> 3);
+                    const uint32_t chunk = lane & 7;
+                    uint4 *src = reinterpret_cast<uint4 *>(stage + blk * 128 + ((chunk ^ ((blk >> 1) & 7)) * 16));
+                    const uint4 v = *src;
+                    const uint4 z = {0, 0, 0, 0};
+                    *src = z;
+                    const uint32_t owner = wave_first + blk;
+                    if (owner < n_ends) {
+                        const uint32_t owner_mcus = (owner == n_intervals - 1) ? total_mcus - owner * dri_eff : dri_eff;
+                        if (mcu < owner_mcus) {
+                            const uint64_t block_index = coef_off + ((uint64_t)owner * dri_eff + mcu) * bpm + b;
+                            *reinterpret_cast<uint4 *>(coefs + block_index * 64 + chunk * 8) = v;
+                        }
                     }
                 }
+            } else {
+                uint64_t step_flags = 0;
+#pragma unroll
+                for (int it = 0; it < 4; it++) {
+                    const uint32_t blk = it * 16 + (lane >> 2);
+                    const uint32_t chunk = lane & 3;
+                    const uint32_t swz = (blk >> 1) & 7;
+                    uint4 *src_lo = reinterpret_cast<uint4 *>(stage + blk * 128 + ((chunk ^ swz) * 16));
+                    uint4 *src_hi = reinterpret_cast<uint4 *>(stage + blk * 128 + (((chunk + 4) ^ swz) * 16));
+                    const uint4 v = *src_lo, w = *src_hi;
+                    const uint4 z = {0, 0, 0, 0};
+                    *src_lo = z;
+                    *src_hi = z;
+                    const uint64_t nz = __ballot((w.x | w.y | w.z | w.w) != 0);
+                    const uint32_t even = wave_first + (blk & ~1u);
+                    const bool have = even < n_ends && mcu < ((even == n_intervals - 1) ? total_mcus - even * dri_eff : dri_eff);
+                    const uint64_t off = split_slot(wave_first + blk, mcu, b, dri_eff, bpm) * 64 + chunk * 16;
+                    if (have) *reinterpret_cast<uint4 *>(split_lo + off) = v;
+                    if (have && ((nz >> (lane & ~7u)) & 0xFFu) != 0) *reinterpret_cast<uint4 *>(split_lo + split_hi_off + off) = w;
+                    uint64_t x = nz | (nz >> 1);
+                    x = (x | (x >> 2)) & 0x1111111111111111ull;
+                    x = (x | (x >> 3)) & 0x0303030303030303ull;
+                    x = (x | (x >> 6)) & 0x000F000F000F000Full;
+                    x = (x | (x >> 12)) & 0x000000FF000000FFull;
+                    x = (x | (x >> 24)) & 0xFFFFull;
+                    step_flags |= x << (16 * it);
+                }
+                if (lane == (split_step & 63u)) my_flags = step_flags;
+                if ((split_step & 63u) == 63u || split_step + 1 == wave_mcus * bpm) {
+                    if (lane <= (split_step & 63u)) split_flags[(split_step & ~63u) + lane] = my_flags;
+                }
+                split_step++;
             }
             __builtin_amdgcn_fence(__ATOMIC_RELEASE, "wavefront");
             __builtin_amdgcn_wave_barrier();
diff --git a/jpeglibrary_amd/csrc/k3_idct.hip b/jpeglibrary_amd/csrc/k3_idct.hip
--- a/jpeglibrary_amd/csrc/k3_idct.hip
+++ b/jpeglibrary_amd/csrc/k3_idct.hip
@@ -17,6 +17,10 @@
 __device__ constexpr uint8_t kNat[64] = {0,  1,  8,  16, 9,  2,  3,  10, 17, 24, 32, 25, 18, 11, 4,  5,  12, 19, 26, 33, 40, 48,
                                          41, 34, 27, 20, 13, 6,  7,  14, 21, 28, 35, 42, 49, 56, 57, 50, 43, 36, 29, 22, 15, 23,
                                          30, 37, 44, 51, 58, 59, 52, 45, 38, 31, 39, 46, 53, 60, 61, 54, 47, 55, 62, 63};
+
+static_assert(kIdctBlocksPerWg == 256, "the split form's reciprocals are exact for tiles of up to 256 blocks");
+static_assert(kMaxBlocksPerMcu == 16, "kRecip16 and the 16-bit reciprocals of the split form cover 1..16 blocks per MCU");
+__device__ constexpr uint32_t kRecip16[kMaxBlocksPerMcu + 1] = {0, 65536, 32768, 21846, 16384, 13108, 10923, 9363, 8192, 7282, 6554, 5958, 5462, 5042, 4682, 4370, 4096};
 
 #define JPGPU_IDCT8(y0, y1, y2, y3, y4, y5, y6, y7)                     \
     {                                                                   \
@@ -426,7 +430,7 @@
 typedef __attribute__((address_space(3))) void jpgpu_lds_void;
 typedef const __attribute__((address_space(1))) void jpgpu_gbl_void;
 
-template <int FMT, int LAY, bool PRE>
+template <int FMT, int LAY, bool PRE, bool SPLIT = false>
 __device__ __forceinline__ void idct_output_body(
     const int16_t *__restrict__ coefs, const DevScan *__restrict__ scans, const IdctWork *__restrict__ work,
     const DevScanStatus *__restrict__ status, const DevQuantTable *__restrict__ quant_pool, uint8_t *__restrict__ out, YccRgbFactors kf) {
@@ -480,9 +484,100 @@
 
     auto tile_mcus = [&](uint32_t first) { return (range_end - first) < mcus_per_tile ? (range_end - first) : mcus_per_tile; };
     const uint32_t tile_blocks = mcus_per_tile * bpm;
-    auto dma_tile = [&](uint32_t tile_first) {
+    constexpr bool split = SPLIT && !PRE;
+    if (split && (s.reserved0 & kScanSplitHandoff) == 0) return;
+    const uint32_t sp_dri = split ? s.dri : 1u;
+    const uint32_t sp_rb = kRecip16[bpm <= (uint32_t)kMaxBlocksPerMcu ? bpm : 0];
+    const uint32_t sp_rd = __builtin_amdgcn_readfirstlane(sp_dri <= 256u ? ((1u << 20) + sp_dri - 1) / sp_dri : 0u);
+    const uint32_t sp_w = sp_dri * bpm;
+    const bool sp_fast = split && mcus_per_tile % (2 * sp_dri) == 0 && first_mcu % (2 * sp_dri) == 0;
+    const uint32_t sp_rw = __builtin_amdgcn_readfirstlane((65536u + sp_w - 1) / sp_w);
+    const uint8_t *sp_hi = coef_bytes + split_plane_lines(s.n_intervals, sp_dri, bpm) * 128;
+    const uint8_t *sp_flags = reinterpret_cast<const uint8_t *>(reinterpret_cast<const uint64_t *>(coefs) + (s.reserved0 >> kSplitFlagShift));
+    auto sp_locate = [&](uint32_t tile_first, uint32_t t, int k, uint32_t &line, uint32_t &iv, uint32_t &word) {
+        const uint32_t i0 = __builtin_amdgcn_readfirstlane(tile_first / sp_dri), m0 = tile_first - i0 * sp_dri;
+        const uint32_t blk = (uint32_t)k * 32 + (t >> 3);
+        uint32_t q = (blk * sp_rb) >> 16;
+        const uint32_t bb = blk - q * bpm;
+        const uint32_t last = s.total_mcus - 1 - tile_first;
+        q = q < last ? q : last;
+        const uint32_t mm = m0 + q;
+        const uint32_t by_mul = (mm * sp_rd) >> 20, by_cmp = mm >= sp_dri ? 1u : 0u;
+        const uint32_t qi = sp_dri > 256u ? by_cmp : by_mul;
+        const uint32_t m = mm - qi * sp_dri;
+        iv = i0 + qi;
+        line = ((iv >> 1) * sp_dri + m) * bpm + bb;
+        word = ((iv >> 6) * sp_dri + m) * bpm + bb;
+    };
+    auto sp_locate_fast = [&](uint32_t i0, uint32_t t, int k, uint32_t &iv, uint32_t &word) {
+        const uint32_t ll = (uint32_t)k * 16 + ((t >> 3) & 15u);
+        const uint32_t pp = (ll * sp_rw) >> 16;
+        iv = i0 + 2 * pp + ((t >> 7) & 1u);
+        iv = iv < s.n_intervals ? iv : s.n_intervals - 1;
+        word = (iv >> 6) * sp_w + (ll - pp * sp_w);
+    };
+    auto sp_own_block = [&](uint32_t t) {
+        const uint32_t ml = (t * sp_rb) >> 16, bb = t - ml * bpm;
+        const uint32_t ir = (ml * sp_rd) >> 20, m = ml - ir * sp_dri;
+        const uint32_t ll = ((ir >> 1) * sp_dri + m) * bpm + bb;
+        return ((ll >> 4) << 5) | ((ir & 1u) << 4) | (ll & 15u);
+    };
+    const uint32_t sp_ipt = __builtin_amdgcn_readfirstlane(mcus_per_tile / sp_dri);
+    uint32_t sp_i0 = __builtin_amdgcn_readfirstlane(first_mcu / sp_dri);
+    auto sp_load_flags = [&](uint32_t tile_first, uint32_t tile_i0, uint32_t (&fb)[8], uint32_t &bit_at) {
         uint32_t t_ = tid;
         asm volatile("" : "+v"(t_));
+        bit_at = 0;
+#pragma unroll
+        for (int k = 0; k < 8; k++) {
+            uint32_t line, iv, word;
+            if (sp_fast) sp_locate_fast(tile_i0, t_, k, iv, word);
+            else sp_locate(tile_first, t_, k, line, iv, word);
+            fb[k] = sp_flags[word * 8 + ((iv >> 3) & 7u)];
+            bit_at |= (iv & 7u) << (3 * k);
+        }
+    };
+    auto sp_pack_flags = [&](uint32_t (&fb)[8], uint32_t bit_at) {
+        uint32_t bits = 0;
+#pragma unroll
+        for (int k = 0; k < 8; k++) {
+            asm volatile("" : "+v"(fb[k]));
+            bits |= ((fb[k] >> ((bit_at >> (3 * k)) & 7u)) & 1u) << k;
+        }
+        return bits;
+    };
+    auto dma_tile = [&](uint32_t tile_first, uint32_t tile_i0, uint32_t hi_bits) {
+        uint32_t t_ = tid;
+        asm volatile("" : "+v"(t_));
+        if (split && sp_fast) {
+            const uint32_t piece = (t_ & 7) ^ ((t_ >> 4) & 7);
+            const uint32_t slot = ((t_ >> 3) & 15u) * 2 + (t_ >> 7);
+            const uint8_t *src = (piece < 4 ? coef_bytes : sp_hi) + (uint64_t)(tile_i0 >> 1) * sp_w * 128 + (slot * 64 + (piece & 3u) * 16);
+            const uint8_t *zeros = sp_flags - 128 + (piece & 3u) * 16;
+            const uint32_t fetch_bits = piece < 4 ? 0xFFu : hi_bits;
+#pragma unroll
+            for (int k = 0; k < 8; k++) {
+                const uint8_t *from = ((fetch_bits >> k) & 1u) ? src + (uint32_t)(k * 2048) : zeros;
+                if (k < 6 || (uint32_t)k * 32 + slot < tile_blocks)
+                    __builtin_amdgcn_global_load_lds((jpgpu_gbl_void *)from, (jpgpu_lds_void *)(sh + ((uint32_t)k * kIdctThreads + wave * 64) * 16), 16, 0, 0);
+            }
+            return;
+        }
+        if (split) {
+            const uint32_t piece = (t_ & 7) ^ ((t_ >> 4) & 7);
+#pragma unroll
+            for (int k = 0; k < 8; k++) {
+                uint32_t line, iv, word;
+                sp_locate(tile_first, t_, k, line, iv, word);
+                const bool wanted = k < 6 || (uint32_t)k * 32 + (t_ >> 3) < tile_blocks;
+                const bool fetch = wanted && (piece < 4 || ((hi_bits >> k) & 1u) != 0);
+                const uint8_t *src = (piece < 4 ? coef_bytes : sp_hi) + ((uint64_t)line * 128 + (iv & 1u) * 64 + (piece & 3u) * 16);
+                if (fetch)
+                    __builtin_amdgcn_global_load_lds((jpgpu_gbl_void *)src, (jpgpu_lds_void *)(sh + ((uint32_t)k * kIdctThreads + wave * 64) * 16), 16, 0, 0);
+                if (wanted && !fetch) *reinterpret_cast<uint4 *>(sh + ((uint32_t)k * kIdctThreads + t_) * 16) = uint4{0, 0, 0, 0};
+            }
+            return;
+        }
         const uint32_t dma_lane_off = (t_ >> 3) * 128 + (((t_ & 7) ^ ((t_ >> 4) & 7)) * 16);
         const uint8_t *src = coef_bytes + (uint64_t)tile_first * bpm * 128;
 #pragma unroll
@@ -492,7 +587,20 @@
                                                  (jpgpu_lds_void *)(sh + ((uint32_t)k * kIdctThreads + wave * 64) * 16), 16, 0, 0);
     };
 
-    dma_tile(first_mcu);
+    uint32_t hi_next = 0;
+    if (split) {
+        uint32_t fb[8], at;
+        sp_load_flags(first_mcu, sp_i0, fb, at);
+        asm volatile("s_waitcnt vmcnt(0)" ::: "memory");
+        hi_next = sp_pack_flags(fb, at);
+    }
+    dma_tile(first_mcu, sp_i0, hi_next);
+    if (split && first_mcu + mcus_per_tile < range_end) {
+        uint32_t fb[8], at;
+        sp_load_flags(first_mcu + mcus_per_tile, sp_i0 + sp_ipt, fb, at);
+        asm volatile("s_waitcnt vmcnt(0)" ::: "memory");
+        hi_next = sp_pack_flags(fb, at);
+    }
     asm volatile("s_waitcnt vmcnt(0)" ::: "memory");
     __syncthreads();
 
@@ -520,16 +628,22 @@
             }
         }
     } else {
-        constexpr bool kPerTile = (FMT == kFmtRgbU8 && (LAY == kLayYccH2V1 || LAY == kLayYccH2V2)) || (kSampleBytes && LAY == kLayGeneric);
+        constexpr bool kPerTile = split || (FMT == kFmtRgbU8 && (LAY == kLayYccH2V1 || LAY == kLayYccH2V2)) || (kSampleBytes && LAY == kLayGeneric);
         uint32_t t_ = tid;
         if (kPerTile) asm volatile("" : "+v"(t_));
+        if (split && sp_fast) t_ = sp_own_block(t_);
         if (have_block) block_dequant(sh + t_ * 128, (t_ >> 1) & 7, sh_q[ci_early], f);
     }
     asm volatile("s_waitcnt lgkmcnt(0)" ::: "memory");
     __builtin_amdgcn_s_barrier();
-    if (have_next) dma_tile(next_first);
+    if (have_next) dma_tile(next_first, sp_i0 + sp_ipt, hi_next);
+    hi_next = 0;
 
     if (!PRE && have_block) block_idct(f, (int32_t)s.level_shift, px);
+    uint32_t sp_fb[8], sp_at = 0;
+    const bool sp_ahead = split && next_first + mcus_per_tile < range_end;
+    if (sp_ahead) sp_load_flags(next_first + mcus_per_tile, sp_i0 + 2 * sp_ipt, sp_fb, sp_at);
+    sp_i0 += sp_ipt;
     const bool reached = mcu < decoded && mcu * bpm + b < fail_block;
     if ((s.shadow_mask & 0xFu) == 0) {
         writes = writes && (reached || !keep);
@@ -562,12 +676,13 @@
     const uint32_t mcu_y = mcu_late / s.mcus_per_line, mcu_x = mcu_late - mcu_y * s.mcus_per_line;
     const uint32_t ci = s.blk_comp[b_late < kMaxBlocksPerMcu ? b_late : 0];
     const DevScanComponent comp = s.comp[ci];
+    const uint32_t b_out = split ? b_late : b;
 
     if (FMT == kFmtPlanarI16) {
         if (writes) {
             int16_t *plane = reinterpret_cast<int16_t *>(out + s.out_off + s.plane_off[ci]);
             const uint32_t pitch = s.plane_pitch[ci];
-            const uint32_t x0 = (mcu_x * comp.h + s.blk_x[b]) * 8, y0 = (mcu_y * comp.v + s.blk_y[b]) * 8;
+            const uint32_t x0 = (mcu_x * comp.h + s.blk_x[b_out]) * 8, y0 = (mcu_y * comp.v + s.blk_y[b_out]) * 8;
 #pragma unroll
             for (int r = 0; r < 8; r++) {
                 const uint4 v = {px[r * 4 + 0], px[r * 4 + 1], px[r * 4 + 2], px[r * 4 + 3]};
@@ -601,7 +716,7 @@
 
     if (CONV != 0 && LAY == kLayGray) {
         if (writes) {
-            const uint32_t x0 = (mcu_x * comp.h + s.blk_x[b]) * 8, y0 = (mcu_y * comp.v + s.blk_y[b]) * 8;
+            const uint32_t x0 = (mcu_x * comp.h + s.blk_x[b_out]) * 8, y0 = (mcu_y * comp.v + s.blk_y[b_out]) * 8;
 #pragma unroll
             for (int r = 0; r < 8; r++) {
                 if (y0 + r >= s.height) continue;
@@ -616,7 +731,7 @@
             const bool gray = kSampleBytes;
             uint8_t *plane = out + s.out_off + (gray ? 0 : s.plane_off[ci]);
             const uint32_t pitch = gray ? s.width : s.plane_pitch[ci];
-            const uint32_t x0 = (mcu_x * comp.h + s.blk_x[b]) * 8, y0 = (mcu_y * comp.v + s.blk_y[b]) * 8;
+            const uint32_t x0 = (mcu_x * comp.h + s.blk_x[b_out]) * 8, y0 = (mcu_y * comp.v + s.blk_y[b_out]) * 8;
 #pragma unroll
             for (int r = 0; r < 8; r++)
                 if (!gray || y0 + r < s.height) *reinterpret_cast<uint2 *>(plane + (size_t)(y0 + r) * pitch + x0) = rows[r];
@@ -627,6 +742,7 @@
         for (int r = 0; r < 8; r++) *reinterpret_cast<uint2 *>(sh_px + r * kPxRowStride + tid * 8) = rows[r];
     }
     asm volatile("s_waitcnt vmcnt(0)\n\ts_waitcnt lgkmcnt(0)" ::: "memory");
+    if (sp_ahead) hi_next = sp_pack_flags(sp_fb, sp_at);
     __builtin_amdgcn_s_barrier();
     synced = true;
 
@@ -636,6 +752,7 @@
 
     if (!synced) {
         asm volatile("s_waitcnt vmcnt(0)\n\ts_waitcnt lgkmcnt(0)" ::: "memory");
+        if (sp_ahead) hi_next = sp_pack_flags(sp_fb, sp_at);
         __builtin_amdgcn_s_barrier();
     }
   }
@@ -654,11 +771,47 @@
 }
 
 
+__global__ __launch_bounds__(256) void expand_handoff_kernel(const int16_t *__restrict__ coefs, int16_t *__restrict__ dense,
+                                                             const DevScan *__restrict__ scans, const uint32_t *__restrict__ scan_ids) {
+    const DevScan &s = scans[scan_ids[blockIdx.y]];
+    const uint32_t bpm = s.blocks_per_mcu, dri = s.dri;
+    const uint32_t n_blocks = s.total_mcus * bpm;
+    const uint8_t *lo = reinterpret_cast<const uint8_t *>(coefs + s.coef_off * 64);
+    const uint8_t *hi = lo + split_plane_lines(s.n_intervals, dri, bpm) * 128;
+    const uint64_t *flags = reinterpret_cast<const uint64_t *>(coefs) + (s.reserved0 >> kSplitFlagShift);
+    const uint32_t piece = threadIdx.x & 7;
+    for (uint32_t g = blockIdx.x * 32 + (threadIdx.x >> 3); g < n_blocks; g += gridDim.x * 32) {
+        const uint32_t mcu = g / bpm, b = g - mcu * bpm;
+        const uint32_t i = mcu / dri, m = mcu - i * dri;
+        const uint64_t off = split_slot(i, m, b, dri, bpm) * 64 + (piece & 3) * 16;
+        uint4 v = {0, 0, 0, 0};
+        if (piece < 4) v = *reinterpret_cast<const uint4 *>(lo + off);
+        else if ((flags[split_flag_word(i, m, b, dri, bpm)] >> (i & 63u)) & 1u) v = *reinterpret_cast<const uint4 *>(hi + off);
+        *reinterpret_cast<uint4 *>(dense + (s.coef_off + g) * 64 + piece * 8) = v;
+    }
+}
+hipError_t launch_expand_handoff(hipStream_t stream, const int16_t *coefs, int16_t *dense, const DevScan *scans, const uint32_t *scan_ids, int n_scans,
+                                 uint32_t max_blocks) {
+    if (n_scans <= 0 || max_blocks == 0) return hipSuccess;
+    const uint32_t bx = (uint32_t)std::min<uint64_t>(((uint64_t)max_blocks + 31) / 32, 2048);
+    for (int base = 0; base < n_scans; base += 65535) {
+        const int n = n_scans - base < 65535 ? n_scans - base : 65535;
+        hipLaunchKernelGGL(expand_handoff_kernel, dim3(bx, (uint32_t)n), dim3(256), 0, stream, coefs, dense, scans, scan_ids + base);
+    }
+    return hipGetLastError();
+}
+
 template <int FMT, int LAY>
 __global__ __launch_bounds__(kIdctThreads, (FMT == kFmtPlanarI16 ? 2 : 3)) void idct_output_kernel(
     const int16_t *__restrict__ coefs, const DevScan *__restrict__ scans, const IdctWork *__restrict__ work,
     const DevScanStatus *__restrict__ status, const DevQuantTable *__restrict__ quant_pool, uint8_t *__restrict__ out, YccRgbFactors kf) {
     idct_output_body<FMT, LAY, false>(coefs, scans, work, status, quant_pool, out, kf);
+}
+template <int FMT, int LAY>
+__global__ __launch_bounds__(kIdctThreads, (FMT == kFmtPlanarI16 ? 2 : 3)) void idct_split_kernel(
+    const int16_t *__restrict__ coefs, const DevScan *__restrict__ scans, const IdctWork *__restrict__ work,
+    const DevScanStatus *__restrict__ status, const DevQuantTable *__restrict__ quant_pool, uint8_t *__restrict__ out, YccRgbFactors kf) {
+    idct_output_body<FMT, LAY, false, true>(coefs, scans, work, status, quant_pool, out, kf);
 }
 template <int FMT>
 __global__ __launch_bounds__(kIdctThreads, 2) void flush_output_kernel(
@@ -700,19 +853,26 @@
 }
 
 template <int FMT, int LAY>
-static void launch_idct_one(hipStream_t stream, const int16_t *coefs, const DevScan *scans, const IdctWork *work, int n_work,
+static void launch_idct_one(hipStream_t stream, const int16_t *coefs, const DevScan *scans, const IdctWork *work, int n_work, int n_dense,
                             const DevScanStatus *status, const DevQuantTable *quant_pool, uint8_t *out,
                             YccRgbFactors kf = YccRgbFactors{0, 0, 0, 0}) {
-    hipLaunchKernelGGL((idct_output_kernel<FMT, LAY>), dim3(n_work), dim3(kIdctThreads), 0, stream, coefs, scans, work, status,
-                       quant_pool, out, kf);
+    if (n_dense > 0)
+        hipLaunchKernelGGL((idct_output_kernel<FMT, LAY>), dim3(n_dense), dim3(kIdctThreads), 0, stream, coefs, scans, work, status,
+                           quant_pool, out, kf);
+    if constexpr (idct_split_supported(FMT, LAY))
+      if (n_work > n_dense)
+        hipLaunchKernelGGL((idct_split_kernel<FMT, LAY>), dim3(n_work - n_dense), dim3(kIdctThreads), 0, stream, coefs, scans, work + n_dense, status,
+                           quant_pool, out, kf);
 }
 
 hipError_t launch_idct(hipStream_t stream, const int16_t *coefs, const DevScan *scans, const IdctWork *work,
                        const int class_begin[kNumIdctLayoutClasses + 1], const DevScanStatus *status,
-                       const DevQuantTable *quant_pool, uint8_t *out, int format, const YccRgbFactors &kf, uint8_t *generic_out) {
+                       const DevQuantTable *quant_pool, uint8_t *out, int format, const YccRgbFactors &kf, uint8_t *generic_out,
+                       const int *split_begin) {
     for (int c = 0; c < kNumIdctLayoutClasses; c++) {
         const int n = class_begin[c + 1] - class_begin[c];
         if (n <= 0) continue;
+        const int nd = split_begin ? split_begin[c] - class_begin[c] : n;
         const IdctWork *w = work + class_begin[c];
         if (c == kIdctClassStoreHoldsSamples) {
             if (format == kFmtPlanarI16) hipLaunchKernelGGL((flush_output_kernel<kFmtPlanarI16>), dim3(n), dim3(kIdctThreads), 0, stream, coefs, scans, w, status, quant_pool, out, kf);
@@ -721,40 +881,40 @@
             else hipLaunchKernelGGL((flush_output_kernel<kFmtInterleavedU8>), dim3(n), dim3(kIdctThreads), 0, stream, coefs, scans, w, status, quant_pool,
                                     (format == kFmtRgbU8 || format == kFmtRgbaU8) ? generic_out : out, kf);
         } else if (format == kFmtPlanarI16) {
-            launch_idct_one<kFmtPlanarI16, kLayGeneric>(stream, coefs, scans, w, n, status, quant_pool, out);
+            launch_idct_one<kFmtPlanarI16, kLayGeneric>(stream, coefs, scans, w, n, nd, status, quant_pool, out);
         } else if (format == kFmtPlanarU8) {
-            launch_idct_one<kFmtPlanarU8, kLayGeneric>(stream, coefs, scans, w, n, status, quant_pool, out);
+            launch_idct_one<kFmtPlanarU8, kLayGeneric>(stream, coefs, scans, w, n, nd, status, quant_pool, out);
         } else if (format == kFmtRgbU8) {
             switch (c) {
-            case kLayYccH1V1: launch_idct_one<kFmtRgbU8, kLayYccH1V1>(stream, coefs, scans, w, n, status, quant_pool, out, kf); break;
-            case kLayYccH2V1: launch_idct_one<kFmtRgbU8, kLayYccH2V1>(stream, coefs, scans, w, n, status, quant_pool, out, kf); break;
-            case kLayYccH2V2: launch_idct_one<kFmtRgbU8, kLayYccH2V2>(stream, coefs, scans, w, n, status, quant_pool, out, kf); break;
-            case kLayGray: launch_idct_one<kFmtRgbU8, kLayGray>(stream, coefs, scans, w, n, status, quant_pool, out, kf); break;
-            default: launch_idct_one<kFmtInterleavedU8, kLayGeneric>(stream, coefs, scans, w, n, status, quant_pool, generic_out); break;
+            case kLayYccH1V1: launch_idct_one<kFmtRgbU8, kLayYccH1V1>(stream, coefs, scans, w, n, nd, status, quant_pool, out, kf); break;
+            case kLayYccH2V1: launch_idct_one<kFmtRgbU8, kLayYccH2V1>(stream, coefs, scans, w, n, nd, status, quant_pool, out, kf); break;
+            case kLayYccH2V2: launch_idct_one<kFmtRgbU8, kLayYccH2V2>(stream, coefs, scans, w, n, nd, status, quant_pool, out, kf); break;
+            case kLayGray: launch_idct_one<kFmtRgbU8, kLayGray>(stream, coefs, scans, w, n, nd, status, quant_pool, out, kf); break;
+            default: launch_idct_one<kFmtInterleavedU8, kLayGeneric>(stream, coefs, scans, w, n, nd, status, quant_pool, generic_out); break;
             }
         } else if (format == kFmtRgbaU8) {
             switch (c) {
-            case kLayYccH1V1: launch_idct_one<kFmtRgbaU8, kLayYccH1V1>(stream, coefs, scans, w, n, status, quant_pool, out, kf); break;
-            case kLayYccH2V1: launch_idct_one<kFmtRgbaU8, kLayYccH2V1>(stream, coefs, scans, w, n, status, quant_pool, out, kf); break;
-            case kLayYccH2V2: launch_idct_one<kFmtRgbaU8, kLayYccH2V2>(stream, coefs, scans, w, n, status, quant_pool, out, kf); break;
-            case kLayGray: launch_idct_one<kFmtRgbaU8, kLayGray>(stream, coefs, scans, w, n, status, quant_pool, out, kf); break;
-            default: launch_idct_one<kFmtInterleavedU8, kLayGeneric>(stream, coefs, scans, w, n, status, quant_pool, generic_out); break;
+            case kLayYccH1V1: launch_idct_one<kFmtRgbaU8, kLayYccH1V1>(stream, coefs, scans, w, n, nd, status, quant_pool, out, kf); break;
+            case kLayYccH2V1: launch_idct_one<kFmtRgbaU8, kLayYccH2V1>(stream, coefs, scans, w, n, nd, status, quant_pool, out, kf); break;
+            case kLayYccH2V2: launch_idct_one<kFmtRgbaU8, kLayYccH2V2>(stream, coefs, scans, w, n, nd, status, quant_pool, out, kf); break;
+            case kLayGray: launch_idct_one<kFmtRgbaU8, kLayGray>(stream, coefs, scans, w, n, nd, status, quant_pool, out, kf); break;
+            default: launch_idct_one<kFmtInterleavedU8, kLayGeneric>(stream, coefs, scans, w, n, nd, status, quant_pool, generic_out); break;
             }
         } else if (format == kFmtInterleavedU8Scaled) {
             switch (c) {
-            case kLayYccH1V1: launch_idct_one<kFmtInterleavedU8Scaled, kLayYccH1V1>(stream, coefs, scans, w, n, status, quant_pool, out); break;
-            case kLayYccH2V1: launch_idct_one<kFmtInterleavedU8Scaled, kLayYccH2V1>(stream, coefs, scans, w, n, status, quant_pool, out); break;
-            case kLayYccH2V2: launch_idct_one<kFmtInterleavedU8Scaled, kLayYccH2V2>(stream, coefs, scans, w, n, status, quant_pool, out); break;
-            case kLayGray: launch_idct_one<kFmtInterleavedU8Scaled, kLayGray>(stream, coefs, scans, w, n, status, quant_pool, out); break;
-            default: launch_idct_one<kFmtInterleavedU8Scaled, kLayGeneric>(stream, coefs, scans, w, n, status, quant_pool, out); break;
+            case kLayYccH1V1: launch_idct_one<kFmtInterleavedU8Scaled, kLayYccH1V1>(stream, coefs, scans, w, n, nd, status, quant_pool, out); break;
+            case kLayYccH2V1: launch_idct_one<kFmtInterleavedU8Scaled, kLayYccH2V1>(stream, coefs, scans, w, n, nd, status, quant_pool, out); break;
+            case kLayYccH2V2: launch_idct_one<kFmtInterleavedU8Scaled, kLayYccH2V2>(stream, coefs, scans, w, n, nd, status, quant_pool, out); break;
+            case kLayGray: launch_idct_one<kFmtInterleavedU8Scaled, kLayGray>(stream, coefs, scans, w, n, nd, status, quant_pool, out); break;
+            default: launch_idct_one<kFmtInterleavedU8Scaled, kLayGeneric>(stream, coefs, scans, w, n, nd, status, quant_pool, out); break;
             }
         } else {
             switch (c) {
-            case kLayYccH1V1: launch_idct_one<kFmtInterleavedU8, kLayYccH1V1>(stream, coefs, scans, w, n, status, quant_pool, out); break;
-            case kLayYccH2V1: launch_idct_one<kFmtInterleavedU8, kLayYccH2V1>(stream, coefs, scans, w, n, status, quant_pool, out); break;
-            case kLayYccH2V2: launch_idct_one<kFmtInterleavedU8, kLayYccH2V2>(stream, coefs, scans, w, n, status, quant_pool, out); break;
-            case kLayGray: launch_idct_one<kFmtInterleavedU8, kLayGray>(stream, coefs, scans, w, n, status, quant_pool, out); break;
-            default: launch_idct_one<kFmtInterleavedU8, kLayGeneric>(stream, coefs, scans, w, n, status, quant_pool, out); break;
+            case kLayYccH1V1: launch_idct_one<kFmtInterleavedU8, kLayYccH1V1>(stream, coefs, scans, w, n, nd, status, quant_pool, out); break;
+            case kLayYccH2V1: launch_idct_one<kFmtInterleavedU8, kLayYccH2V1>(stream, coefs, scans, w, n, nd, status, quant_pool, out); break;
+            case kLayYccH2V2: launch_idct_one<kFmtInterleavedU8, kLayYccH2V2>(stream, coefs, scans, w, n, nd, status, quant_pool, out); break;
+            case kLayGray: launch_idct_one<kFmtInterleavedU8, kLayGray>(stream, coefs, scans, w, n, nd, status, quant_pool, out); break;
+            default: launch_idct_one<kFmtInterleavedU8, kLayGeneric>(stream, coefs, scans, w, n, nd, status, quant_pool, out); break;
             }
         }
         const hipError_t e = hipGetLastError();
diff --git a/jpeglibrary_amd/csrc/kernels.h b/jpeglibrary_amd/csrc/kernels.h
--- a/jpeglibrary_amd/csrc/kernels.h
+++ b/jpeglibrary_amd/csrc/kernels.h
@@ -50,9 +50,20 @@
 constexpr int kNumIdctLayoutClasses = 6;
 constexpr int kIdctClassStoreHoldsSamples = 5;
 int idct_layout_class(const DevScan &s);
+constexpr bool idct_split_supported(int format, int layout_class) {
+    if (format == kFmtPlanarI16 || format == kFmtPlanarU8 || format == kFmtExtendedU16) return true;
+    if (layout_class == 0 || layout_class >= kIdctClassStoreHoldsSamples) return false;
+    if (format == kFmtRgbU8) return layout_class == 1 || layout_class == 4;
+    if (format == kFmtRgbaU8) return layout_class != 3;
+    if (format == kFmtInterleavedU8Scaled) return layout_class != 4;
+    return true;
+}
 hipError_t launch_idct(hipStream_t stream, const int16_t *coefs, const DevScan *scans, const IdctWork *work,
                        const int class_begin[kNumIdctLayoutClasses + 1], const DevScanStatus *status,
-                       const DevQuantTable *quant_pool, uint8_t *out, int format, const YccRgbFactors &kf, uint8_t *generic_out);
+                       const DevQuantTable *quant_pool, uint8_t *out, int format, const YccRgbFactors &kf, uint8_t *generic_out,
+                       const int *split_begin = nullptr);
+hipError_t launch_expand_handoff(hipStream_t stream, const int16_t *coefs, int16_t *dense, const DevScan *scans, const uint32_t *scan_ids, int n_scans,
+                                 uint32_t max_blocks);
 hipError_t launch_dispose_pass(hipStream_t stream, int16_t *coefs, const DisposeJob *jobs, int n_jobs, uint32_t max_blocks, const DevQuantTable *quant_pool);
 hipError_t launch_ycc_to_rgb(hipStream_t stream, const uint8_t *src, uint8_t *dst, uint64_t n_pixels, int comps, int bpp, const YccRgbFactors &kf);
 
```

Result: faster. 599,200 Mpixels/s, median of 6 (+8.4%).
